# bytedance/particle-sfm

Hardware: AMD Instinct MI355X
Metric: trajectory-points/s (higher is better)
Workload: dtype f32 sampling + f64 positions; 1 GPU; configs[1]: synthetic 100x(1920x1080) flow pairs, sample_ratio=2, flow_check + chaining + occlusion + id assignment, 1 sequence per GPU; frames=101, height=1080, width=1920, trajectories=2073277, parallelism=sequence-per-gpu x1, world_size=1

## Files before the change

particle-sfm_amd/csrc/psfm_api.hip:

```cpp
#include <stdarg.h>
#include <stdio.h>
#include <string.h>
#include <mutex>
#include <shared_mutex>
#include <atomic>
#include <chrono>
#include <stdlib.h>

#include "psfm_internal.h"

static thread_local char g_err[512] = "";
static std::shared_mutex g_dev_gate[16];
std::shared_mutex& psfm_device_gate(int device) { return g_dev_gate[device & 15]; }
static std::atomic<int> g_dev_waiters[16];
int psfm_gate_waiters(int device) { return g_dev_waiters[device & 15].load(std::memory_order_relaxed); }
void psfm_gate_waiters_add(int device, int d) { g_dev_waiters[device & 15].fetch_add(d, std::memory_order_relaxed); }
static int psfm_wants_persist(psfm_ctx* c, bool optimize, int h, int w, int ratio, bool fused)
{
    if (c->chain_mode == 1 || ratio < 1 || !psfm_frame_ok(h, w)) return 0;
    if (optimize) return c->resident_budget > 0 ? 0 : 1;
    const int64_t G = (int64_t)((w + ratio - 1) / ratio) * ((h + ratio - 1) / ratio);
    const int64_t P = (int64_t)h * w;
    const int maxb = psfm_persist_max_blocks(c);
    if (maxb <= 0 || (G + 255) / 256 > maxb) return 0;
    if (c->chain_mode == 2) return 2;
    if (ratio < 2 || G < 100000) return 0;
    if (fused && (G < 400000 || P > 6 * G)) return 0;
    return 1;
}

void psfm_set_error(const char* fmt, ...)
{
    va_list ap;
    va_start(ap, fmt);
    vsnprintf(g_err, sizeof(g_err), fmt, ap);
    va_end(ap);
}

extern "C" const char* psfm_last_error(void) { return g_err; }
extern "C" int psfm_version(void) { return PSFM_VERSION; }

extern "C" int psfm_device_count(void)
{
    int n = 0;
    if (hipGetDeviceCount(&n) != hipSuccess) { (void)hipGetLastError(); return 0; }
    return n;
}

psfm_status PsfmBuf::ensure(size_t need)
{
    if (need <= bytes) return PSFM_OK;
    if (p) { (void)hipFree(p); p = nullptr; bytes = 0; }
    size_t want = (need + (size_t)(1 << 20) - 1) & ~((size_t)(1 << 20) - 1);
    hipError_t e = hipMalloc(&p, want);
    if (e != hipSuccess) {
        p = nullptr;
        psfm_set_error("hipMalloc(%zu bytes) failed: %s", want, hipGetErrorString(e));
        return PSFM_ERR_HIP;
    }
    bytes = want;
    return PSFM_OK;
}

void PsfmBuf::release()
{
    if (p) (void)hipFree(p);
    p = nullptr;
    bytes = 0;
}

hipEvent_t PsfmProfiler::get()
{
    if (!pool.empty()) { hipEvent_t e = pool.back(); pool.pop_back(); return e; }
    hipEvent_t e;
    (void)hipEventCreate(&e);
    return e;
}
void PsfmProfiler::begin(int kind, hipStream_t s)
{
    if (!enabled) return;
    Span sp; sp.kind = kind; sp.a = get(); sp.b = get();
    (void)hipEventRecord(sp.a, s);
    spans.push_back(sp);
}
void PsfmProfiler::kernel_span(int kind, hipEvent_t* a, hipEvent_t* b, bool always)
{
    if (!enabled || (!always && (calls++ % stride) != 0)) { *a = nullptr; *b = nullptr; return; }
    Span sp; sp.kind = kind; sp.a = get(); sp.b = get();
    spans.push_back(sp);
    *a = sp.a; *b = sp.b;
}
void PsfmProfiler::end(hipStream_t s)
{
    if (!enabled) return;
    (void)hipEventRecord(spans.back().b, s);
}
void PsfmProfiler::collect()
{
    for (auto& sp : spans) {
        float ms = 0.f;
        if (hipEventElapsedTime(&ms, sp.a, sp.b) == hipSuccess) { total_ms[sp.kind] += ms; launches[sp.kind]++; }
        pool.push_back(sp.a); pool.push_back(sp.b);
    }
    spans.clear();
}
void PsfmProfiler::reset()
{
    for (int k = 0; k < PSFM_PROF_KINDS; ++k) { total_ms[k] = 0; launches[k] = 0; }
}
void PsfmProfiler::destroy()
{
    collect();
    for (auto e : pool) (void)hipEventDestroy(e);
    pool.clear();
}

#define PSFM_CHECK_CTX(c)                                                     \
    do {                                                                      \
        if (!(c)) { psfm_set_error("ctx is NULL"); return PSFM_ERR_ARG; }     \
        PSFM_HIP(hipSetDevice((c)->device));                                  \
    } while (0)

extern "C" psfm_status psfm_ctx_create(int device, psfm_ctx** out)
{
    if (!out) { psfm_set_error("psfm_ctx_create: out is NULL"); return PSFM_ERR_ARG; }
    *out = nullptr;
    int n = 0;
    hipError_t e = hipGetDeviceCount(&n);
    if (e != hipSuccess || n <= 0) {
        (void)hipGetLastError();
        psfm_set_error("no HIP device available (%s); libpsfm_hip has no CPU fallback",
                       e != hipSuccess ? hipGetErrorString(e) : "device count 0");
        return PSFM_ERR_HIP;
    }
    if (device < 0 || device >= n) { psfm_set_error("device %d out of range [0,%d)", device, n); return PSFM_ERR_ARG; }
    PSFM_HIP(hipSetDevice(device));
    psfm_ctx* c = new psfm_ctx();
    c->device = device;
    c->host_pinned_bytes = 512 + sizeof(PsfmShard) * PSFM_NSHARD + 4096;
    e = hipHostMalloc(&c->host_pinned, c->host_pinned_bytes, hipHostMallocDefault);
    if (e != hipSuccess) { delete c; psfm_set_error("hipHostMalloc failed: %s", hipGetErrorString(e)); return PSFM_ERR_HIP; }
    *out = c;
    return PSFM_OK;
}

extern "C" psfm_status psfm_ctx_destroy(psfm_ctx* c)
{
    if (!c) return PSFM_OK;
    (void)hipSetDevice(c->device);
    PsfmBuf* bufs[] = {&c->log, &c->birth_frame, &c->birth_idx, &c->free_stack, &c->fin_keys, &c->fin_lanes,
                       &c->occupied, &c->counters, &c->shards, &c->survivors, &c->sort_keys, &c->sort_lanes, &c->sort_tmp,
                       &c->scan_tmp, &c->fin_marks, &c->res_birth, &c->res_len, &c->res_off, &c->res_xy, &c->sol_x, &c->sol_state,
                       &c->sol_partials, &c->sol_ctrl, &c->sol_misc, &c->sol_stats, &c->sol_fused, &c->sol_bar, &c->sol_list, &c->occ_own, &c->occ2_own,
                       &c->handoff, &c->seg_info, &c->seg_table, &c->persist_bar, &c->batch_tab, &c->batch_ws, &c->batch_fc, &c->win_ws, &c->flt_ids, &c->flt_birth, &c->flt_len, &c->flt_off, &c->flt_xy,
                       &c->mt_kp_off, &c->mt_q, &c->mt_pts, &c->mt_kp_ind, &c->mt_kp_xy, &c->mt_moff, &c->mt_keys, &c->mt_rows, &c->mt_gid, &c->mt_pairs,
                       &c->lb_state, &c->lb_first, &c->lb_flag, &c->lb_ws, &c->lb_ids, &c->lb_off, &c->lb_frames, &c->lb_xy, &c->lb_labels};
    for (auto b : bufs) b->release();
    for (void*& q : c->peer_opened) { if (q) (void)hipIpcCloseMemHandle(q); q = nullptr; }
    c->peer_area.release();
    psfm_shard_abandon(c);
    c->prof.destroy();
    if (c->side_stream) (void)hipStreamDestroy(c->side_stream);
    if (c->redo_stream) (void)hipStreamDestroy(c->redo_stream);
    if (c->copy_stream) (void)hipStreamDestroy(c->copy_stream);
    if (c->copy_stream2) (void)hipStreamDestroy(c->copy_stream2);
    for (void* p : c->ingest_slots) (void)hipHostFree(p);
    for (hipEvent_t e : c->ingest_events) (void)hipEventDestroy(e);
    if (c->host_pinned) (void)hipHostFree(c->host_pinned);
    if (c->host_seg) (void)hipHostFree(c->host_seg);
    if (c->host_batch) (void)hipHostFree(c->host_batch);
    if (c->host_batch2) (void)hipHostFree(c->host_batch2);
    delete c;
    return PSFM_OK;
}

extern "C" psfm_status psfm_ctx_set_capacity(psfm_ctx* c, double lane_factor, double traj_factor)
{
    if (!c || !(lane_factor >= 1.0) || !(traj_factor >= 1.0)) { psfm_set_error("psfm_ctx_set_capacity: factors must be >= 1"); return PSFM_ERR_ARG; }
    c->lane_factor = lane_factor;
    c->traj_factor = traj_factor;
    return PSFM_OK;
}

extern "C" psfm_status psfm_ctx_set_chain_mode(psfm_ctx* c, int mode)
{
    if (!c || mode < 0 || mode > 2) { psfm_set_error("psfm_ctx_set_chain_mode: mode must be 0 (auto), 1 (per-frame launches) or 2 (persistent loop)"); return PSFM_ERR_ARG; }
    c->chain_mode = mode;
    return PSFM_OK;
}

extern "C" psfm_status psfm_ctx_set_solver(psfm_ctx* c, int mode, int k)
{
    if (!c || mode < 0 || mode > 2 || k < 0 || k > psfm_solve_kmax()) {
        psfm_set_error("psfm_ctx_set_solver: mode must be 0 (adaptive), 1 (launch chain) or 2 (fused solve), k in [0, %d]", psfm_solve_kmax());
        return PSFM_ERR_ARG;
    }
    c->solver_mode = mode;
    c->solver_K = k;
    return PSFM_OK;
}

extern "C" psfm_status psfm_solver_counters(psfm_ctx* c, int64_t* fused, int64_t* fused_redone, int64_t* chain, int32_t* k_now)
{
    if (!c) { psfm_set_error("ctx is NULL"); return PSFM_ERR_ARG; }
    if (fused) *fused = c->n_fused_ok;
    if (fused_redone) *fused_redone = c->n_fused_redone;
    if (chain) *chain = c->n_chain;
    if (k_now) *k_now = c->solve_K;
    return PSFM_OK;
}

extern "C" psfm_status psfm_ctx_set_resident_budget(psfm_ctx* c, int blocks)
{
    if (!c || blocks < 0) { psfm_set_error("psfm_ctx_set_resident_budget: blocks must be >= 0"); return PSFM_ERR_ARG; }
    c->resident_budget = blocks;
    return PSFM_OK;
}

extern "C" psfm_status psfm_resident_capacity(psfm_ctx* c, int32_t* blocks)
{
    PSFM_CHECK_CTX(c);
    if (blocks) *blocks = psfm_resident_blocks(c);
    return PSFM_OK;
}

extern "C" psfm_status psfm_solver_launches(psfm_ctx* c, int64_t* resident, int64_t* giveups, int64_t* iterations)
{
    if (!c) { psfm_set_error("ctx is NULL"); return PSFM_ERR_ARG; }
    if (resident) *resident = c->n_resident;
    if (giveups) *giveups = c->pc_giveups;
    if (iterations) *iterations = c->n_iter_launches;
    return PSFM_OK;
}

extern "C" psfm_status psfm_ctx_set_profiling(psfm_ctx* c, int enable)
{
    if (!c) { psfm_set_error("ctx is NULL"); return PSFM_ERR_ARG; }
    c->prof.enabled = enable != 0;
    c->prof.stride = enable > 1 ? enable : 1;
    c->prof.calls = 0;
    c->prof.collect();
    c->prof.reset();
    return PSFM_OK;
}

extern "C" psfm_status psfm_profile_get(psfm_ctx* c, int kind, double* total_ms, int64_t* launches)
{
    if (!c || kind < 0 || kind >= PSFM_PROF_KINDS) { psfm_set_error("psfm_profile_get: bad argument"); return PSFM_ERR_ARG; }
    if (total_ms) *total_ms = c->prof.total_ms[kind];
    if (launches) *launches = c->prof.launches[kind];
    return PSFM_OK;
}

extern "C" psfm_status psfm_flow_check(psfm_ctx* c, const float* flows_f, const float* flows_b, int n_pairs, int h, int w,
                                       float thres, uint8_t* occ_out, float* err_out, void* stream)
{
    PSFM_CHECK_CTX(c);
    PsfmGate gate(c->device, 0);
    if (n_pairs < 0 || !psfm_frame_ok(h, w) || (n_pairs > 0 && (!flows_f || !flows_b || !occ_out))) {
        psfm_set_error("psfm_flow_check: bad argument (n_pairs=%d h=%d w=%d)", n_pairs, h, w);
        return PSFM_ERR_ARG;
    }
    hipStream_t s = (hipStream_t)stream;
    c->prof.begin(PSFM_PROF_FLOW_CHECK, s);
    psfm_status st = psfm_launch_flow_check(flows_f, flows_b, n_pairs, h, w, thres, occ_out, err_out, s);
    c->prof.end(s);
    return st;
}

extern "C" psfm_status psfm_grid_sample(psfm_ctx* c, const float* map_hwc, int ch, int h, int w, const double* xy,
                                        int64_t n, float* out, void* stream)
{
    PSFM_CHECK_CTX(c);
    PsfmGate gate(c->device, 0);
    if ((ch != 1 && ch != 2) || !psfm_frame_ok(h, w) || n < 0 || (n > 0 && (!map_hwc || !xy || !out))) {
        psfm_set_error("psfm_grid_sample: bad argument (c=%d h=%d w=%d n=%lld)", ch, h, w, (long long)n);
        return PSFM_ERR_ARG;
    }
    return psfm_launch_grid_sample(map_hwc, ch, h, w, xy, n, out, (hipStream_t)stream);
}

extern "C" psfm_status psfm_optimize_location(psfm_ctx* c, const double* uv12, const double* ref1, const double* ref2,
                                              const double* scale, const float* flow12, int64_t n, int w, int h,
                                              double* out, psfm_solve_stats* stats_host, void* stream)
{
    PSFM_CHECK_CTX(c);
    PsfmGate gate(c->device, (c->chain_mode == 1 || c->resident_budget > 0) ? 0 : 1);
    c->pc_persist_ok = gate.exclusive || c->resident_budget > 0;
    c->pc_giveups = 0;
    c->n_resident = c->n_iter_launches = 0;
    if (n < 0 || !psfm_frame_ok(h, w) || (n > 0 && (!uv12 || !ref1 || !ref2 || !scale || !flow12 || !out))) {
        psfm_set_error("psfm_optimize_location: bad argument (n=%lld h=%d w=%d)", (long long)n, h, w);
        return PSFM_ERR_ARG;
    }
    psfm_solve_stats st;
    memset(&st, 0, sizeof(st));
    hipStream_t s = (hipStream_t)stream;
    c->prof.begin(PSFM_PROF_SOLVER, s);
    psfm_status rc = psfm_solve_batch(c, uv12, ref1, ref2, scale, flow12, n, w, h, out, &st, s);
    c->prof.end(s);
    if (stats_host) *stats_host = st;
    return rc;
}

extern "C" psfm_status psfm_path_consistency_eval(psfm_ctx* c, const double* uv12, const double* ref1, const double* ref2,
                                                  const double* scale, const float* flow12, int64_t n, int w, int h,
                                                  double* residuals, double* jacobians, void* stream)
{
    PSFM_CHECK_CTX(c);
    PsfmGate gate(c->device, 0);
    if (n < 0 || n > 0x3fffffff || !psfm_frame_ok(h, w) || (n > 0 && (!uv12 || !ref1 || !ref2 || !scale || !flow12 || (!residuals && !jacobians)))) {
        psfm_set_error("psfm_path_consistency_eval: bad argument (n=%lld h=%d w=%d)", (long long)n, h, w);
        return PSFM_ERR_ARG;
    }
    return psfm_launch_pc_eval(uv12, ref1, ref2, scale, flow12, n, w, h, residuals, jacobians, (hipStream_t)stream);
}

extern "C" psfm_status psfm_sort_records(psfm_ctx* c, uint32_t* keys, int32_t* values, int64_t n, int end_bit, void* stream)
{
    PSFM_CHECK_CTX(c);
    PsfmGate gate(c->device, 0);
    if (n < 0 || n >= (1ll << 31) || end_bit < 1 || end_bit > 32 || (n > 0 && (!keys || !values))) {
        psfm_set_error("psfm_sort_records: bad argument (n=%lld end_bit=%d)", (long long)n, end_bit);
        return PSFM_ERR_ARG;
    }
    if (n == 0) return PSFM_OK;
    hipStream_t s = (hipStream_t)stream;
    psfm_status st;
    if ((st = c->sort_keys.ensure(sizeof(unsigned long long) * (size_t)n * 2)) != PSFM_OK) return st;
    if ((st = c->sort_lanes.ensure(sizeof(int) * (size_t)n * 2)) != PSFM_OK) return st;
    const int64_t half = psfm_sort_pairs32_passes((unsigned)end_bit) % 2 == 0 ? 0 : n;
    unsigned* k0 = c->sort_keys.as<unsigned>();
    int* v0 = c->sort_lanes.as<int>();
    PSFM_HIP(hipMemcpyAsync(k0 + half, keys, sizeof(unsigned) * (size_t)n, hipMemcpyDeviceToDevice, s));
    PSFM_HIP(hipMemcpyAsync(v0 + half, values, sizeof(int) * (size_t)n, hipMemcpyDeviceToDevice, s));
    if ((st = psfm_sort_pairs32(c, k0, v0, k0 + n, v0 + n, n, (unsigned)end_bit, s)) != PSFM_OK) return st;
    PSFM_HIP(hipMemcpyAsync(keys, k0, sizeof(unsigned) * (size_t)n, hipMemcpyDeviceToDevice, s));
    PSFM_HIP(hipMemcpyAsync(values, v0, sizeof(int) * (size_t)n, hipMemcpyDeviceToDevice, s));
    return PSFM_OK;
}

psfm_status psfm_track_dims(psfm_ctx* c, int n_flows, int h, int w, int ratio, int64_t g_own, PsfmTrackDims& d)
{
    d.H = h; d.W = w; d.ratio = ratio; d.n_flows = n_flows;
    d.GW = (w + ratio - 1) / ratio; d.GH = (h + ratio - 1) / ratio;
    d.G = (int64_t)d.GW * d.GH;
    const int64_t Gown = g_own < 0 ? d.G : (g_own > 0 ? g_own : 1);
    d.cap = (int64_t)(c->lane_factor * (double)Gown);
    d.cap = ((d.cap + 255) / 256) * 256;
    const int64_t n_blocks = d.cap / 256;
    {
        const int64_t gb = (Gown + 255) / 256;
        d.nsh = (int)(gb < PSFM_NSHARD ? (gb > 0 ? gb : 1) : PSFM_NSHARD);
    }
    d.free_cap = (int)(((n_blocks + d.nsh - 1) / d.nsh) * 256) + 1024;
    const double tf = c->traj_factor > (double)n_flows / 8.0 ? c->traj_factor : (double)n_flows / 8.0;
    d.shard_cap = (int)(((int64_t)(tf * (double)Gown) + d.cap) / d.nsh) + 1024;
    d.traj_cap = (int64_t)d.shard_cap * PSFM_NSHARD;
    if (d.cap > 0x7fffffff / 2 || d.traj_cap > 0x7fffffff / 2) { psfm_set_error("psfm_track: grid too large"); return PSFM_ERR_ARG; }
    d.shift_b = 1; while ((1ll << d.shift_b) < d.G) ++d.shift_b;
    int tbits = 1; while ((1ll << tbits) < (long long)n_flows + 2) ++tbits;
    d.shift_d = d.shift_b + tbits;
    if (d.shift_d + tbits > 63) { psfm_set_error("psfm_track: key does not fit 64 bits"); return PSFM_ERR_ARG; }
    d.cw = (float)((double)(w - 1) / 2.0); d.ch = (float)((double)(h - 1) / 2.0);
    return PSFM_OK;
}

psfm_status psfm_track_alloc(psfm_ctx* c, const PsfmTrackDims& d)
{
    psfm_status st;
    const int n_flows = d.n_flows;
    if ((st = c->log.ensure(sizeof(double2) * (size_t)(n_flows + 1) * d.cap)) != PSFM_OK) return st;
    if ((st = c->birth_frame.ensure(sizeof(int) * d.cap)) != PSFM_OK) return st;
    if ((st = c->birth_idx.ensure(sizeof(int) * d.cap)) != PSFM_OK) return st;
    if ((st = c->free_stack.ensure(sizeof(int) * (size_t)d.free_cap * PSFM_NSHARD * 2)) != PSFM_OK) return st;
    if ((st = c->shards.ensure(sizeof(PsfmShard) * PSFM_NSHARD * 2)) != PSFM_OK) return st;
    if ((st = c->fin_keys.ensure(sizeof(unsigned long long) * d.traj_cap)) != PSFM_OK) return st;
    if ((st = c->fin_lanes.ensure(sizeof(int) * d.traj_cap)) != PSFM_OK) return st;
    if ((st = c->occupied.ensure((size_t)d.G * 3 + 8)) != PSFM_OK) return st;
    if ((st = c->counters.ensure(sizeof(PsfmCounters))) != PSFM_OK) return st;
    if ((st = c->survivors.ensure(sizeof(int) * (size_t)(n_flows + 1))) != PSFM_OK) return st;
    return PSFM_OK;
}

struct PsfmOccPipeline {
    int chunk = 0;
    std::vector<hipEvent_t> ready;
    std::vector<hipEvent_t> ready_s2;
    int waited = -1, waited_s2 = -1;
    psfm_status need(int pair, bool s2, hipStream_t s)
    {
        if (chunk <= 0) return PSFM_OK;
        std::vector<hipEvent_t>& ev = s2 ? ready_s2 : ready;
        int& w = s2 ? waited_s2 : waited;
        const int cidx = pair / chunk;
        while (w < cidx && w + 1 < (int)ev.size()) {
            ++w;
            PSFM_HIP(hipStreamWaitEvent(s, ev[w], 0));
        }
        return PSFM_OK;
    }
};

static psfm_status psfm_track_impl(psfm_ctx* c, const float* flows, const uint8_t* occ, const float* flows_f2,
                                   const uint8_t* occ_s2, int n_flows, int h, int w, int ratio, psfm_track_info* info,
                                   void* stream, PsfmOccPipeline* pipe, PsfmGate& gate,
                                   const float* fuse_flows_b = nullptr, float fuse_thres = 0.f, int64_t occ_pitch = 0)
{
    const bool device_is_ours = gate.exclusive;
    if (occ_pitch == 0) occ_pitch = (int64_t)h * w;
    PSFM_CHECK_CTX(c);
    psfm_shard_abandon(c);
    const bool optimize = flows_f2 != nullptr;
    if (n_flows < 1 || !psfm_frame_ok(h, w) || ratio < 1 || !flows || !occ || (optimize && !occ_s2 && n_flows > 1)) {
        psfm_set_error("psfm_track: bad argument (n_flows=%d h=%d w=%d ratio=%d)", n_flows, h, w, ratio);
        return PSFM_ERR_ARG;
    }
    if (ratio > 64) { psfm_set_error("psfm_track: sample_ratio %d > 64 unsupported", ratio); return PSFM_ERR_ARG; }
    hipStream_t s = (hipStream_t)stream;
    PsfmTrackDims d;
    psfm_status st;
    if ((st = psfm_track_dims(c, n_flows, h, w, ratio, -1, d)) != PSFM_OK) return st;
    const int64_t P = (int64_t)h * w;
    if ((st = psfm_track_alloc(c, d)) != PSFM_OK) return st;

    c->solve_stats.clear();
    c->res_n_traj = c->res_n_points = 0;
    c->res_n_flows = n_flows;
    c->pc_persist_ok = device_is_ours || c->resident_budget > 0;
    c->pc_giveups = 0;

    if (!optimize && c->chain_mode != 1) {
        const int maxb = psfm_persist_max_blocks(c);
        const int64_t need_blocks = (d.G + 255) / 256;
        if (maxb > 0 && need_blocks <= maxb && device_is_ours) {
            PsfmTrackDims dp = d;
            int64_t nb = need_blocks <= 256 ? 2 * need_blocks + 4 : need_blocks + need_blocks / 4;
            dp.nblk = (int)(nb < maxb ? nb : maxb);
            if (fuse_flows_b) {
                const int64_t fc_blocks = (P + 1023) / 1024;
                const int64_t want = fc_blocks < maxb ? fc_blocks : maxb;
                if (want > dp.nblk) dp.nblk = (int)want;
            }
            dp.cap = (int64_t)dp.nblk * (256 + psfm_persist_guests());
            dp.nsh = dp.nblk < PSFM_NSHARD ? dp.nblk : PSFM_NSHARD;
            dp.free_cap = (int)(((dp.nblk + dp.nsh - 1) / dp.nsh) * 256) + 1024;
            dp.seg_cap = (int)(d.traj_cap / dp.nblk) + 64;
            dp.spill_cap = (int)(d.traj_cap / 8) + 4096;
            const int64_t fin_total = (int64_t)dp.nblk * dp.seg_cap + dp.spill_cap;
            if ((st = c->log.ensure(sizeof(double2) * (size_t)(n_flows + 1) * dp.cap)) != PSFM_OK) return st;
            if ((st = c->free_stack.ensure(sizeof(int) * (size_t)dp.free_cap * PSFM_NSHARD * 2)) != PSFM_OK) return st;
            if ((st = c->fin_keys.ensure(sizeof(unsigned long long) * fin_total)) != PSFM_OK) return st;
            if ((st = c->fin_lanes.ensure(sizeof(int) * fin_total)) != PSFM_OK) return st;
            if ((st = c->handoff.ensure((size_t)dp.nblk * 256 * 24)) != PSFM_OK) return st;
            if ((st = c->seg_info.ensure(sizeof(int) * 2 * (size_t)dp.nblk)) != PSFM_OK) return st;
            if ((st = c->persist_bar.ensure((size_t)(4 * PSFM_NSHARD + 1) * 128)) != PSFM_OK) return st;
            if (pipe && (st = pipe->need(n_flows - 1, false, s)) != PSFM_OK) return st;
            bool fallback = false;
            {
                const bool trace = getenv("PSFM_TRACE") != nullptr;
                const auto t1 = std::chrono::steady_clock::now();
                st = psfm_launch_chain_persist(c, dp, flows, occ, occ_pitch, fuse_flows_b, fuse_thres, s);
                if (st == PSFM_ERR_CAPACITY) {
                    fallback = true;
                    st = PSFM_OK;
                } else {
                    if (st != PSFM_OK) return st;
                    c->prof.begin(PSFM_PROF_FINALIZE, s);
                    st = psfm_finalize_persist(c, dp, &fallback, s);
                    c->prof.end(s);
                }
                if (trace) {
                    const auto t2 = std::chrono::steady_clock::now();
                    fprintf(stderr, "[psfm %p] persistent loop: launch+finalize %.2f ms, fallback %d, overflow %d\n", (void*)c,
                            std::chrono::duration<double, std::milli>(t2 - t1).count(), (int)fallback,
                            ((PsfmCounters*)c->host_pinned)->overflow);
                }
            }
            if (st != PSFM_OK) return st;
            if (!fallback) {
                PSFM_HIP(hipStreamSynchronize(s));
                c->prof.collect();
                if (info) {
                    memset(info, 0, sizeof(*info));
                    info->n_traj = c->res_n_traj;
                    info->n_points = c->res_n_points;
                    info->n_lanes_peak = ((PsfmCounters*)c->host_pinned)->n_lanes;
                    info->lane_capacity = dp.cap;
                    info->chain_mode = 2;
                }
                return PSFM_OK;
            }
            c->prof.collect();
        }
    }
    if (fuse_flows_b) {
        c->prof.begin(PSFM_PROF_FLOW_CHECK, s);
        for (int f = 0; f < n_flows; ++f)
            if ((st = psfm_launch_flow_check(flows + (size_t)f * P * 2, fuse_flows_b + (size_t)f * P * 2, 1, h, w, fuse_thres,
                                             const_cast<uint8_t*>(occ) + (size_t)f * occ_pitch, nullptr, s)) != PSFM_OK) return st;
        c->prof.end(s);
    }
    if ((st = psfm_launch_track_init(c, d, s)) != PSFM_OK) return st;
    int64_t total_iters = 0;
    static const int check_env = getenv("PSFM_CHECK_FRAMES") ? atoi(getenv("PSFM_CHECK_FRAMES")) : 0;
    const int PSFM_CHECK = check_env >= 2 ? check_env : 16;
    std::vector<psfm_solve_stats> hstats((size_t)n_flows + 1);
    int first_unchecked = 1;
    if (optimize) {
        if ((st = c->sol_stats.ensure(sizeof(psfm_solve_stats) * (size_t)(n_flows + 1))) != PSFM_OK) return st;
    }
    const char* unroll_env = getenv("PSFM_SOLVE_UNROLL");
    const int unroll_fixed = unroll_env ? (atoi(unroll_env) < 1 ? 1 : atoi(unroll_env)) : 0;
    c->n_fused_ok = c->n_fused_redone = c->n_chain = 0;
    c->n_resident = c->n_iter_launches = 0;
    if (optimize && (st = psfm_solve_prepare(c, d, s)) != PSFM_OK) return st;
    static const bool merge = !(getenv("PSFM_MERGE_FRAME") && atoi(getenv("PSFM_MERGE_FRAME")) == 0);
    const bool seq_env = !(getenv("PSFM_SEQ") && atoi(getenv("PSFM_SEQ")) == 0);
    bool seq_ok = optimize && merge && seq_env && unroll_fixed == 0;
    int launch_id = 0;
    int idle_windows = 0;
    bool pc_in_step = true;
    int* hpc = (int*)((char*)c->host_pinned + 320);
    PsfmCounters* dctr = c->counters.as<PsfmCounters>();

    auto checkpoint = [&](int f_hi, bool fused_now, bool seq, int* f_next) -> psfm_status {
        PsfmCounters* hc = (PsfmCounters*)c->host_pinned;
        PSFM_HIP(hipMemcpyAsync(hc, c->counters.p, sizeof(PsfmCounters), hipMemcpyDeviceToHost, s));
        PSFM_HIP(hipMemcpyAsync(hstats.data() + first_unchecked, c->sol_stats.as<psfm_solve_stats>() + first_unchecked,
                                sizeof(psfm_solve_stats) * (size_t)(f_hi - first_unchecked + 1), hipMemcpyDeviceToHost, s));
        PSFM_HIP(hipStreamSynchronize(s));
        if (gate.yield_exclusive()) c->pc_persist_ok = c->resident_budget > 0;
        if ((hc->overflow & 7) != 0 || hc->n_lanes > d.cap) {
            psfm_set_error("capacity exceeded: lanes used %d of %lld, overflow bits %d (frame %d of %d); raise psfm_ctx_set_capacity",
                           hc->n_lanes, (long long)d.cap, hc->overflow, hc->pc_frame, n_flows);
            return PSFM_ERR_CAPACITY;
        }
        const int stalled = hc->stall ? hc->stall - 1 : -1;
        int last_ok = f_hi;
        if (seq) {
            const int pcf = hc->pc_frame < n_flows ? hc->pc_frame : n_flows;
            last_ok = pcf - 1;
        }
        if (stalled >= 0) {
            const int fs = stalled;
            psfm_solve_stats ss;
            memset(&ss, 0, sizeof(ss));
            const int k_used = c->solver_K > 0 ? c->solver_K : c->solve_K;
            psfm_status st2 = psfm_solve_frame_resume(c, d, flows + (size_t)(fs - 1) * P * 2, flows + (size_t)fs * P * 2,
                                                      flows_f2 + (size_t)(fs - 1) * P * 2, occ_s2 + (size_t)(fs - 1) * P, fs, &ss,
                                                      (fused_now && !seq && c->solver_K == 0 && k_used < psfm_solve_kmax())
                                                          ? (k_used + 2 < psfm_solve_kmax() ? k_used + 2 : psfm_solve_kmax()) : 0,
                                                      !fused_now, s);
            if (st2 != PSFM_OK) return st2;
            hstats[fs] = ss;
            last_ok = fs;
            pc_in_step = false;
        }
        int max_it = 0, n_solved = 0, n_unclean = 0, k_need = 2;
        for (int k = first_unchecked; k <= last_ok; ++k) {
            if (hstats[k].termination >= 0) {
                c->solve_stats.push_back(hstats[k]);
                total_iters += hstats[k].iterations;
                const psfm_solve_stats& q = hstats[k];
                const bool clean = q.dogleg_nonGN == 0 && q.termination != PSFM_TERM_FAILURE &&
                                   (q.iterations == q.successful_steps + 1 ||
                                    (q.termination == PSFM_TERM_GRADIENT_TOL && q.iterations == q.successful_steps)) &&
                                   q.successful_steps + 1 <= psfm_solve_kmax();
                ++n_solved;
                if (!clean) ++n_unclean;
                else if (q.successful_steps + 1 > k_need) k_need = q.successful_steps + 1;
                if (!fused_now) ++c->n_chain;
                else if (k == stalled) ++c->n_fused_redone;
                else ++c->n_fused_ok;
            }
            if (hstats[k].iterations > max_it) max_it = hstats[k].iterations;
        }
        if (n_solved > 0) {
            c->solve_mode = (n_unclean * 8 > n_solved) ? 1 : 0;
            if (seq) {
                int hist[16] = {0};
                for (int k = first_unchecked; k <= last_ok; ++k)
                    if (hstats[k].termination >= 0) ++hist[hstats[k].successful_steps + 1 < 15 ? hstats[k].successful_steps + 1 : 15];
                int best = 2;
                for (int q = 2; q <= psfm_solve_kmax(); ++q) if (hist[q] > hist[best]) best = q;
                c->solve_K = best;
            } else {
                c->solve_K = k_need > c->solve_K ? k_need : c->solve_K - (c->solve_K - k_need + 1) / 2;
            }
        }
        int want = max_it + 1;
        want = want < 4 ? 4 : (want > 64 ? 64 : want);
        c->solve_unroll = want > c->solve_unroll ? want : c->solve_unroll - (c->solve_unroll - want + 1) / 2;
        first_unchecked = last_ok + 1;
        *f_next = last_ok + 1;
        return PSFM_OK;
    };

    int f = 0;
    while (f < n_flows) {
        const bool fused_now = c->solver_mode == 2 || (c->solver_mode == 0 && c->solve_mode == 0);
        if (seq_ok && fused_now && f >= 1) {
            const int k_now = c->solver_K > 0 ? c->solver_K : c->solve_K;
            if (!pc_in_step) {
                hpc[0] = f; hpc[1] = 0; hpc[2] = launch_id; hpc[3] = k_now;
                PSFM_HIP(hipMemcpyAsync(&dctr->pc_frame, hpc, 4 * sizeof(int), hipMemcpyHostToDevice, s));
                pc_in_step = true;
            } else {
                hpc[3] = k_now;
                PSFM_HIP(hipMemcpyAsync(&dctr->solve_K, hpc + 3, sizeof(int), hipMemcpyHostToDevice, s));
            }
            const int left = n_flows - f;
            const int n_launch = (left < PSFM_CHECK ? left : PSFM_CHECK) + 2;
            const int f_hi = f + n_launch - 1 < n_flows - 1 ? f + n_launch - 1 : n_flows - 1;
            if (pipe && (st = pipe->need(f_hi, false, s)) != PSFM_OK) return st;
            if (pipe && (st = pipe->need(f_hi - 1, true, s)) != PSFM_OK) return st;
            if ((st = psfm_launch_seq(c, d, flows, occ, occ_pitch, flows_f2, occ_s2, n_launch, launch_id, s)) != PSFM_OK) return st;
            launch_id += n_launch;
            const int f_before = f;
            if ((st = checkpoint(f_hi, true, true, &f)) != PSFM_OK) return st;
            if (f == f_before) {
                if (getenv("PSFM_TRACE")) {
                    const PsfmCounters* hc = (const PsfmCounters*)c->host_pinned;
                    unsigned tk[8] = {0};
                    if (c->sol_fused.p) (void)hipMemcpy(tk, c->sol_fused.p, sizeof(tk), hipMemcpyDeviceToHost);
                    fprintf(stderr, "[psfm %p] device-paced window without a completed frame: host frame %d, next launch %d; device pc {frame %d, phase %d, "
                            "owner %d, K %d}, lanes %d (snapshots %d %d), stall %d, overflow %d, tickets %u %u %u %u\n", (void*)c, f, launch_id,
                            hc->pc_frame, hc->pc_phase, hc->pc_owner, hc->solve_K, hc->n_lanes, hc->n_lanes_snap[0], hc->n_lanes_snap[1], hc->stall,
                            hc->overflow, tk[0], tk[1], tk[2], tk[3]);
                }
                if (++idle_windows > 8) { psfm_set_error("psfm_track: the device-paced sequence made no progress in 8 windows (frame %d)", f); return PSFM_ERR_SOLVER; }
            } else {
                idle_windows = 0;
            }
            continue;
        }
        pc_in_step = false;
        if (pipe && (st = pipe->need(f, false, s)) != PSFM_OK) return st;
        const bool solve_now = optimize && f + 1 >= 2;
        if (solve_now && fused_now && merge) {
            if (pipe && (st = pipe->need(f - 1, true, s)) != PSFM_OK) return st;
            st = psfm_launch_frame(c, d, flows + (size_t)(f - 1) * P * 2, flows + (size_t)f * P * 2, flows_f2 + (size_t)(f - 1) * P * 2,
                                   occ + (size_t)f * occ_pitch, occ_s2 + (size_t)(f - 1) * P, f, c->solver_K > 0 ? c->solver_K : c->solve_K, s);
            if (st != PSFM_OK) return st;
        } else {
            st = psfm_launch_chain_step(c, d, flows + (size_t)f * P * 2, occ + (size_t)f * occ_pitch, f, optimize, s);
            if (st != PSFM_OK) return st;
            if (solve_now) {
                if (pipe && (st = pipe->need(f - 1, true, s)) != PSFM_OK) return st;
                if (fused_now) {
                    st = psfm_solve_frame_fused(c, d, flows + (size_t)(f - 1) * P * 2, flows + (size_t)f * P * 2,
                                                flows_f2 + (size_t)(f - 1) * P * 2, occ_s2 + (size_t)(f - 1) * P, f,
                                                c->solver_K > 0 ? c->solver_K : c->solve_K, s);
                } else {
                    c->prof.begin(PSFM_PROF_SOLVER, s);
                    st = psfm_solve_frame_enqueue(c, d, flows + (size_t)(f - 1) * P * 2, flows + (size_t)f * P * 2,
                                                  flows_f2 + (size_t)(f - 1) * P * 2, occ_s2 + (size_t)(f - 1) * P, f,
                                                  unroll_fixed > 0 ? unroll_fixed : c->solve_unroll, s);
                    c->prof.end(s);
                }
                if (st != PSFM_OK) return st;
            }
        }
        if (optimize && f >= 1 && ((f % PSFM_CHECK) == PSFM_CHECK - 1 || f == n_flows - 1)) {
            if ((st = checkpoint(f, fused_now, false, &f)) != PSFM_OK) return st;
            continue;
        }
        ++f;
    }
    if (optimize && n_flows >= 2 && (st = psfm_solve_flush(c, d, n_flows - 1, s)) != PSFM_OK) return st;
    c->prof.begin(PSFM_PROF_FINALIZE, s);
    st = psfm_finalize(c, d, s);
    c->prof.end(s);
    if (st != PSFM_OK) return st;
    PSFM_HIP(hipStreamSynchronize(s));
    c->prof.collect();
    if (info) {
        memset(info, 0, sizeof(*info));
        info->n_traj = c->res_n_traj;
        info->n_points = c->res_n_points;
        info->n_lanes_peak = ((PsfmCounters*)c->host_pinned)->n_lanes;
        info->lane_capacity = d.cap;
        info->solver_iterations = total_iters;
        info->n_solves = (int32_t)c->solve_stats.size();
        info->chain_mode = 1;
    }
    return PSFM_OK;
}

extern "C" psfm_status psfm_track(psfm_ctx* c, const float* flows, const uint8_t* occ, const float* flows_f2,
                                  const uint8_t* occ_s2, int n_flows, int h, int w, int ratio, psfm_track_info* info,
                                  void* stream)
{
    PSFM_CHECK_CTX(c);
    c->res_gen++;
    PsfmGate gate(c->device, psfm_wants_persist(c, flows_f2 != nullptr, h, w, ratio, false));
    return psfm_track_impl(c, flows, occ, flows_f2, occ_s2, n_flows, h, w, ratio, info, stream, nullptr, gate);
}

extern "C" psfm_status psfm_connect(psfm_ctx* c, const float* flows_f, const float* flows_b, const float* flows_f2,
                                    const float* flows_b2, int n_flows, int h, int w, float thres, int ratio,
                                    uint8_t* occ, uint8_t* occ_s2, psfm_track_info* info, void* stream)
{
    PSFM_CHECK_CTX(c);
    c->res_gen++;
    const bool optimize = flows_f2 != nullptr;
    PsfmGate gate(c->device, psfm_wants_persist(c, optimize, h, w, ratio, true));
    if (n_flows < 1 || !psfm_frame_ok(h, w) || !flows_f || !flows_b || (optimize && n_flows > 1 && !flows_b2)) {
        psfm_set_error("psfm_connect: bad argument (n_flows=%d h=%d w=%d)", n_flows, h, w);
        return PSFM_ERR_ARG;
    }
    hipStream_t s = (hipStream_t)stream;
    const size_t P = (size_t)h * w;
    psfm_status st;
    if (gate.exclusive && !optimize && (!occ || (P % 128 == 0 && ((uintptr_t)occ & 127) == 0))) {
        int64_t pitch = (int64_t)P;
        if (!occ) {
            pitch = (int64_t)((P + 127) / 128 * 128);
            if ((st = c->occ_own.ensure((size_t)pitch * (size_t)n_flows)) != PSFM_OK) return st;
            occ = c->occ_own.as<uint8_t>();
        }
        return psfm_track_impl(c, flows_f, occ, nullptr, nullptr, n_flows, h, w, ratio, info, stream, nullptr, gate, flows_b,
                               thres, pitch);
    }
    if (!occ) {
        if ((st = c->occ_own.ensure(P * (size_t)n_flows)) != PSFM_OK) return st;
        occ = c->occ_own.as<uint8_t>();
    }
    const int n2 = optimize ? (n_flows > 1 ? n_flows - 1 : 0) : 0;
    if (optimize && !occ_s2) {
        if ((st = c->occ2_own.ensure(P * (size_t)(n2 > 0 ? n2 : 1))) != PSFM_OK) return st;
        occ_s2 = c->occ2_own.as<uint8_t>();
    }
    if (!c->side_stream) PSFM_HIP(hipStreamCreateWithFlags(&c->side_stream, hipStreamNonBlocking));
    hipStream_t side = c->side_stream;
    hipEvent_t e_in = c->prof.get();
    PSFM_HIP(hipEventRecord(e_in, s));
    PSFM_HIP(hipStreamWaitEvent(side, e_in, 0));
    PsfmOccPipeline pipe;
    pipe.chunk = getenv("PSFM_FC_CHUNK") && atoi(getenv("PSFM_FC_CHUNK")) > 0 ? atoi(getenv("PSFM_FC_CHUNK")) : (optimize ? 5 : 10);
    c->prof.begin(PSFM_PROF_FLOW_CHECK, side);
    const bool bg = optimize && getenv("PSFM_FC_BG") && atoi(getenv("PSFM_FC_BG")) == 1;
    int cus = 256;
    if (bg) {
        (void)hipDeviceGetAttribute(&cus, hipDeviceAttributeMultiprocessorCount, c->device);
        const int mult = getenv("PSFM_FC_BG_BLOCKS") ? atoi(getenv("PSFM_FC_BG_BLOCKS")) : 0;
        cus *= mult > 0 ? mult : 0;
    }
    for (int p0 = 0; p0 < n_flows; p0 += pipe.chunk) {
        const int np = n_flows - p0 < pipe.chunk ? n_flows - p0 : pipe.chunk;
        if (bg && p0 > 0) st = psfm_launch_flow_check_bg(flows_f + (size_t)p0 * P * 2, flows_b + (size_t)p0 * P * 2, np, h, w, thres,
                                                        occ + (size_t)p0 * P, cus, side);
        else st = psfm_launch_flow_check(flows_f + (size_t)p0 * P * 2, flows_b + (size_t)p0 * P * 2, np, h, w, thres,
                                         occ + (size_t)p0 * P, nullptr, side);
        if (st != PSFM_OK) return st;
        hipEvent_t e = c->prof.get();
        PSFM_HIP(hipEventRecord(e, side));
        pipe.ready.push_back(e);
        if (p0 < n2) {
            const int np2 = n2 - p0 < pipe.chunk ? n2 - p0 : pipe.chunk;
            if (bg && p0 > 0) st = psfm_launch_flow_check_bg(flows_f2 + (size_t)p0 * P * 2, flows_b2 + (size_t)p0 * P * 2, np2, h, w, thres,
                                                            occ_s2 + (size_t)p0 * P, cus, side);
            else st = psfm_launch_flow_check(flows_f2 + (size_t)p0 * P * 2, flows_b2 + (size_t)p0 * P * 2, np2, h, w,
                                             thres, occ_s2 + (size_t)p0 * P, nullptr, side);
            if (st != PSFM_OK) return st;
            hipEvent_t e2 = c->prof.get();
            PSFM_HIP(hipEventRecord(e2, side));
            pipe.ready_s2.push_back(e2);
        }
    }
    c->prof.end(side);
    st = psfm_track_impl(c, flows_f, occ, flows_f2, occ_s2, n_flows, h, w, ratio, info, stream, &pipe, gate);
    c->prof.pool.push_back(e_in);
    for (auto e : pipe.ready) c->prof.pool.push_back(e);
    for (auto e : pipe.ready_s2) c->prof.pool.push_back(e);
    return st;
}

extern "C" psfm_status psfm_result_device(psfm_ctx* c, const int32_t** birth, const int32_t** len, const int64_t** off,
                                          const double** xy)
{
    if (!c) { psfm_set_error("ctx is NULL"); return PSFM_ERR_ARG; }
    if (birth) *birth = c->res_birth.as<int32_t>();
    if (len) *len = c->res_len.as<int32_t>();
    if (off) *off = c->res_off.as<int64_t>();
    if (xy) *xy = c->res_xy.as<double>();
    return PSFM_OK;
}

extern "C" psfm_status psfm_result_copy(psfm_ctx* c, int32_t* birth_host, int32_t* len_host, int64_t* off_host,
                                        double* xy_host, void* stream)
{
    PSFM_CHECK_CTX(c);
    PsfmGate gate(c->device, 0);
    hipStream_t s = (hipStream_t)stream;
    const int64_t n = c->res_n_traj, np = c->res_n_points;
    if (n > 0) {
        if (birth_host) PSFM_HIP(hipMemcpyAsync(birth_host, c->res_birth.p, sizeof(int32_t) * n, hipMemcpyDeviceToHost, s));
        if (len_host) PSFM_HIP(hipMemcpyAsync(len_host, c->res_len.p, sizeof(int32_t) * n, hipMemcpyDeviceToHost, s));
        if (off_host) PSFM_HIP(hipMemcpyAsync(off_host, c->res_off.p, sizeof(int64_t) * (n + 1), hipMemcpyDeviceToHost, s));
        if (xy_host && np > 0) PSFM_HIP(hipMemcpyAsync(xy_host, c->res_xy.p, sizeof(double) * 2 * np, hipMemcpyDeviceToHost, s));
    } else if (off_host) {
        off_host[0] = 0;
    }
    PSFM_HIP(hipStreamSynchronize(s));
    return PSFM_OK;
}

extern "C" psfm_status psfm_result_solve_stats(psfm_ctx* c, psfm_solve_stats* stats_host, int32_t max_n, int32_t* n_out)
{
    if (!c) { psfm_set_error("ctx is NULL"); return PSFM_ERR_ARG; }
    const int32_t n = (int32_t)c->solve_stats.size();
    if (n_out) *n_out = n;
    if (stats_host) for (int32_t i = 0; i < n && i < max_n; ++i) stats_host[i] = c->solve_stats[i];
    return PSFM_OK;
}
```

particle-sfm_amd/csrc/psfm_finalize.hip:

```cpp
#include <cstring>
#include <stdio.h>
#include <rocprim/device/device_radix_sort.hpp>
#include <rocprim/device/device_scan.hpp>

#include "psfm_device.h"
#include "psfm_internal.h"

#define PSFM_BLOCK 256

__device__ __forceinline__ void psfm_collect_alive_body(
    const int* __restrict__ birth_frame, const int* __restrict__ birth_idx, PsfmCounters* __restrict__ ctr,
    PsfmShard* __restrict__ shards, unsigned long long* __restrict__ fin_keys, int* __restrict__ fin_lanes, int cap,
    int shard_cap, int last_time, int shift_b, int shift_d)
{
    __shared__ int s_cnt[PSFM_BLOCK / PSFM_WAVE];
    __shared__ int s_base;
    const int n_lanes = min(ctr->n_lanes, cap);
    if ((int)(blockIdx.x * PSFM_BLOCK) >= n_lanes) return;
    const int i = blockIdx.x * PSFM_BLOCK + threadIdx.x;
    int bf = -1;
    if (i < n_lanes) bf = birth_frame[i];
    const bool pending = bf <= -2;
    const bool alive = (bf >= 0) | pending;
    const int my_last = pending ? last_time - 1 : last_time;
    if (pending) bf = -2 - bf;
    const unsigned long long am = __ballot(alive);
    const int lane = psfm_lane_id(), wave = threadIdx.x / PSFM_WAVE;
    if (lane == 0) s_cnt[wave] = __popcll(am);
    __syncthreads();
    const int shard = blockIdx.x % PSFM_NSHARD;
    if (threadIdx.x == 0) {
        int tot = 0;
        for (int w = 0; w < PSFM_BLOCK / PSFM_WAVE; ++w) tot += s_cnt[w];
        s_base = tot > 0 ? atomicAdd(&shards[shard].fin_cnt, tot) : 0;
    }
    __syncthreads();
    if (alive) {
        int r = s_base + psfm_rank_in(am);
        for (int w = 0; w < wave; ++w) r += s_cnt[w];
        if (r < shard_cap) {
            const int64_t o = (int64_t)shard * shard_cap + r;
            fin_keys[o] = ((unsigned long long)my_last << shift_d) | ((unsigned long long)bf << shift_b) |
                          (unsigned long long)birth_idx[i];
            fin_lanes[o] = i;
        } else {
            atomicOr(&ctr->overflow, 2);
        }
    }
}

__global__ __launch_bounds__(PSFM_BLOCK) void psfm_collect_alive_kernel(
    const int* __restrict__ birth_frame, const int* __restrict__ birth_idx, PsfmCounters* __restrict__ ctr,
    PsfmShard* __restrict__ shards, unsigned long long* __restrict__ fin_keys, int* __restrict__ fin_lanes, int cap,
    int shard_cap, int last_time, int shift_b, int shift_d)
{
    psfm_collect_alive_body(birth_frame, birth_idx, ctr, shards, fin_keys, fin_lanes, cap, shard_cap, last_time, shift_b, shift_d);
}

struct PsfmKeyFmt { int shift_b, shift_d; int use32; };
__device__ __forceinline__ unsigned psfm_key32(unsigned long long k, const PsfmKeyFmt& f)
{
    const unsigned last = (unsigned)(k >> f.shift_d);
    const unsigned birth = (unsigned)((k >> f.shift_b) & ((1ull << (f.shift_d - f.shift_b)) - 1ull));
    const unsigned idx = (unsigned)(k & ((1ull << f.shift_b) - 1ull));
    return ((last * (last + 1u) / 2u + birth) << f.shift_b) | idx;
}
__device__ __forceinline__ void psfm_put_key(unsigned long long* keys, int64_t pos, unsigned long long k, const PsfmKeyFmt& f)
{
    if (f.use32) ((unsigned*)keys)[pos] = psfm_key32(k, f);
    else keys[pos] = k;
}

struct PsfmShardOffsets { int count[PSFM_NSHARD]; int64_t start[PSFM_NSHARD]; };
__global__ __launch_bounds__(PSFM_BLOCK) void psfm_compact_shards_kernel(
    const unsigned long long* __restrict__ fin_keys, const int* __restrict__ fin_lanes, int shard_cap,
    PsfmShardOffsets so, unsigned long long* __restrict__ keys, int* __restrict__ lanes, PsfmKeyFmt fmt)
{
    const int shard = blockIdx.y;
    const int n = so.count[shard];
    for (int i = blockIdx.x * PSFM_BLOCK + threadIdx.x; i < n; i += gridDim.x * PSFM_BLOCK) {
        psfm_put_key(keys, so.start[shard] + i, fin_keys[(int64_t)shard * shard_cap + i], fmt);
        lanes[so.start[shard] + i] = fin_lanes[(int64_t)shard * shard_cap + i];
    }
}

__global__ __launch_bounds__(PSFM_BLOCK) void psfm_decode_kernel(const unsigned long long* __restrict__ keys, int64_t n,
                                                                 int shift_b, int shift_d, int* __restrict__ birth,
                                                                 int* __restrict__ len, int64_t* __restrict__ len64)
{
    const int64_t i = (int64_t)blockIdx.x * PSFM_BLOCK + threadIdx.x;
    if (i > n) return;
    if (i == n) { len64[i] = 0; return; }
    const unsigned long long k = keys[i];
    const int last = (int)(k >> shift_d);
    const int b = (int)((k >> shift_b) & ((1ull << (shift_d - shift_b)) - 1ull));
    birth[i] = b;
    len[i] = last - b + 1;
    len64[i] = (int64_t)(last - b + 1);
}

__global__ __launch_bounds__(PSFM_BLOCK) void psfm_decode32_kernel(const unsigned* __restrict__ keys, int64_t n, int shift_b,
                                                                   int* __restrict__ birth, int* __restrict__ len,
                                                                   int64_t* __restrict__ len64)
{
    const int64_t i = (int64_t)blockIdx.x * PSFM_BLOCK + threadIdx.x;
    if (i > n) return;
    if (i == n) { len64[i] = 0; return; }
    const unsigned tri = keys[i] >> shift_b;
    int l = (int)((sqrtf(8.0f * (float)tri + 1.0f) - 1.0f) * 0.5f);
    while (l > 0 && (unsigned)l * (unsigned)(l + 1) / 2u > tri) --l;
    while ((unsigned)(l + 1) * (unsigned)(l + 2) / 2u <= tri) ++l;
    const int b = (int)(tri - (unsigned)l * (unsigned)(l + 1) / 2u);
    birth[i] = b;
    len[i] = l - b + 1;
    len64[i] = (int64_t)(l - b + 1);
}

#define PSFM_PLAN_MAX_GROUPS 16384
#define PSFM_PLAN_BLOCK 1024
struct PsfmPlan {
    const int* gstart; const int64_t* goff;
    const void* keys; int use32, shift_b, shift_d;
    int* birth_w; int* len_w; int64_t* off_w;
};
__device__ __forceinline__ void psfm_tri_invert(unsigned tri, int* last, int* birth)
{
    int l = (int)((sqrtf(8.0f * (float)tri + 1.0f) - 1.0f) * 0.5f);
    while (l > 0 && (unsigned)l * (unsigned)(l + 1) / 2u > tri) --l;
    while ((unsigned)(l + 1) * (unsigned)(l + 2) / 2u <= tri) ++l;
    *last = l;
    *birth = (int)(tri - (unsigned)l * (unsigned)(l + 1) / 2u);
}
__device__ __forceinline__ void psfm_key_fields(const void* keys, int64_t id, int use32, int shift_b, int shift_d, int* last, int* birth, int* idx)
{
    if (use32) {
        const unsigned k = ((const unsigned*)keys)[id];
        psfm_tri_invert(k >> shift_b, last, birth);
        *idx = (int)(k & ((1u << shift_b) - 1u));
    } else {
        const unsigned long long k = ((const unsigned long long*)keys)[id];
        *last = (int)(k >> shift_d);
        *birth = (int)((k >> shift_b) & ((1ull << (shift_d - shift_b)) - 1ull));
        *idx = (int)(k & ((1ull << shift_b) - 1ull));
    }
}
__device__ __forceinline__ int psfm_key_group(const void* keys, int64_t id, int use32, int shift_b, int shift_d)
{
    if (use32) return (int)(((const unsigned*)keys)[id] >> shift_b);
    const unsigned long long k = ((const unsigned long long*)keys)[id];
    const unsigned last = (unsigned)(k >> shift_d);
    const unsigned birth = (unsigned)((k >> shift_b) & ((1ull << (shift_d - shift_b)) - 1ull));
    return (int)(last * (last + 1u) / 2u + birth);
}

__global__ __launch_bounds__(PSFM_BLOCK) void psfm_group_bounds_kernel(const void* __restrict__ keys, int64_t n, int use32, int shift_b,
                                                                       int shift_d, int* __restrict__ gstart)
{
    const int64_t i = (int64_t)blockIdx.x * PSFM_BLOCK + threadIdx.x;
    if (i >= n) return;
    const int g = psfm_key_group(keys, i, use32, shift_b, shift_d);
    const int gp = i > 0 ? psfm_key_group(keys, i - 1, use32, shift_b, shift_d) : -1;
    if (g != gp) gstart[g] = (int)i;
}

__global__ __launch_bounds__(PSFM_PLAN_BLOCK) void psfm_group_plan_kernel(int* __restrict__ marks, int* __restrict__ gstart,
                                                                          int64_t* __restrict__ goff, int ng, int64_t n,
                                                                          int64_t* __restrict__ off_n)
{
    __shared__ int s_g[PSFM_PLAN_MAX_GROUPS];
    __shared__ int s_wmin[PSFM_PLAN_BLOCK / PSFM_WAVE];
    __shared__ long long s_wsum[PSFM_PLAN_BLOCK / PSFM_WAVE];
    constexpr int NW = PSFM_PLAN_BLOCK / PSFM_WAVE;
    constexpr int INF = 0x7fffffff;
    const int tid = threadIdx.x, lane = tid & (PSFM_WAVE - 1), wave = tid / PSFM_WAVE;
    for (int k = tid; k < ng; k += PSFM_PLAN_BLOCK) {
        const int v = marks[k];
        s_g[k] = v;
        gstart[k] = v;
        if (v >= 0) marks[k] = -1;
    }
    __syncthreads();
    const int per = (ng + PSFM_PLAN_BLOCK - 1) / PSFM_PLAN_BLOCK;
    const int g0 = min(tid * per, ng), g1 = min(g0 + per, ng);
    int first = INF;
    for (int g = g1 - 1; g >= g0; --g) if (s_g[g] >= 0) first = s_g[g];
    int sm = first;
#pragma unroll
    for (int o = 1; o < PSFM_WAVE; o <<= 1) {
        const int v = __shfl_down(sm, o);
        if (lane + o < PSFM_WAVE && v < sm) sm = v;
    }
    if (lane == 0) s_wmin[wave] = sm;
    int nxt = __shfl_down(sm, 1);
    if (lane == PSFM_WAVE - 1) nxt = INF;
    __syncthreads();
    for (int w = wave + 1; w < NW; ++w) nxt = min(nxt, s_wmin[w]);
    if (nxt == INF) nxt = (int)n;
    int last = 0, birth = 0;
    if (g0 < g1) psfm_tri_invert((unsigned)g0, &last, &birth);
    for (int g = g1 - 1; g >= g0; --g) {
        const int st = s_g[g];
        if (st >= 0) { s_g[g] = nxt - st; nxt = st; } else s_g[g] = 0;
    }
    long long pts = 0;
    {
        int l = last, b = birth;
        for (int g = g0; g < g1; ++g) {
            pts += (long long)s_g[g] * (long long)(l - b + 1);
            if (++b > l) { ++l; b = 0; }
        }
    }
    long long inc = pts;
#pragma unroll
    for (int o = 1; o < PSFM_WAVE; o <<= 1) {
        const long long v = __shfl_up(inc, o);
        if (lane >= o) inc += v;
    }
    if (lane == PSFM_WAVE - 1) s_wsum[wave] = inc;
    __syncthreads();
    long long base = 0, total = 0;
    for (int w = 0; w < NW; ++w) { const long long v = s_wsum[w]; if (w < wave) base += v; total += v; }
    long long run = base + inc - pts;
    {
        int l = last, b = birth;
        for (int g = g0; g < g1; ++g) {
            goff[g] = run;
            run += (long long)s_g[g] * (long long)(l - b + 1);
            if (++b > l) { ++l; b = 0; }
        }
    }
    if (tid == 0) *off_n = total;
}

__device__ __forceinline__ void psfm_track_header(const PsfmPlan& pl, const int* __restrict__ birth, const int* __restrict__ len,
                                                  int64_t id, int* b, int* l, int* idx)
{
    if (pl.gstart) {
        int last;
        psfm_key_fields(pl.keys, id, pl.use32, pl.shift_b, pl.shift_d, &last, b, idx);
        *l = last - *b + 1;
    } else {
        *b = birth[id]; *l = len[id]; *idx = -1;
    }
}
__device__ __forceinline__ int64_t psfm_track_offset(const PsfmPlan& pl, const int64_t* __restrict__ off, int64_t id, int b, int l)
{
    if (!pl.gstart) return off[id];
    const int last = b + l - 1;
    const int g = last * (last + 1) / 2 + b;
    const int64_t o = pl.goff[g] + (id - (int64_t)pl.gstart[g]) * (int64_t)l;
    pl.birth_w[id] = b; pl.len_w[id] = l; pl.off_w[id] = o;
    return o;
}

#ifndef TILE_J
#define TILE_J 64
#endif
#ifndef TILE_K
#define TILE_K 32
#endif
__device__ __forceinline__ void psfm_gather_body(const double2* __restrict__ log, int64_t cap,
                                                                 const int* __restrict__ lanes,
                                                                 const int* __restrict__ birth,
                                                                 const int* __restrict__ len,
                                                                 const int64_t* __restrict__ off, int64_t n,
                                                                 double2* __restrict__ out, const PsfmPlan& pl)
{
    __shared__ double2 tile[TILE_J][TILE_K + 1];
    __shared__ int s_lane[TILE_J], s_birth[TILE_J], s_len[TILE_J];
    __shared__ int64_t s_off[TILE_J];
    __shared__ int s_maxlen;
    const int tid = threadIdx.x;
    const int64_t id0 = (int64_t)blockIdx.x * TILE_J;
    int hb = 0, hl = 0;
    if (tid == 0) s_maxlen = 0;
    __syncthreads();
    if (tid < TILE_J) {
        const int64_t id = id0 + tid;
        const bool ok = id < n;
        int b = 0, l = 0, idx;
        const int my_lane = ok ? lanes[id] : 0;
        if (ok) psfm_track_header(pl, birth, len, id, &b, &l, &idx);
        hb = b; hl = l;
        s_lane[tid] = my_lane;
        s_birth[tid] = b;
        s_len[tid] = l;
        if (ok) atomicMax(&s_maxlen, l);
    }
    __syncthreads();
    const int maxlen = s_maxlen;
    const int j = tid & (TILE_J - 1);
    const int q = tid / TILE_J;
    constexpr int NLD = TILE_K * TILE_J / PSFM_BLOCK;
    const int lj = s_len[j];
    const int64_t col = s_lane[j];
    const int bj = s_birth[j];
    double2 r[NLD];
#pragma unroll
    for (int u = 0; u < NLD; ++u) {
        const int t = q + u * (PSFM_BLOCK / TILE_J);
        r[u] = t < lj ? log[(int64_t)(bj + t) * cap + col] : make_double2(0.0, 0.0);
    }
    if (tid < TILE_J) s_off[tid] = id0 + tid < n ? psfm_track_offset(pl, off, id0 + tid, hb, hl) : 0;
    for (int k0 = 0; k0 < maxlen; k0 += TILE_K) {
#pragma unroll
        for (int u = 0; u < NLD; ++u) tile[j][q + u * (PSFM_BLOCK / TILE_J)] = r[u];
        __syncthreads();
        if (k0 + TILE_K < maxlen) {
#pragma unroll
            for (int u = 0; u < NLD; ++u) {
                const int t = k0 + TILE_K + q + u * (PSFM_BLOCK / TILE_J);
                r[u] = t < lj ? log[(int64_t)(bj + t) * cap + col] : make_double2(0.0, 0.0);
            }
        }
        const int kk = tid & (TILE_K - 1);
        for (int jj = tid / TILE_K; jj < TILE_J; jj += PSFM_BLOCK / TILE_K) {
            const int t = k0 + kk;
            if (t < s_len[jj]) out[s_off[jj] + t] = tile[jj][kk];
        }
        __syncthreads();
    }
}

__global__ __launch_bounds__(PSFM_BLOCK) void psfm_gather_kernel(const double2* __restrict__ log, int64_t cap,
                                                                 const int* __restrict__ lanes,
                                                                 const int* __restrict__ birth,
                                                                 const int* __restrict__ len,
                                                                 const int64_t* __restrict__ off, int64_t n,
                                                                 double2* __restrict__ out, PsfmPlan pl)
{
    psfm_gather_body(log, cap, lanes, birth, len, off, n, out, pl);
}

__global__ __launch_bounds__(PSFM_BLOCK) void psfm_gather_delta_kernel(const float2* __restrict__ dlog, int64_t cap,
                                                                       const int* __restrict__ lanes,
                                                                       const int* __restrict__ birth,
                                                                       const int* __restrict__ len,
                                                                       const int64_t* __restrict__ off, int64_t n,
                                                                       const void* __restrict__ keys, int use32, int shift_b,
                                                                       int GW, int ratio, double2* __restrict__ out, PsfmPlan pl)
{
    __shared__ float2 dtile[TILE_J][TILE_K + 1];
    __shared__ double2 tile[TILE_J][TILE_K + 1];
    __shared__ double2 s_pos[TILE_J];
    __shared__ int s_lane[TILE_J], s_birth[TILE_J], s_len[TILE_J];
    __shared__ int64_t s_off[TILE_J];
    __shared__ int s_maxlen;
    const int tid = threadIdx.x;
    const int64_t id0 = (int64_t)blockIdx.x * TILE_J;
    int hb = 0, hl = 0;
    if (tid == 0) s_maxlen = 0;
    __syncthreads();
    if (tid < TILE_J) {
        const int64_t id = id0 + tid;
        const bool ok = id < n;
        int b = 0, l = 0, idx = -1;
        const int my_lane = ok ? lanes[id] : 0;
        if (ok) psfm_track_header(pl, birth, len, id, &b, &l, &idx);
        hb = b; hl = l;
        s_lane[tid] = my_lane;
        s_birth[tid] = b;
        s_len[tid] = l;
        if (ok) {
            atomicMax(&s_maxlen, l);
            if (idx < 0) {
                const unsigned long long mask = (1ull << shift_b) - 1ull;
                idx = (int)((use32 ? (unsigned long long)((const unsigned*)keys)[id] : ((const unsigned long long*)keys)[id]) & mask);
            }
            const int gy = idx / GW, gx = idx - gy * GW;
            s_pos[tid] = make_double2((double)(gx * ratio), (double)(gy * ratio));
        }
    }
    __syncthreads();
    const int maxlen = s_maxlen;
    const int j = tid & (TILE_J - 1);
    const int q = tid / TILE_J;
    constexpr int NLD = TILE_K * TILE_J / PSFM_BLOCK;
    const int lj = s_len[j];
    const int64_t col = s_lane[j];
    const int bj = s_birth[j];
    float2 r[NLD];
#pragma unroll
    for (int u = 0; u < NLD; ++u) {
        const int t = q + u * (PSFM_BLOCK / TILE_J);
        r[u] = (t >= 1 && t < lj) ? dlog[(int64_t)(bj + t - 1) * cap + col] : make_float2(0.f, 0.f);
    }
    if (tid < TILE_J) s_off[tid] = id0 + tid < n ? psfm_track_offset(pl, off, id0 + tid, hb, hl) : 0;
    for (int k0 = 0; k0 < maxlen; k0 += TILE_K) {
#pragma unroll
        for (int u = 0; u < NLD; ++u) dtile[j][q + u * (PSFM_BLOCK / TILE_J)] = r[u];
        __syncthreads();
        if (k0 + TILE_K < maxlen) {
#pragma unroll
            for (int u = 0; u < NLD; ++u) {
                const int t = k0 + TILE_K + q + u * (PSFM_BLOCK / TILE_J);
                r[u] = (t < lj) ? dlog[(int64_t)(bj + t - 1) * cap + col] : make_float2(0.f, 0.f);
            }
        }
        if (tid < TILE_J) {
            double2 pos = s_pos[tid];
            const int l = s_len[tid];
            float2 f[TILE_K];
#pragma unroll
            for (int k = 0; k < TILE_K; ++k) f[k] = dtile[tid][k];
#pragma unroll
            for (int k = 0; k < TILE_K; ++k) {
                const int t = k0 + k;
                if (t >= 1 && t < l) { pos.x = pos.x + (double)f[k].x; pos.y = pos.y + (double)f[k].y; }
                tile[tid][k] = pos;
            }
            s_pos[tid] = pos;
        }
        __syncthreads();
        const int kk = tid & (TILE_K - 1);
        for (int jj = tid / TILE_K; jj < TILE_J; jj += PSFM_BLOCK / TILE_K) {
            const int t = k0 + kk;
            if (t < s_len[jj]) out[s_off[jj] + t] = tile[jj][kk];
        }
        __syncthreads();
    }
}

static PsfmKeyFmt psfm_key_fmt(const PsfmTrackDims& d, unsigned* end_bit)
{
    PsfmKeyFmt f;
    f.shift_b = d.shift_b; f.shift_d = d.shift_d;
    const long long lmax = (long long)d.n_flows + 1;
    const long long tri_max = lmax * (lmax + 1) / 2 + lmax;
    int tri_bits = 1;
    while ((1ll << tri_bits) <= tri_max) ++tri_bits;
    f.use32 = (tri_bits + d.shift_b <= 32) ? 1 : 0;
    int tbits = 1;
    while ((1ll << tbits) < (long long)d.n_flows + 2) ++tbits;
    *end_bit = f.use32 ? (unsigned)(tri_bits + d.shift_b) : (unsigned)(d.shift_d + tbits);
    return f;
}

static bool psfm_own_sort(const PsfmKeyFmt& fmt, int64_t n)
{
    static const int on = getenv("PSFM_FIN_SORT") ? atoi(getenv("PSFM_FIN_SORT")) : 1;
    return on && fmt.use32 && n < (1ll << 31);
}
static bool psfm_records_in_first_half(const PsfmTrackDims& d, int64_t n)
{
    unsigned end_bit = 0;
    const PsfmKeyFmt fmt = psfm_key_fmt(d, &end_bit);
    return psfm_own_sort(fmt, n) && (psfm_sort_pairs32_passes(end_bit) % 2 == 0);
}

static psfm_status psfm_finalize_sorted(psfm_ctx* c, const PsfmTrackDims& d, int64_t n, int64_t npts, bool delta_log, hipStream_t s)
{
    psfm_status st;
    unsigned end_bit = 0;
    const PsfmKeyFmt fmt = psfm_key_fmt(d, &end_bit);
    int* l_in = c->sort_lanes.as<int>() + n;
    int* l_out = c->sort_lanes.as<int>();
    size_t tmp_bytes = 0, scan_bytes = 0;
    PSFM_HIP(rocprim::exclusive_scan(nullptr, scan_bytes, (int64_t*)nullptr, (int64_t*)nullptr, (int64_t)0,
                                     (size_t)(n + 1), rocprim::plus<int64_t>(), s));
    if (psfm_own_sort(fmt, n)) {
        if ((st = c->sort_tmp.ensure(scan_bytes)) != PSFM_OK) return st;
        if ((st = psfm_sort_pairs32(c, c->sort_keys.as<unsigned>(), l_out, c->sort_keys.as<unsigned>() + n, l_in, n, end_bit, s)) != PSFM_OK) return st;
    } else if (fmt.use32) {
        unsigned* k_in = c->sort_keys.as<unsigned>() + n;
        unsigned* k_out = c->sort_keys.as<unsigned>();
        PSFM_HIP(rocprim::radix_sort_pairs(nullptr, tmp_bytes, k_in, k_out, l_in, l_out, (size_t)n, 0u, end_bit, s));
        if ((st = c->sort_tmp.ensure(tmp_bytes > scan_bytes ? tmp_bytes : scan_bytes)) != PSFM_OK) return st;
        PSFM_HIP(rocprim::radix_sort_pairs(c->sort_tmp.p, tmp_bytes, k_in, k_out, l_in, l_out, (size_t)n, 0u, end_bit, s));
    } else {
        unsigned long long* k_in = c->sort_keys.as<unsigned long long>() + n;
        unsigned long long* k_out = c->sort_keys.as<unsigned long long>();
        PSFM_HIP(rocprim::radix_sort_pairs(nullptr, tmp_bytes, k_in, k_out, l_in, l_out, (size_t)n, 0u, end_bit, s));
        if ((st = c->sort_tmp.ensure(tmp_bytes > scan_bytes ? tmp_bytes : scan_bytes)) != PSFM_OK) return st;
        PSFM_HIP(rocprim::radix_sort_pairs(c->sort_tmp.p, tmp_bytes, k_in, k_out, l_in, l_out, (size_t)n, 0u, end_bit, s));
    }
    if ((st = c->res_birth.ensure(sizeof(int) * n)) != PSFM_OK) return st;
    if ((st = c->res_len.ensure(sizeof(int) * n)) != PSFM_OK) return st;
    if ((st = c->res_off.ensure(sizeof(int64_t) * (n + 1))) != PSFM_OK) return st;
    static const int plan_on = getenv("PSFM_FIN_PLAN") ? atoi(getenv("PSFM_FIN_PLAN")) : 1;
    const long long lmax = (long long)d.n_flows + 1;
    const long long ng = lmax * (lmax + 1) / 2 + lmax + 1;
    PsfmPlan pl;
    pl.gstart = nullptr; pl.goff = nullptr; pl.keys = (const void*)c->sort_keys.p; pl.use32 = fmt.use32; pl.shift_b = d.shift_b; pl.shift_d = d.shift_d;
    pl.birth_w = c->res_birth.as<int>(); pl.len_w = c->res_len.as<int>(); pl.off_w = c->res_off.as<int64_t>();
    if (plan_on && ng <= PSFM_PLAN_MAX_GROUPS && n < (1ll << 31)) {
        if ((st = c->scan_tmp.ensure((sizeof(int64_t) + sizeof(int)) * (size_t)ng)) != PSFM_OK) return st;
        int64_t* goff = c->scan_tmp.as<int64_t>();
        int* gstart = (int*)(goff + ng);
        const void* had = c->fin_marks.p;
        if ((st = c->fin_marks.ensure(sizeof(int) * (size_t)PSFM_PLAN_MAX_GROUPS)) != PSFM_OK) return st;
        if (!c->fin_marks_clean || had != c->fin_marks.p)
            PSFM_HIP(hipMemsetAsync(c->fin_marks.p, 0xff, sizeof(int) * (size_t)PSFM_PLAN_MAX_GROUPS, s));
        c->fin_marks_clean = false;
        hipLaunchKernelGGL(psfm_group_bounds_kernel, dim3((unsigned)((n + PSFM_BLOCK - 1) / PSFM_BLOCK)), dim3(PSFM_BLOCK), 0, s,
                           (const void*)c->sort_keys.p, n, fmt.use32, d.shift_b, d.shift_d, c->fin_marks.as<int>());
        hipLaunchKernelGGL(psfm_group_plan_kernel, dim3(1), dim3(PSFM_PLAN_BLOCK), 0, s, c->fin_marks.as<int>(), gstart, goff, (int)ng, n,
                           c->res_off.as<int64_t>() + n);
        PSFM_HIP(hipGetLastError());
        c->fin_marks_clean = true;
        pl.gstart = gstart; pl.goff = goff;
    } else {
        if ((st = c->scan_tmp.ensure(sizeof(int64_t) * (n + 1))) != PSFM_OK) return st;
        if (fmt.use32)
            hipLaunchKernelGGL(psfm_decode32_kernel, dim3((unsigned)((n + 1 + PSFM_BLOCK - 1) / PSFM_BLOCK)), dim3(PSFM_BLOCK), 0, s,
                               c->sort_keys.as<unsigned>(), n, d.shift_b, c->res_birth.as<int>(), c->res_len.as<int>(),
                               c->scan_tmp.as<int64_t>());
        else
            hipLaunchKernelGGL(psfm_decode_kernel, dim3((unsigned)((n + 1 + PSFM_BLOCK - 1) / PSFM_BLOCK)), dim3(PSFM_BLOCK), 0, s,
                               c->sort_keys.as<unsigned long long>(), n, d.shift_b, d.shift_d, c->res_birth.as<int>(),
                               c->res_len.as<int>(), c->scan_tmp.as<int64_t>());
        PSFM_HIP(hipGetLastError());
        PSFM_HIP(rocprim::exclusive_scan(c->sort_tmp.p, scan_bytes, c->scan_tmp.as<int64_t>(), c->res_off.as<int64_t>(),
                                         (int64_t)0, (size_t)(n + 1), rocprim::plus<int64_t>(), s));
    }
    c->res_n_points = npts;
    if ((st = c->res_xy.ensure(sizeof(double2) * (size_t)(npts > 0 ? npts : 1))) != PSFM_OK) return st;
    if (delta_log)
        hipLaunchKernelGGL(psfm_gather_delta_kernel, dim3((unsigned)((n + TILE_J - 1) / TILE_J)), dim3(PSFM_BLOCK), 0, s,
                           c->log.as<float2>(), d.cap, c->sort_lanes.as<int>(), c->res_birth.as<int>(),
                           c->res_len.as<int>(), c->res_off.as<int64_t>(), n, (const void*)c->sort_keys.p, fmt.use32,
                           d.shift_b, d.GW, d.ratio, c->res_xy.as<double2>(), pl);
    else
        hipLaunchKernelGGL(psfm_gather_kernel, dim3((unsigned)((n + TILE_J - 1) / TILE_J)), dim3(PSFM_BLOCK), 0, s,
                           c->log.as<double2>(), d.cap, c->sort_lanes.as<int>(), c->res_birth.as<int>(),
                           c->res_len.as<int>(), c->res_off.as<int64_t>(), n, c->res_xy.as<double2>(), pl);
    PSFM_HIP(hipGetLastError());
    return PSFM_OK;
}

psfm_status psfm_finalize(psfm_ctx* c, const PsfmTrackDims& d, hipStream_t s)
{
    PsfmCounters* ctr = c->counters.as<PsfmCounters>();
    PsfmShard* shards = c->shards.as<PsfmShard>();
    hipLaunchKernelGGL(psfm_collect_alive_kernel, dim3((unsigned)((d.cap + PSFM_BLOCK - 1) / PSFM_BLOCK)), dim3(PSFM_BLOCK),
                       0, s, c->birth_frame.as<int>(), c->birth_idx.as<int>(), ctr, shards,
                       c->fin_keys.as<unsigned long long>(), c->fin_lanes.as<int>(), (int)d.cap, d.shard_cap,
                       d.n_flows, d.shift_b, d.shift_d);
    PSFM_HIP(hipGetLastError());
    PsfmCounters* hc = (PsfmCounters*)c->host_pinned;
    PsfmShard* hs = (PsfmShard*)((char*)c->host_pinned + 512);
    PSFM_HIP(hipMemcpyAsync(hc, ctr, sizeof(PsfmCounters), hipMemcpyDeviceToHost, s));
    PSFM_HIP(hipMemcpyAsync(hs, shards, sizeof(PsfmShard) * PSFM_NSHARD, hipMemcpyDeviceToHost, s));
    PSFM_HIP(hipStreamSynchronize(s));
    PsfmShardOffsets so;
    int64_t n = 0, npts = 0;
    bool over = hc->overflow != 0;
    for (int k = 0; k < PSFM_NSHARD; ++k) npts += hs[k].points;
    for (int k = 0; k < PSFM_NSHARD; ++k) {
        if (hs[k].fin_cnt > d.shard_cap) over = true;
        so.count[k] = hs[k].fin_cnt > d.shard_cap ? d.shard_cap : hs[k].fin_cnt;
        so.start[k] = n;
        n += so.count[k];
    }
    if (over || hc->n_lanes > d.cap) {
        psfm_set_error("capacity exceeded: lanes used %d of %lld, trajectory records %lld of %lld (%d shards); "
                       "raise psfm_ctx_set_capacity", hc->n_lanes, (long long)d.cap, (long long)n,
                       (long long)d.traj_cap, PSFM_NSHARD);
        return PSFM_ERR_CAPACITY;
    }
    c->res_n_traj = n;
    c->res_n_points = 0;
    if (n == 0) return PSFM_OK;
    psfm_status st;
    if ((st = c->sort_keys.ensure(sizeof(unsigned long long) * n * 2)) != PSFM_OK) return st;
    if ((st = c->sort_lanes.ensure(sizeof(int) * n * 2)) != PSFM_OK) return st;
    unsigned end_bit_unused = 0;
    const PsfmKeyFmt fmt = psfm_key_fmt(d, &end_bit_unused);
    const int64_t half = psfm_records_in_first_half(d, n) ? 0 : n;
    unsigned long long* kdst = fmt.use32 ? (unsigned long long*)(c->sort_keys.as<unsigned>() + half) : c->sort_keys.as<unsigned long long>() + half;
    hipLaunchKernelGGL(psfm_compact_shards_kernel, dim3(64, PSFM_NSHARD), dim3(PSFM_BLOCK), 0, s,
                       c->fin_keys.as<unsigned long long>(), c->fin_lanes.as<int>(), d.shard_cap, so,
                       kdst, c->sort_lanes.as<int>() + half, fmt);
    PSFM_HIP(hipGetLastError());
    return psfm_finalize_sorted(c, d, n, npts, false, s);
}

__global__ __launch_bounds__(PSFM_BLOCK) void psfm_compact_segments_kernel(
    const unsigned long long* __restrict__ fin_keys, const int* __restrict__ fin_lanes, const int2* __restrict__ seg_info, int nblk,
    int seg_cap, const PsfmCounters* __restrict__ ctr, int spill_cap, unsigned long long* __restrict__ keys, int* __restrict__ lanes,
    PsfmKeyFmt fmt)
{
    __shared__ long long s_part[PSFM_BLOCK / PSFM_WAVE];
    const int b = blockIdx.x, tid = threadIdx.x;
    long long mine = 0;
    for (int k = tid; k < b; k += PSFM_BLOCK) mine += seg_info[k].x;
#pragma unroll
    for (int o = 32; o > 0; o >>= 1) mine += __shfl_down(mine, o);
    if ((tid & (PSFM_WAVE - 1)) == 0) s_part[tid / PSFM_WAVE] = mine;
    __syncthreads();
    long long dst = 0;
    for (int w = 0; w < PSFM_BLOCK / PSFM_WAVE; ++w) dst += s_part[w];
    const int count = b < nblk ? seg_info[b].x : min(ctr->spill_cnt, spill_cap);
    const long long src = (long long)b * seg_cap;
    for (int i0 = 0; i0 < count; i0 += 4 * PSFM_BLOCK) {
        unsigned long long k[4];
        int l[4];
#pragma unroll
        for (int u = 0; u < 4; ++u) {
            const int i = i0 + u * PSFM_BLOCK + tid;
            k[u] = i < count ? fin_keys[src + i] : 0ull;
            l[u] = i < count ? fin_lanes[src + i] : 0;
        }
#pragma unroll
        for (int u = 0; u < 4; ++u) {
            const int i = i0 + u * PSFM_BLOCK + tid;
            if (i < count) {
                psfm_put_key(keys, dst + i, k[u], fmt);
                lanes[dst + i] = l[u];
            }
        }
    }
}

psfm_status psfm_finalize_persist(psfm_ctx* c, const PsfmTrackDims& d, bool* fallback, hipStream_t s)
{
    *fallback = false;
    const int nseg = d.nblk + 1;
    const size_t need = sizeof(int2) * (size_t)d.nblk;
    if (c->host_seg_bytes < need) {
        if (c->host_seg) (void)hipHostFree(c->host_seg);
        c->host_seg = nullptr; c->host_seg_bytes = 0;
        PSFM_HIP(hipHostMalloc(&c->host_seg, need, hipHostMallocDefault));
        c->host_seg_bytes = need;
    }
    int2* hinfo = (int2*)c->host_seg;
    PsfmCounters* hc = (PsfmCounters*)c->host_pinned;
    PSFM_HIP(hipMemcpyAsync(hc, c->counters.p, sizeof(PsfmCounters), hipMemcpyDeviceToHost, s));
    PSFM_HIP(hipMemcpyAsync(hinfo, c->seg_info.p, sizeof(int2) * (size_t)d.nblk, hipMemcpyDeviceToHost, s));
    PSFM_HIP(hipStreamSynchronize(s));
    if (hc->pad[0]) fprintf(stderr, "psfm persist check: site %d index %d\n", hc->pad[0], hc->pad[1]);
    if (hc->overflow & (4 | 8)) {
        *fallback = true;
        return PSFM_OK;
    }
    int64_t n = 0, npts = 0;
    for (int b = 0; b < d.nblk; ++b) {
        n += hinfo[b].x;
        npts += hinfo[b].y;
    }
    const int spilled = hc->spill_cnt < d.spill_cap ? hc->spill_cnt : d.spill_cap;
    n += spilled;
    if (hc->overflow != 0) {
        psfm_set_error("capacity exceeded (persistent loop): overflow bits %d, trajectory records %lld (%d spilled of %d); "
                       "raise psfm_ctx_set_capacity", hc->overflow, (long long)n, hc->spill_cnt, d.spill_cap);
        return PSFM_ERR_CAPACITY;
    }
    c->res_n_traj = n;
    c->res_n_points = 0;
    if (n == 0) return PSFM_OK;
    psfm_status st;
    if ((st = c->sort_keys.ensure(sizeof(unsigned long long) * n * 2)) != PSFM_OK) return st;
    if ((st = c->sort_lanes.ensure(sizeof(int) * n * 2)) != PSFM_OK) return st;
    unsigned end_bit_unused = 0;
    const PsfmKeyFmt fmt = psfm_key_fmt(d, &end_bit_unused);
    const int64_t half = psfm_records_in_first_half(d, n) ? 0 : n;
    unsigned long long* kdst = fmt.use32 ? (unsigned long long*)(c->sort_keys.as<unsigned>() + half) : c->sort_keys.as<unsigned long long>() + half;
    hipLaunchKernelGGL(psfm_compact_segments_kernel, dim3((unsigned)nseg), dim3(PSFM_BLOCK), 0, s,
                       c->fin_keys.as<unsigned long long>(), c->fin_lanes.as<int>(), (const int2*)c->seg_info.as<int2>(), d.nblk, d.seg_cap,
                       (const PsfmCounters*)c->counters.as<PsfmCounters>(), d.spill_cap, kdst, c->sort_lanes.as<int>() + half, fmt);
    PSFM_HIP(hipGetLastError());
    return psfm_finalize_sorted(c, d, n, npts, true, s);
}

struct PsfmFinSeq {
    const int* birth_frame; const int* birth_idx; PsfmCounters* ctr; PsfmShard* shards;
    unsigned long long* fin_keys; int* fin_lanes;
    const double2* log; int64_t cap;
    int shard_cap, last_time;
    int64_t rec_start, n;
    int* res_birth; int* res_len; int64_t* res_off; double2* res_xy;
};

__global__ __launch_bounds__(PSFM_BLOCK) void psfm_collect_alive_batch_kernel(const PsfmFinSeq* __restrict__ T, int shift_b, int shift_d)
{
    const PsfmFinSeq& q = T[blockIdx.y];
    psfm_collect_alive_body(q.birth_frame, q.birth_idx, q.ctr, q.shards, q.fin_keys, q.fin_lanes, (int)q.cap, q.shard_cap, q.last_time,
                            shift_b, shift_d);
}

__global__ __launch_bounds__(PSFM_WAVE) void psfm_batch_counts_kernel(const PsfmFinSeq* __restrict__ T, long long* __restrict__ counts)
{
    const PsfmFinSeq& q = T[blockIdx.x];
    const int k = threadIdx.x;
    static_assert(PSFM_NSHARD == PSFM_WAVE, "one lane per shard");
    const int fc = q.shards[k].fin_cnt;
    long long n = fc > q.shard_cap ? q.shard_cap : fc;
    long long pts = q.shards[k].points;
    int over = fc > q.shard_cap ? 1 : 0;
#pragma unroll
    for (int o = 32; o > 0; o >>= 1) { n += __shfl_down(n, o); pts += __shfl_down(pts, o); over |= __shfl_down(over, o); }
    if (k == 0) {
        counts[blockIdx.x * 4 + 0] = n;
        counts[blockIdx.x * 4 + 1] = pts;
        counts[blockIdx.x * 4 + 2] = (long long)(q.ctr->overflow | (over ? 2 : 0));
        counts[blockIdx.x * 4 + 3] = (long long)q.ctr->n_lanes;
    }
}

__global__ __launch_bounds__(PSFM_BLOCK) void psfm_compact_shards_batch_kernel(const PsfmFinSeq* __restrict__ T, unsigned long long* __restrict__ keys,
                                                                               int* __restrict__ lanes, PsfmKeyFmt fmt, int seq_shift)
{
    __shared__ int s_cnt[PSFM_NSHARD];
    const int shard = blockIdx.y, seq = blockIdx.z;
    const PsfmFinSeq& q = T[seq];
    if (threadIdx.x < PSFM_NSHARD) { const int fc = q.shards[threadIdx.x].fin_cnt; s_cnt[threadIdx.x] = fc > q.shard_cap ? q.shard_cap : fc; }
    __syncthreads();
    int64_t start = q.rec_start;
    for (int k = 0; k < shard; ++k) start += s_cnt[k];
    const int n = s_cnt[shard];
    for (int i = blockIdx.x * PSFM_BLOCK + threadIdx.x; i < n; i += gridDim.x * PSFM_BLOCK) {
        const unsigned long long k = q.fin_keys[(int64_t)shard * q.shard_cap + i];
        if (fmt.use32) ((unsigned*)keys)[start + i] = psfm_key32(k, fmt) | (seq_shift < 32 ? (unsigned)seq << seq_shift : 0u);
        else keys[start + i] = k | ((unsigned long long)seq << seq_shift);
        lanes[start + i] = q.fin_lanes[(int64_t)shard * q.shard_cap + i];
    }
}

__global__ __launch_bounds__(PSFM_BLOCK) void psfm_decode_batch_kernel(const PsfmFinSeq* __restrict__ T, const void* __restrict__ keys, int64_t n,
                                                                       PsfmKeyFmt fmt, int seq_shift, int64_t* __restrict__ len64)
{
    const int64_t i = (int64_t)blockIdx.x * PSFM_BLOCK + threadIdx.x;
    if (i > n) return;
    if (i == n) { len64[i] = 0; return; }
    int seq, b, last;
    if (fmt.use32) {
        const unsigned k = ((const unsigned*)keys)[i];
        seq = seq_shift < 32 ? (int)(k >> seq_shift) : 0;
        const unsigned tri = (seq_shift < 32 ? k & ((1u << seq_shift) - 1u) : k) >> fmt.shift_b;
        int l = (int)((sqrtf(8.0f * (float)tri + 1.0f) - 1.0f) * 0.5f);
        while (l > 0 && (unsigned)l * (unsigned)(l + 1) / 2u > tri) --l;
        while ((unsigned)(l + 1) * (unsigned)(l + 2) / 2u <= tri) ++l;
        last = l;
        b = (int)(tri - (unsigned)l * (unsigned)(l + 1) / 2u);
    } else {
        const unsigned long long kk = ((const unsigned long long*)keys)[i];
        seq = (int)(kk >> seq_shift);
        const unsigned long long k = kk & ((1ull << seq_shift) - 1ull);
        last = (int)(k >> fmt.shift_d);
        b = (int)((k >> fmt.shift_b) & ((1ull << (fmt.shift_d - fmt.shift_b)) - 1ull));
    }
    const PsfmFinSeq& q = T[seq];
    const int64_t local = i - q.rec_start;
    q.res_birth[local] = b;
    q.res_len[local] = last - b + 1;
    len64[i] = (int64_t)(last - b + 1);
}

__global__ __launch_bounds__(PSFM_BLOCK) void psfm_offsets_batch_kernel(const PsfmFinSeq* __restrict__ T, const int64_t* __restrict__ scan)
{
    const PsfmFinSeq& q = T[blockIdx.y];
    const int64_t i = (int64_t)blockIdx.x * PSFM_BLOCK + threadIdx.x;
    if (i > q.n) return;
    q.res_off[i] = scan[q.rec_start + i] - scan[q.rec_start];
}

__global__ __launch_bounds__(PSFM_BLOCK) void psfm_gather_batch_kernel(const PsfmFinSeq* __restrict__ T, const int* __restrict__ lanes)
{
    const PsfmFinSeq& q = T[blockIdx.y];
    if ((int64_t)blockIdx.x * TILE_J >= q.n) return;
    PsfmPlan none; none.gstart = nullptr;
    psfm_gather_body(q.log, q.cap, lanes + q.rec_start, q.res_birth, q.res_len, q.res_off, q.n, q.res_xy, none);
}

psfm_status psfm_finalize_batch(psfm_ctx* own, psfm_ctx* const* ctxs, const PsfmTrackDims* dims, int n_seq, hipStream_t s)
{
    if (n_seq < 1 || n_seq > PSFM_BATCH_MAX) { psfm_set_error("psfm_finalize_batch: bad batch size %d", n_seq); return PSFM_ERR_ARG; }
    psfm_status st;
    const size_t tbytes = sizeof(PsfmFinSeq) * (size_t)n_seq, cbytes = sizeof(long long) * 4 * (size_t)n_seq;
    const size_t need_host = tbytes + cbytes;
    if (own->host_seg_bytes < need_host) {
        if (own->host_seg) (void)hipHostFree(own->host_seg);
        own->host_seg = nullptr; own->host_seg_bytes = 0;
        PSFM_HIP(hipHostMalloc(&own->host_seg, need_host + 4096, hipHostMallocDefault));
        own->host_seg_bytes = need_host + 4096;
    }
    if ((st = own->seg_table.ensure(tbytes + cbytes)) != PSFM_OK) return st;
    PsfmFinSeq* hT = (PsfmFinSeq*)own->host_seg;
    long long* hcnt = (long long*)((char*)own->host_seg + tbytes);
    PsfmFinSeq* dT = own->seg_table.as<PsfmFinSeq>();
    long long* dcnt = (long long*)((char*)own->seg_table.p + tbytes);
    int64_t cap_max = 0;
    PsfmTrackDims dk = dims[0];
    for (int i = 0; i < n_seq; ++i) {
        const PsfmTrackDims& d = dims[i];
        psfm_ctx* c = ctxs[i];
        if (d.shift_b != dk.shift_b || d.shift_d != dk.shift_d) { psfm_set_error("psfm_finalize_batch: sequences with different key formats"); return PSFM_ERR_ARG; }
        if (d.n_flows > dk.n_flows) dk.n_flows = d.n_flows;
        memset(&hT[i], 0, sizeof(PsfmFinSeq));
        hT[i].birth_frame = c->birth_frame.as<int>(); hT[i].birth_idx = c->birth_idx.as<int>();
        hT[i].ctr = c->counters.as<PsfmCounters>(); hT[i].shards = c->shards.as<PsfmShard>();
        hT[i].fin_keys = c->fin_keys.as<unsigned long long>(); hT[i].fin_lanes = c->fin_lanes.as<int>();
        hT[i].log = c->log.as<double2>(); hT[i].cap = d.cap;
        hT[i].shard_cap = d.shard_cap; hT[i].last_time = d.n_flows;
        if (d.cap > cap_max) cap_max = d.cap;
    }
    PSFM_HIP(hipMemcpyAsync(dT, hT, tbytes, hipMemcpyHostToDevice, s));
    hipLaunchKernelGGL(psfm_collect_alive_batch_kernel, dim3((unsigned)((cap_max + PSFM_BLOCK - 1) / PSFM_BLOCK), (unsigned)n_seq), dim3(PSFM_BLOCK),
                       0, s, dT, dk.shift_b, dk.shift_d);
    hipLaunchKernelGGL(psfm_batch_counts_kernel, dim3((unsigned)n_seq), dim3(PSFM_WAVE), 0, s, dT, dcnt);
    PSFM_HIP(hipGetLastError());
    PSFM_HIP(hipMemcpyAsync(hcnt, dcnt, cbytes, hipMemcpyDeviceToHost, s));
    PSFM_HIP(hipStreamSynchronize(s));
    int64_t N = 0, n_max = 0;
    for (int i = 0; i < n_seq; ++i) {
        psfm_ctx* c = ctxs[i];
        const int64_t n = hcnt[4 * i + 0], npts = hcnt[4 * i + 1];
        PsfmCounters* hc = (PsfmCounters*)c->host_pinned;
        hc->n_lanes = (int)hcnt[4 * i + 3]; hc->overflow = (int)hcnt[4 * i + 2];
        if (hcnt[4 * i + 2] != 0 || hcnt[4 * i + 3] > dims[i].cap) {
            psfm_set_error("capacity exceeded (sequence %d of the batch): lanes used %lld of %lld, trajectory records %lld of %lld, overflow bits %lld; "
                           "raise psfm_ctx_set_capacity", i, hcnt[4 * i + 3], (long long)dims[i].cap, (long long)n, (long long)dims[i].traj_cap,
                           hcnt[4 * i + 2]);
            return PSFM_ERR_CAPACITY;
        }
        c->res_n_traj = n;
        c->res_n_points = npts;
        hT[i].rec_start = N; hT[i].n = n;
        N += n;
        if (n > n_max) n_max = n;
        if ((st = c->res_birth.ensure(sizeof(int) * (size_t)(n > 0 ? n : 1))) != PSFM_OK) return st;
        if ((st = c->res_len.ensure(sizeof(int) * (size_t)(n > 0 ? n : 1))) != PSFM_OK) return st;
        if ((st = c->res_off.ensure(sizeof(int64_t) * (size_t)(n + 1))) != PSFM_OK) return st;
        if ((st = c->res_xy.ensure(sizeof(double2) * (size_t)(npts > 0 ? npts : 1))) != PSFM_OK) return st;
        hT[i].res_birth = c->res_birth.as<int>(); hT[i].res_len = c->res_len.as<int>();
        hT[i].res_off = c->res_off.as<int64_t>(); hT[i].res_xy = c->res_xy.as<double2>();
    }
    PSFM_HIP(hipMemcpyAsync(dT, hT, tbytes, hipMemcpyHostToDevice, s));
    if (N == 0) {
        for (int i = 0; i < n_seq; ++i) PSFM_HIP(hipMemsetAsync(ctxs[i]->res_off.p, 0, sizeof(int64_t), s));
        return PSFM_OK;
    }
    unsigned end_bit = 0;
    PsfmKeyFmt fmt = psfm_key_fmt(dk, &end_bit);
    int seq_bits = 0;
    while ((1 << seq_bits) < n_seq) ++seq_bits;
    if (fmt.use32 && (int)end_bit + seq_bits > 32) {
        fmt.use32 = 0;
        int tbits = 1;
        while ((1ll << tbits) < (long long)dk.n_flows + 2) ++tbits;
        end_bit = (unsigned)(dk.shift_d + tbits);
    }
    if (!fmt.use32 && (int)end_bit + seq_bits > 64) { psfm_set_error("psfm_finalize_batch: key does not fit 64 bits"); return PSFM_ERR_ARG; }
    const int seq_shift = (int)end_bit;
    const unsigned sort_end = end_bit + (unsigned)seq_bits;
    if ((st = own->sort_keys.ensure(sizeof(unsigned long long) * (size_t)N * 2)) != PSFM_OK) return st;
    if ((st = own->sort_lanes.ensure(sizeof(int) * (size_t)N * 2)) != PSFM_OK) return st;
    if ((st = own->scan_tmp.ensure(sizeof(int64_t) * (size_t)(N + 1) * 2)) != PSFM_OK) return st;
    const bool own_sort = psfm_own_sort(fmt, N);
    const int64_t half = (own_sort && psfm_sort_pairs32_passes(sort_end) % 2 == 0) ? 0 : N;
    unsigned long long* kdst = fmt.use32 ? (unsigned long long*)(own->sort_keys.as<unsigned>() + half) : own->sort_keys.as<unsigned long long>() + half;
    hipLaunchKernelGGL(psfm_compact_shards_batch_kernel, dim3(8, PSFM_NSHARD, (unsigned)n_seq), dim3(PSFM_BLOCK), 0, s, dT, kdst,
                       own->sort_lanes.as<int>() + half, fmt, seq_shift);
    PSFM_HIP(hipGetLastError());
    int* l_in = own->sort_lanes.as<int>() + N;
    int* l_out = own->sort_lanes.as<int>();
    size_t tmp_bytes = 0, scan_bytes = 0;
    PSFM_HIP(rocprim::exclusive_scan(nullptr, scan_bytes, (int64_t*)nullptr, (int64_t*)nullptr, (int64_t)0, (size_t)(N + 1),
                                     rocprim::plus<int64_t>(), s));
    if (own_sort) {
        if ((st = own->sort_tmp.ensure(scan_bytes)) != PSFM_OK) return st;
        if ((st = psfm_sort_pairs32(own, own->sort_keys.as<unsigned>(), l_out, own->sort_keys.as<unsigned>() + N, l_in, N, sort_end, s)) != PSFM_OK) return st;
    } else if (fmt.use32) {
        unsigned* k_in = own->sort_keys.as<unsigned>() + N;
        unsigned* k_out = own->sort_keys.as<unsigned>();
        PSFM_HIP(rocprim::radix_sort_pairs(nullptr, tmp_bytes, k_in, k_out, l_in, l_out, (size_t)N, 0u, sort_end, s));
        if ((st = own->sort_tmp.ensure(tmp_bytes > scan_bytes ? tmp_bytes : scan_bytes)) != PSFM_OK) return st;
        PSFM_HIP(rocprim::radix_sort_pairs(own->sort_tmp.p, tmp_bytes, k_in, k_out, l_in, l_out, (size_t)N, 0u, sort_end, s));
    } else {
        unsigned long long* k_in = own->sort_keys.as<unsigned long long>() + N;
        unsigned long long* k_out = own->sort_keys.as<unsigned long long>();
        PSFM_HIP(rocprim::radix_sort_pairs(nullptr, tmp_bytes, k_in, k_out, l_in, l_out, (size_t)N, 0u, sort_end, s));
        if ((st = own->sort_tmp.ensure(tmp_bytes > scan_bytes ? tmp_bytes : scan_bytes)) != PSFM_OK) return st;
        PSFM_HIP(rocprim::radix_sort_pairs(own->sort_tmp.p, tmp_bytes, k_in, k_out, l_in, l_out, (size_t)N, 0u, sort_end, s));
    }
    int64_t* len64 = own->scan_tmp.as<int64_t>();
    int64_t* scan = len64 + (N + 1);
    hipLaunchKernelGGL(psfm_decode_batch_kernel, dim3((unsigned)((N + 1 + PSFM_BLOCK - 1) / PSFM_BLOCK)), dim3(PSFM_BLOCK), 0, s, dT,
                       (const void*)own->sort_keys.p, N, fmt, seq_shift, len64);
    PSFM_HIP(hipGetLastError());
    PSFM_HIP(rocprim::exclusive_scan(own->sort_tmp.p, scan_bytes, len64, scan, (int64_t)0, (size_t)(N + 1), rocprim::plus<int64_t>(), s));
    hipLaunchKernelGGL(psfm_offsets_batch_kernel, dim3((unsigned)((n_max + 1 + PSFM_BLOCK - 1) / PSFM_BLOCK), (unsigned)n_seq), dim3(PSFM_BLOCK), 0, s,
                       dT, (const int64_t*)scan);
    hipLaunchKernelGGL(psfm_gather_batch_kernel, dim3((unsigned)((n_max + TILE_J - 1) / TILE_J), (unsigned)n_seq), dim3(PSFM_BLOCK), 0, s, dT,
                       (const int*)own->sort_lanes.as<int>());
    PSFM_HIP(hipGetLastError());
    return PSFM_OK;
}
```

particle-sfm_amd/csrc/psfm_internal.h:

```cpp
#pragma once
#include <hip/hip_runtime.h>
#include <stdint.h>
#include <shared_mutex>
#include <string>
#include <vector>

#include "../../include/psfm.h"

#define PSFM_MAX_PEERS 8

void psfm_set_error(const char* fmt, ...);

#define PSFM_HIP(expr)                                                                          \
    do {                                                                                        \
        hipError_t e_ = (expr);                                                                 \
        if (e_ != hipSuccess) {                                                                 \
            psfm_set_error("%s failed: %s (%s:%d)", #expr, hipGetErrorString(e_), __FILE__, __LINE__); \
            return PSFM_ERR_HIP;                                                                \
        }                                                                                       \
    } while (0)

static inline bool psfm_frame_ok(int h, int w) { return h >= 2 && w >= 2 && (int64_t)h * (int64_t)w * 8 < ((int64_t)1 << 32); }

std::shared_mutex& psfm_device_gate(int device);
int psfm_gate_waiters(int device);
void psfm_gate_waiters_add(int device, int d);
struct PsfmGate {
    std::shared_mutex& m;
    int device;
    bool exclusive = false;
    PsfmGate(int dev, int want_exclusive ) : m(psfm_device_gate(dev)), device(dev)
    {
        if (want_exclusive == 2) { m.lock(); exclusive = true; }
        else if (want_exclusive == 1 && m.try_lock()) exclusive = true;
        else if (!m.try_lock_shared()) {
            psfm_gate_waiters_add(device, 1);
            m.lock_shared();
            psfm_gate_waiters_add(device, -1);
        }
    }
    bool yield_exclusive()
    {
        if (!exclusive || psfm_gate_waiters(device) <= 0) return false;
        m.unlock();
        exclusive = false;
        m.lock_shared();
        return true;
    }
    ~PsfmGate() { if (exclusive) m.unlock(); else m.unlock_shared(); }
    PsfmGate(const PsfmGate&) = delete;
    PsfmGate& operator=(const PsfmGate&) = delete;
};

struct PsfmBuf {
    void* p = nullptr;
    size_t bytes = 0;
    psfm_status ensure(size_t need);
    void release();
    template <class T> T* as() const { return (T*)p; }
};

struct PsfmCounters {
    int n_lanes;
    int overflow;
    int stall;
    int abort;
    int spill_cnt;
    int sel;
    int n_lanes_snap[2];
    int pc_frame, pc_phase, pc_owner, solve_K;
    int pad[4];
};

#define PSFM_NSHARD 64
struct PsfmShard {
    int fin_cnt;
    unsigned points;
    int pad0[30];
    int free_top;
    int pad1[31];
};

enum { PSFM_PROF_FLOW_CHECK = 0, PSFM_PROF_CHAIN = 1, PSFM_PROF_RESPAWN = 2, PSFM_PROF_SOLVER = 3,
       PSFM_PROF_FINALIZE = 4, PSFM_PROF_KINDS = 5 };

struct PsfmProfiler {
    bool enabled = false;
    int stride = 1;
    int64_t calls = 0;
    struct Span { int kind; hipEvent_t a, b; };
    std::vector<Span> spans;
    std::vector<hipEvent_t> pool;
    double total_ms[PSFM_PROF_KINDS] = {0};
    int64_t launches[PSFM_PROF_KINDS] = {0};
    hipEvent_t get();
    void begin(int kind, hipStream_t s);
    void kernel_span(int kind, hipEvent_t* a, hipEvent_t* b, bool always = false);
    void end(hipStream_t s);
    void collect();
    void reset();
    void destroy();
};

struct PsfmSolveCtrl;

struct PsfmTrackDims;

struct psfm_ctx {
    int device = 0;
    double lane_factor = 2.0, traj_factor = 8.0;
    PsfmBuf log;
    PsfmBuf birth_frame;
    PsfmBuf birth_idx;
    PsfmBuf free_stack;
    PsfmBuf fin_keys;
    PsfmBuf fin_lanes;
    PsfmBuf occupied;
    PsfmBuf counters;
    PsfmBuf shards;
    PsfmBuf survivors;
    PsfmBuf handoff;
    PsfmBuf seg_info;
    PsfmBuf seg_table;
    PsfmBuf persist_bar;
    int persist_max_blocks = -1;
    int chain_mode = 0;
    void* host_seg = nullptr;
    size_t host_seg_bytes = 0;
    PsfmBuf sort_keys, sort_lanes, sort_tmp, scan_tmp;
    PsfmBuf fin_marks;
    bool fin_marks_clean = false;
    PsfmBuf res_birth, res_len, res_off, res_xy;
    int64_t res_n_traj = 0, res_n_points = 0;
    int res_n_flows = 0;
    PsfmBuf sol_x, sol_state, sol_partials, sol_ctrl, sol_misc, sol_stats, sol_fused, sol_bar;
    PsfmBuf sol_list;
    int pc_persist_blocks[4] = {-1, -1, -1, -1};
    bool pc_persist_ok = false;
    int resident_budget = 0;
    unsigned pc_epoch = 0;
    PsfmBuf peer_area;
    unsigned peer_epoch = 0;
    int peer_world = 0, peer_rank = 0;
    int peer_L[PSFM_MAX_PEERS] = {0};
    void* peer_lead[PSFM_MAX_PEERS] = {nullptr};
    void* peer_opened[PSFM_MAX_PEERS] = {nullptr};
    int pc_giveups = 0;
    int solve_K = 4;
    int solve_mode = 0;
    int solver_mode = 0, solver_K = 0;
    int64_t n_fused_ok = 0, n_fused_redone = 0, n_chain = 0;
    int64_t n_resident = 0, n_iter_launches = 0;
    PsfmTrackDims* shard_dims = nullptr;
    bool shard_optimize = false;
    int solve_unroll = 6;
    PsfmBuf occ_own, occ2_own;
    PsfmBuf batch_tab, batch_ws, batch_fc;
    void* host_batch = nullptr;
    size_t host_batch_bytes = 0;
    void* host_batch2 = nullptr;
    size_t host_batch2_bytes = 0;
    int64_t batch_notrim_shape = 0;
    PsfmBuf win_ws;
    PsfmBuf flt_ids, flt_birth, flt_len, flt_off, flt_xy;
    int64_t flt_n_traj = 0, flt_n_points = 0;
    PsfmBuf mt_kp_off, mt_q, mt_pts, mt_kp_ind, mt_kp_xy, mt_moff, mt_keys, mt_rows, mt_gid, mt_pairs;
    int64_t mt_n_kp = 0, mt_n_m = 0, mt_n_pairs = 0;
    int mt_n_img = 0;
    uint64_t res_gen = 0;
    uint64_t lb_gen = 0;
    bool lb_active = false, lb_finished = false;
    int64_t lb_rows = 0;
    PsfmBuf lb_state, lb_first, lb_flag;
    PsfmBuf lb_ws;
    PsfmBuf lb_ids, lb_off, lb_frames, lb_xy, lb_labels;
    int64_t lb_n_traj = 0, lb_n_points = 0;
    hipStream_t side_stream = nullptr;
    hipStream_t copy_stream = nullptr;
    hipStream_t copy_stream2 = nullptr;
    std::vector<void*> ingest_slots;
    std::vector<hipEvent_t> ingest_events;
    size_t ingest_slot_bytes = 0;
    hipStream_t redo_stream = nullptr;
    std::vector<psfm_solve_stats> solve_stats;
    PsfmProfiler prof;
    void* host_pinned = nullptr;
    size_t host_pinned_bytes = 0;
};

psfm_status psfm_launch_flow_check(const float* ff, const float* fb, int n_pairs, int h, int w, float thres,
                                   uint8_t* occ, float* err, hipStream_t s);
psfm_status psfm_launch_flow_check_bg(const float* ff, const float* fb, int n_pairs, int h, int w, float thres, uint8_t* occ,
                                      int n_blocks, hipStream_t s);
psfm_status psfm_launch_grid_sample(const float* map, int c, int h, int w, const double* xy, int64_t n,
                                    float* out, hipStream_t s);

struct PsfmTrackDims {
    int H, W, ratio, GW, GH, n_flows;
    int64_t G, cap, traj_cap;
    int shard_cap;
    int free_cap;
    int nsh = PSFM_NSHARD;
    int shift_b, shift_d;
    float cw, ch;
    int nblk = 0, seg_cap = 0, spill_cap = 0;
    int64_t g0 = 0, Gband = 0, shard_pitch = 0;
    uint8_t* shard_maps = nullptr;
};

psfm_status psfm_track_dims(psfm_ctx* c, int n_flows, int h, int w, int ratio, int64_t g_own, PsfmTrackDims& d);
psfm_status psfm_track_alloc(psfm_ctx* c, const PsfmTrackDims& d);
psfm_status psfm_launch_track_init(psfm_ctx* c, const PsfmTrackDims& d, hipStream_t s);
psfm_status psfm_launch_chain_step(psfm_ctx* c, const PsfmTrackDims& d, const float* flow, const uint8_t* occ,
                                   int frame, bool optimize, hipStream_t s);

#define PSFM_BATCH_MAX 64
struct PsfmBatchSeq;
struct PsfmFcSeq { const float* ff; const float* fb; uint8_t* occ; int n_pairs; int pad; };
bool psfm_flow_check_batch_ok(int h, int w, const void* ff, const void* fb, const void* occ);
psfm_status psfm_launch_flow_check_batch(const PsfmFcSeq* tab_dev, int n_seq, int pair0, int n_pairs, int h, int w, float thres, hipStream_t s);
void psfm_batch_fill_seq(psfm_ctx* c, const PsfmTrackDims& d, const float* flows, const uint8_t* occ, int64_t occ_pitch, PsfmBatchSeq* row);
psfm_status psfm_launch_track_init_batch(const PsfmBatchSeq* tab_dev, int n_seq, int64_t cap_max, hipStream_t s);
psfm_status psfm_launch_chain_step_batch(psfm_ctx* owner, const PsfmBatchSeq* tab_dev, int n_seq, int ratio, int64_t cap_max, int frame,
                                         bool optimize, hipStream_t s);
size_t psfm_batch_seq_opt_bytes(void);
psfm_status psfm_batch_fill_seq_opt(psfm_ctx* c, const PsfmTrackDims& d, const float* flows, const uint8_t* occ, int64_t occ_pitch,
                                    const float* flows_f2, const uint8_t* occ_s2, void* row_host, hipStream_t s);
psfm_status psfm_launch_seq_batch(psfm_ctx* owner, const void* tab_dev, int n_seq, int ratio, int64_t cap_max, int n_launches, int launch_id0,
                                  hipStream_t s);
psfm_status psfm_launch_flush_batch(const void* tab_dev, int n_seq, int64_t cap_max, hipStream_t s);
psfm_status psfm_launch_batch_set_pc(const void* tab_dev, const int (*v)[4], int n_seq, hipStream_t s);
size_t psfm_batch_pack_row_bytes(int win);
psfm_status psfm_launch_batch_pack(const void* tab_dev, const int* lo, int n_seq, int win, char* out_dev, hipStream_t s);
psfm_status psfm_finalize_batch(psfm_ctx* own, psfm_ctx* const* ctxs, const PsfmTrackDims* dims, int n_seq, hipStream_t s);

struct PsfmMatchSrc {
    int64_t k = 0, n_pts = 0;
    const int64_t* off = nullptr; const int* birth = nullptr; const int* frames = nullptr;
    const double2* xy = nullptr; const uint8_t* labels = nullptr;
    const char* who = "psfm_traj_to_matches";
};
psfm_status psfm_match_tables(psfm_ctx* c, const PsfmMatchSrc& src, int n_img, int sample_k, int64_t* n_kp_host, int64_t* n_matches_host,
                              int64_t* n_pairs_host, hipStream_t s);

int psfm_persist_max_blocks(psfm_ctx* c);
int psfm_persist_guests(void);
psfm_status psfm_launch_chain_persist(psfm_ctx* c, const PsfmTrackDims& d, const float* flows, const uint8_t* occ,
                                      int64_t occ_pitch, const float* flows_b, float thres, hipStream_t s);

psfm_status psfm_finalize(psfm_ctx* c, const PsfmTrackDims& d, hipStream_t s);
int psfm_sort_pairs32_passes(unsigned end_bit);
psfm_status psfm_sort_pairs32(psfm_ctx* c, unsigned* k_half0, int* v_half0, unsigned* k_half1, int* v_half1, int64_t n, unsigned end_bit, hipStream_t s);
psfm_status psfm_finalize_persist(psfm_ctx* c, const PsfmTrackDims& d, bool* fallback, hipStream_t s);

psfm_status psfm_solve_frame_enqueue(psfm_ctx* c, const PsfmTrackDims& d, const float* flow01, const float* flow12,
                                     const float* flow02, const uint8_t* occ02, int frame, int unroll, hipStream_t s);
psfm_status psfm_solve_frame_resume(psfm_ctx* c, const PsfmTrackDims& d, const float* flow01, const float* flow12,
                                    const float* flow02, const uint8_t* occ02, int frame, psfm_solve_stats* st,
                                    int try_fused_k, bool chain_stalled, hipStream_t s);
psfm_status psfm_solve_frame_fused(psfm_ctx* c, const PsfmTrackDims& d, const float* flow01, const float* flow12,
                                   const float* flow02, const uint8_t* occ02, int frame, int K, hipStream_t s);
psfm_status psfm_launch_frame(psfm_ctx* c, const PsfmTrackDims& d, const float* flow01, const float* flow12, const float* flow02,
                              const uint8_t* occ, const uint8_t* occ02, int frame, int K, hipStream_t s, double* export_sums = nullptr);
psfm_status psfm_launch_seq(psfm_ctx* c, const PsfmTrackDims& d, const float* flows, const uint8_t* occ, int64_t occ_pitch,
                            const float* flows_f2, const uint8_t* occ_s2, int n_launches, int launch_id0, hipStream_t s);
psfm_status psfm_solve_flush(psfm_ctx* c, const PsfmTrackDims& d, int frame, hipStream_t s);
psfm_status psfm_solve_prepare(psfm_ctx* c, const PsfmTrackDims& d, hipStream_t s);
int psfm_solve_kmax(void);
int psfm_resident_blocks(psfm_ctx* c);
void psfm_shard_abandon(psfm_ctx* c);
psfm_status psfm_solve_export(psfm_ctx* c, const PsfmTrackDims& d, const float* flow01, const float* flow12, const float* flow02,
                              const uint8_t* occ02, int frame, int kind, int K, double* sums_out, hipStream_t s);
psfm_status psfm_solve_control(psfm_ctx* c, const PsfmTrackDims& d, int frame, int kind, int K, const double* totals, hipStream_t s,
                               int* stall_host = nullptr);
psfm_status psfm_solve_state(psfm_ctx* c, int* done, int* stall, psfm_solve_stats* st, hipStream_t s);
psfm_status psfm_solve_restore(psfm_ctx* c, const PsfmTrackDims& d, int frame, hipStream_t s);
psfm_status psfm_solve_writeback(psfm_ctx* c, const PsfmTrackDims& d, int frame, hipStream_t s);
size_t psfm_peer_area_bytes(void);
size_t psfm_peer_lead_offset(void);
int psfm_peer_leaders(int n_blocks);
int psfm_solve_blocks(psfm_ctx* c, const PsfmTrackDims& d);
psfm_status psfm_solve_frame_enqueue_peer(psfm_ctx* c, const PsfmTrackDims& d, const float* flow01, const float* flow12,
                                          const float* flow02, const uint8_t* occ02, int frame, unsigned epoch, hipStream_t s);
psfm_status psfm_launch_pc_eval(const double* uv12, const double* ref1, const double* ref2, const double* scale, const float* flow12,
                                int64_t n, int w, int h, double* res, double* jac, hipStream_t s);
psfm_status psfm_solve_batch(psfm_ctx* c, const double* uv12, const double* ref1, const double* ref2,
                             const double* scale, const float* flow12, int64_t n, int w, int h, double* out,
                             psfm_solve_stats* st, hipStream_t s);
```

particle-sfm_amd/csrc/psfm_persist.hip:

```cpp
#include <hip/hip_ext.h>
#include <stdlib.h>

#include "psfm_internal.h"
#include "psfm_chain.h"

#define PP_BLOCK 256
#define PP_NW (PP_BLOCK / PSFM_WAVE)
#define PP_PROBE 8
#ifndef PP_PRE_WAVES
#define PP_PRE_WAVES 4
#endif
#ifndef PP_KEEP
#define PP_KEEP 0
#endif
#ifndef PP_FC_AHEAD
#define PP_FC_AHEAD 4
#endif
#ifndef PP_FC_FAST
#define PP_FC_FAST 0
#endif
#define PP_GUESTS 32
#ifndef PP_WHATIF
#define PP_WHATIF 0
#endif
#ifndef PP_WAVES_N
#define PP_WAVES_N 8
#endif
#define PP_WAVES __attribute__((amdgpu_waves_per_eu(PP_WAVES_N, PP_WAVES_N)))

#ifdef PSFM_PERSIST_CHECK
#define PP_CHK(idx, lim, code) (((idx) >= 0 && (idx) < (lim)) ? true : (atomicCAS(&psfm_cold()->ctr->pad[0], 0, (code)), atomicMax(&psfm_cold()->ctr->pad[1], (int)(idx)), false))
#else
#define PP_CHK(idx, lim, code) true
#endif
#ifndef PP_COH_MARKS
#define PP_COH_MARKS true
#endif
#define PP_POOLED (-1)
#define PP_PEND (-2)
#define PP_DIED (-3)

struct PsfmPersistArgs {
    const float2* flows; uint8_t* occ;
    const float2* flows_b; float t2; int fc; int fc_xcd_per;
    int xcd_per;
    int64_t occ_pitch; PsfmFastDiv wdiv;
    int H, W; float cw, ch, rcw, rch;
    int ratio, GW, GH, G;
    float2* dlog; int cap;
    uint8_t* maps;
    unsigned long long* handoff;
    unsigned* bar;
    int n_flows;
    int nblk;
    PsfmFastDiv gwdiv, rdiv;
};
#define PP_SURV ((2 * PSFM_NSHARD + 1) * 32)

struct PsfmPersistCold {
    int cap_main;
    int cap;
    PsfmCounters* ctr;
    PsfmShard* shards;
    int* free_stack; int free_cap; int nsh;
    unsigned long long* fin_keys; int* fin_lanes;
    int seg_cap; int spill_base; int spill_cap;
    int2* seg_info;
    int shift_b, shift_d;
    int spin_limit;
};
struct PsfmPersistKernarg { PsfmPersistArgs hot; PsfmPersistCold cold; };

typedef const __attribute__((address_space(4))) PsfmPersistArgs* PsfmHotPtr;
typedef const __attribute__((address_space(4))) PsfmPersistCold* PsfmColdPtr;
__device__ __forceinline__ PsfmHotPtr psfm_hot()
{
    const __attribute__((address_space(4))) char* k = (const __attribute__((address_space(4))) char*)__builtin_amdgcn_kernarg_segment_ptr();
    asm volatile("" : "+s"(k));
    return (PsfmHotPtr)(k + offsetof(PsfmPersistKernarg, hot));
}
#define PA psfm_hot()
__device__ __forceinline__ int psfm_bid()
{
    int b = (int)blockIdx.x;
    asm volatile("" : "+s"(b));
    return b;
}
#define PP_BID psfm_bid()
#define PP_SHARD (psfm_bid() & (PSFM_NSHARD - 1))
template <class P> __device__ __forceinline__ PsfmFastDiv psfm_fd(P p)
{
    PsfmFastDiv f;
    f.m = p->m; f.sh1 = p->sh1; f.sh2 = p->sh2; f.d = 0u;
    return f;
}
__device__ __forceinline__ PsfmColdPtr psfm_cold()
{
    const __attribute__((address_space(4))) char* k = (const __attribute__((address_space(4))) char*)__builtin_amdgcn_kernarg_segment_ptr();
    asm volatile("" : "+s"(k));
    return (PsfmColdPtr)(k + offsetof(PsfmPersistKernarg, cold));
}

struct PsfmFrameView {
    const float2* flow; const uint8_t* occ;
    int H, W; float cw, ch, rcw, rch;
};
struct PsfmMarksView {
    int ratio, GW, GH;
    uint8_t* blocked_cur; uint8_t stamp_cur;
    PsfmFastDiv rdiv;
    float2* slab;
};

__device__ __forceinline__ PsfmFrameView psfm_frame_view(int t)
{
    const PsfmHotPtr a = psfm_hot();
    PsfmFrameView v;
    v.H = a->H; v.W = a->W; v.cw = a->cw; v.ch = a->ch; v.rcw = a->rcw; v.rch = a->rch;
    v.flow = a->flows + (size_t)t * ((size_t)v.H * v.W); v.occ = a->occ + (size_t)t * a->occ_pitch;
    return v;
}
template <int R>
__device__ __forceinline__ PsfmMarksView psfm_marks_view(int t)
{
    const PsfmHotPtr a = psfm_hot();
    PsfmMarksView m;
    m.ratio = R > 0 ? R : a->ratio; m.GW = a->GW; m.GH = a->GH;
    if (R > 0) { m.rdiv.m = 0u; m.rdiv.sh1 = 0; m.rdiv.sh2 = 0; m.rdiv.d = 0u; }
    else m.rdiv = psfm_fd(&a->rdiv);
    m.blocked_cur = a->maps + (size_t)(t % 3) * a->G; m.stamp_cur = 1;
    m.slab = a->dlog + (size_t)t * a->cap;
    return m;
}

__device__ __forceinline__ void psfm_put_record(int slot, unsigned long long key, int lane)
{
    const PsfmColdPtr c = psfm_cold();
    const int seg_cap = c->seg_cap;
    int64_t o;
    if (slot < seg_cap) {
        o = (int64_t)PP_BID * seg_cap + slot;
    } else {
        PsfmCounters* ctr = c->ctr;
        const int q = atomicAdd(&ctr->spill_cnt, 1);
        if (q >= c->spill_cap) { atomicOr(&ctr->overflow, 2); return; }
        o = (int64_t)c->spill_base + q;
    }
    if (!PP_CHK(lane, c->cap, 6)) return;
    c->fin_keys[o] = key;
    c->fin_lanes[o] = lane;
}
__device__ __forceinline__ unsigned long long psfm_cold_key(int last_time, int bf, int idx)
{
    const PsfmColdPtr c = psfm_cold();
    return psfm_key(last_time, bf, idx, c->shift_b, c->shift_d);
}

__device__ __forceinline__ int psfm_record_slot(int* s_rec_cnt, bool dead)
{
    const unsigned long long dm = __ballot(dead);
    if (dm == 0ull) return 0;
    int base = 0;
    if (psfm_lane_id() == (int)__builtin_ctzll(dm)) base = atomicAdd(s_rec_cnt, __popcll(dm));
    base = __shfl(base, (int)__builtin_ctzll(dm));
    return base + psfm_rank_in(dm);
}

#ifdef PSFM_TIMELINE
__device__ unsigned long long g_pp_tl[2 * 4096 * 8];
__device__ int g_pp_st[4096 * 8];
__device__ int g_pp_tl_frame = -1;
#define PP_TL(k) do { if ((unsigned)(t - g_pp_tl_frame) < 2u && tid == 0) g_pp_tl[((t - g_pp_tl_frame) * 4096 + blockIdx.x) * 8 + (k)] = __builtin_amdgcn_s_memrealtime(); } while (0)
extern "C" int psfm_debug_persist_timeline(int frame, unsigned long long* out_host, int n_blocks)
{
    if (out_host && n_blocks < 0) return hipMemcpyFromSymbol(out_host, HIP_SYMBOL(g_pp_st), (size_t)(-n_blocks) * 32) != hipSuccess;
    if (out_host) return hipMemcpyFromSymbol(out_host, HIP_SYMBOL(g_pp_tl), (size_t)2 * 4096 * 64) != hipSuccess;
    return hipMemcpyToSymbol(HIP_SYMBOL(g_pp_tl_frame), &frame, sizeof(int)) != hipSuccess;
}
#else
#define PP_TL(k) do {} while (0)
#endif

__device__ __forceinline__ void psfm_bar_arrive(int shard, int k, int lane)
{
    int last = 0;
    asm volatile("" : "+s"(k));
    if (lane == 0) {
        const int nblk = PA->nblk;
        const unsigned members = (unsigned)((nblk - shard + PSFM_NSHARD - 1) / PSFM_NSHARD);
        const unsigned old = __hip_atomic_fetch_add(PA->bar + shard * 32, 1u, __ATOMIC_RELAXED, __HIP_MEMORY_SCOPE_AGENT);
        if (old + 1 == members * (unsigned)(k + 1)) {
            const unsigned nsh = (unsigned)(nblk < PSFM_NSHARD ? nblk : PSFM_NSHARD);
            const unsigned o2 = __hip_atomic_fetch_add(PA->bar + 64 * 32, 1u, __ATOMIC_RELAXED, __HIP_MEMORY_SCOPE_AGENT);
            if (o2 + 1 == nsh * (unsigned)(k + 1)) last = 1;
        }
    }
    last = __builtin_amdgcn_readfirstlane(last);
    if (last) psfm_coh_st(PA->bar + (65 + lane) * 32, (unsigned)(k + 1));
}
__device__ __forceinline__ bool psfm_bar_wait(int shard, int k)
{
    const unsigned* flag = PA->bar + (65 + shard) * 32;
    int n = 0;
    while (psfm_coh_ld(flag) < (unsigned)(k + 1)) {
        __builtin_amdgcn_s_sleep(1);
        if (++n > psfm_cold()->spin_limit) { PsfmCounters* ctr = psfm_cold()->ctr; atomicOr(&ctr->overflow, 8); psfm_coh_st(&ctr->abort, 1); return false; }
        if ((n & 127) == 0 && psfm_coh_ld(&psfm_cold()->ctr->abort)) return false;
    }
    return true;
}

__device__ __forceinline__ void psfm_fc_slice(int f, int tid)
{
    const PsfmHotPtr a = psfm_hot();
    const int P = a->H * a->W;
    PsfmFcParams q;
    q.H = a->H; q.W = a->W; q.cw = a->cw; q.ch = a->ch; q.rcw = a->rcw; q.rch = a->rch; q.thres = 0.f ; q.t2 = a->t2;
    const float2* __restrict__ F = a->flows + (size_t)f * P;
    const float2* __restrict__ B = a->flows_b + (size_t)f * P;
    uint8_t* O = a->occ + (size_t)f * a->occ_pitch;
    const PsfmFastDiv wdiv = psfm_fd(&a->wdiv);
    const int W = a->W;
    const int nch = (P + 1023) / 1024;
    const int per = a->fc_xcd_per, nblk = a->nblk;
    for (int q0 = PP_BID; q0 < (per > 0 ? 8 * per : nch); q0 += nblk) {
        const int ci = per > 0 ? (q0 & 7) * per + (q0 >> 3) : q0;
        if (ci >= nch) continue;
        const int p0 = ci * 1024 + tid;
        float2 fv[4];
#pragma unroll
        for (int k = 0; k < 4; ++k) {
            const int p = p0 + k * 256;
            fv[k] = p < P ? psfm_ld(F, (unsigned)p * 8u) : make_float2(0.f, 0.f);
        }
        int y = (int)psfm_fastdiv((unsigned)p0, wdiv), x = p0 - y * W;
#pragma unroll
        for (int k = 0; k < 4; ++k) {
            const int p = p0 + k * 256;
            if (p >= P) break;
            uint8_t o;
#if PP_FC_FAST
            {
                const float X = __fadd_rn((float)x, fv[k].x), Y = __fadd_rn((float)y, fv[k].y);
                const PsfmTaps t = psfm_taps_t<true>(X, Y, q.cw, q.ch, q.rcw, q.rch, q.H, q.W);
                const bool interior = (t.x0 >= 0) & (t.x0 + 1 < q.W) & (t.y0 >= 0) & (t.y0 + 1 < q.H);
                if (__builtin_amdgcn_ballot_w64(!interior) == 0ull) o = psfm_flow_check_px_interior(B, X, Y, fv[k], t, q);
                else { float e; int xb = x, yb = y; asm volatile("" : "+v"(xb), "+v"(yb)); o = psfm_flow_check_px<false>(B, xb, yb, fv[k], q, &e); }
            }
#else
            float e;
            o = psfm_flow_check_px<false>(B, x, y, fv[k], q, &e);
#endif
            psfm_coh_st(O + p, o);
            x += 256;
            while (x >= W) { x -= W; ++y; }
        }
    }
}

__device__ __forceinline__ int psfm_vblock()
{
    const int b = PP_BID, per = PA->xcd_per;
    return (per > 0 && b < 8 * per) ? (b & 7) * per + (b >> 3) : b;
}

struct PsfmEntry { int kind, ex, host; };

template <int R>
__global__ __launch_bounds__(PP_BLOCK) PP_WAVES void psfm_chain_persist_kernel(PsfmPersistKernarg)
{
    __shared__ int s_births[PP_NW], s_adopt[PP_NW], s_pend[PP_NW];
    __shared__ int s_new_g[PP_BLOCK];
    __shared__ int s_ad_tid[PP_BLOCK];
    __shared__ int s_pend_tid[PP_BLOCK];
    __shared__ double2 s_xp[PP_BLOCK];
    __shared__ int s_xg[PP_BLOCK];
    __shared__ int s_xf[PP_BLOCK];
    __shared__ int s_gi[PP_BLOCK];
    __shared__ int s_npts[PP_BLOCK];
    __shared__ int s_seg_start[PP_PROBE + 1], s_seg_end[PP_PROBE + 1];
    __shared__ int s_nseg, s_base_free, s_ok, s_alive_any[2], s_rec_cnt, s_done;
    __shared__ double2 s_gp[PP_GUESTS];
    __shared__ int s_gbf[PP_GUESTS];
    __shared__ int s_ggi[PP_GUESTS];
    __shared__ int s_glive[PP_GUESTS], s_gfree[PP_GUESTS], s_nglive, s_ngfree;

    int tid = threadIdx.x;
    int L = psfm_vblock() * PP_BLOCK + tid;
    const int ratio = R > 0 ? R : PA->ratio;

    int bf = PP_POOLED;
    double2 p = make_double2(0.0, 0.0);
    s_gi[tid] = L;
    s_npts[tid] = 0;
    if (L < PA->G) {
        const PsfmHotPtr a = psfm_hot();
        const int gy = (int)psfm_fastdiv((unsigned)L, psfm_fd(&a->gwdiv)), gx = L - gy * a->GW;
        p = make_double2((double)(gx * ratio), (double)(gy * ratio));
        bf = 0;
        s_npts[tid] = 1;
    }
    s_xf[tid] = 0;
    if (tid < PP_GUESTS) s_gbf[tid] = -1;
    if (tid == 0) { s_rec_cnt = 0; s_alive_any[0] = 0; s_alive_any[1] = 0; s_done = 0; }
    int fc_next = 0;
    if (PA->fc) {
        for (; fc_next < 2 && fc_next < PA->n_flows; ++fc_next) psfm_fc_slice(fc_next, tid);
        __builtin_amdgcn_s_waitcnt(0);
    }
    __syncthreads();
    if (tid / PSFM_WAVE == PP_NW - 1) psfm_bar_arrive(PP_SHARD, 0, tid & (PSFM_WAVE - 1));
    if (PA->fc) {
        if (tid == 0) s_ok = psfm_bar_wait(PP_SHARD, 0) ? 1 : 0;
        __syncthreads();
        if (!s_ok) return;
    }

    for (int t = 0; t < PA->n_flows; ++t) {
        asm volatile("" : "+v"(tid));
        L = psfm_vblock() * PP_BLOCK + tid;
        const int lane = tid & (PSFM_WAVE - 1), wave = tid / PSFM_WAVE;
        PsfmFrameView v = psfm_frame_view(t);
        const int cur = t & 1, prev = cur ^ 1;

        PP_TL(0);
        const bool live = bf >= 0;
        bool any_alive = false;
        int npts = 0;
        auto own_step = [&](const PsfmFrameView& vs, int s, const PsfmStepLoads& ld, bool mine, bool& alive_any) {
            PsfmStep s1;
            s1.alive = true;
            if (mine) s1 = psfm_step_finish(vs, p, ld);
            const int slot1 = psfm_record_slot(&s_rec_cnt, !s1.alive);
            if (mine) {
                if (s1.alive) {
                    const PsfmMarksView m = psfm_marks_view<R>(s);
                    if (PP_CHK(L, PA->cap, 1)) m.slab[L] = s1.flow;
                    psfm_block_grid<R, PP_COH_MARKS>(m, (int)s1.next.x, (int)s1.next.y);
                    p = s1.next;
                    alive_any = true;
                    ++npts;
                } else {
                    psfm_put_record(slot1, psfm_cold_key(s, bf, s_gi[tid]), L);
                    bf = PP_DIED;
                    p = make_double2(0.0, 0.0);
                }
            }
        };
        PsfmStepLoads l1 = psfm_step_issue(v, p);

        auto do_E = [&]() { own_step(v, t, l1, live, any_alive); };
        const bool e_first = wave < PP_PRE_WAVES;
        if (e_first) do_E();

        if (PA->fc) {
            const PsfmHotPtr a = psfm_hot();
            const unsigned* flag = a->bar + (65 + PP_SHARD) * 32;
            const int nf = a->n_flows, fc_lim = t + PP_FC_AHEAD < nf ? t + PP_FC_AHEAD : nf;
            while (fc_next < fc_lim) {
                if (__builtin_amdgcn_readfirstlane((int)psfm_coh_ld(flag)) >= t + 1 || (PP_WHATIF & 32)) break;
                psfm_fc_slice(fc_next, tid);
                ++fc_next;
            }
        }
        if (tid == 0) s_ok = (PP_WHATIF & 4) ? 1 : (psfm_bar_wait(PP_SHARD, t) ? 1 : 0);
        __syncthreads();
        if (!s_ok) return;

#ifndef PP_NO_SETPRIO
        __builtin_amdgcn_s_setprio(3);
#endif
        PP_TL(1);
        const bool poll = t > 0 && bf == PP_POOLED && !(PP_WHATIF & 8);
        const PsfmHotPtr ac = psfm_hot();
        const int G = ac->G;
        const bool gridpt = t > 0 && L < G && !(PP_WHATIF & 8);
        uint8_t* map_prev = ac->maps + (size_t)((t + 2) % 3) * G;
        unsigned sv = 0, byte = 0;
        unsigned long long h0 = 0, h1 = 0, h2 = ~0ull;
        if (t > 0 && PP_BID == 0 && tid < PSFM_NSHARD) sv = psfm_coh_ld(ac->bar + PP_SURV + (prev * PSFM_NSHARD + tid) * 32);
        if (gridpt) byte = psfm_coh_ld(map_prev + L);
        if (poll) {
            const unsigned long long* h = ac->handoff + (size_t)L * 3;
            h0 = psfm_coh_ld(h); h1 = psfm_coh_ld(h + 1); h2 = psfm_coh_ld(h + 2);
        }

        v = psfm_frame_view(t);
        if (!e_first) do_E();

        const unsigned long long svm = __ballot(sv == (unsigned)t);
        bool birth = false;
        if (gridpt) {
            if (byte != 0) psfm_coh_st(map_prev + L, (uint8_t)0);
            birth = byte == 0;
            if (L == 0 && svm == 0ull) {
                const int r0 = R > 0 ? R : PA->ratio;
                birth = ((0 + 1) * (0 + 1) + 0 * 0) > r0 * r0;
            }
            if (PP_WHATIF & 1) birth = false;
        }
        bool adopted = false;
        if (poll) {
            const int tag = (int)(h2 >> 32);
            if ((tag >> 1) == t - 1 && !(PP_WHATIF & 1)) {
                if (tag & 1) {
                    adopted = true;
                    s_xp[tid] = make_double2(__longlong_as_double((long long)h0), __longlong_as_double((long long)h1));
                    s_xg[tid] = (int)(unsigned)h2;
                } else {
                    bf = PP_PEND;
                }
            }
        }
        const bool pend = bf == PP_PEND;
        if (bf == PP_DIED) bf = PP_PEND;
        const unsigned long long bm = __ballot(birth), am = __ballot(adopted), pm = __ballot(pend);
        if (lane == 0) { s_births[wave] = __popcll(bm); s_adopt[wave] = __popcll(am); s_pend[wave] = __popcll(pm); }
        if (birth) s_new_g[wave * PSFM_WAVE + psfm_rank_in(bm)] = L;
        if (adopted) s_ad_tid[wave * PSFM_WAVE + psfm_rank_in(am)] = tid;
        if (pend) s_pend_tid[wave * PSFM_WAVE + psfm_rank_in(pm)] = tid;
        if (wave == 0) {
            const int gb = tid < PP_GUESTS ? s_gbf[tid] : -1;
            const bool gl = gb >= 0, gf = (tid < PP_GUESTS) & (gb < 0);
            const unsigned long long glm = __ballot(gl), gfm = __ballot(gf);
            if (lane == 0) { s_nglive = __popcll(glm); s_ngfree = __popcll(gfm); }
            if (gl) s_glive[psfm_rank_in(glm)] = tid;
            if (gf) s_gfree[psfm_rank_in(gfm)] = tid;
        }
        __syncthreads();

        PP_TL(2);
        int nb = 0, nad = 0, npd = 0, my_pend_before = 0;
#pragma unroll
        for (int w = 0; w < PP_NW; ++w) {
            if (w == wave) my_pend_before = npd;
            nb += s_births[w]; nad += s_adopt[w]; npd += s_pend[w];
        }
        const int matched = nb < npd ? nb : npd;
        const int ngl = s_nglive;
        const int gmatched = (nb - matched) < s_ngfree ? (nb - matched) : s_ngfree;
        const int n2 = nb + nad + ngl;
        const int t_frame = t, nb_f = __builtin_amdgcn_readfirstlane(nb), nad_f = __builtin_amdgcn_readfirstlane(nad), npd_f = __builtin_amdgcn_readfirstlane(npd),
                  matched_f = __builtin_amdgcn_readfirstlane(matched), gmatched_f = __builtin_amdgcn_readfirstlane(gmatched);

        for (int base = 0; base == 0 || base < n2; base += PP_BLOCK) {
            int t = t_frame, nb = nb_f, nad = nad_f, npd = npd_f, matched = matched_f, gmatched = gmatched_f;
            asm volatile("" : "+s"(t), "+s"(nb), "+s"(nad), "+s"(npd), "+s"(matched), "+s"(gmatched));
            const int cur = t & 1, prev = cur ^ 1;
            const int k = base + tid;
            PsfmEntry e;
            e.kind = 0; e.ex = -1; e.host = -1;
            if (k < nb) {
                int before = 0, pb = 0;
#pragma unroll
                for (int w = 0; w < PP_NW; ++w) {
                    const int c = s_births[w], pc = s_pend[w];
                    if (k >= before && k < before + c) e.ex = s_new_g[w * PSFM_WAVE + (k - before)];
                    if (k >= pb && k < pb + pc) e.host = s_pend_tid[w * PSFM_WAVE + (k - pb)];
                    before += c; pb += pc;
                }
                e.kind = 1;
            } else if (k < nb + nad) {
                const int kk = k - nb;
                int before = 0;
#pragma unroll
                for (int w = 0; w < PP_NW; ++w) {
                    const int c = s_adopt[w];
                    if (kk >= before && kk < before + c) e.ex = s_ad_tid[w * PSFM_WAVE + (kk - before)];
                    before += c;
                }
                e.kind = 2;
            } else if (k < n2) {
                e.ex = s_glive[k - nb - nad];
                e.kind = 3;
            }
            PsfmStepLoads l2 = {};
            if (e.kind != 0) {
                double2 q;
                if (e.kind == 1) {
                    const PsfmHotPtr a = psfm_hot();
                    const int gy = (int)psfm_fastdiv((unsigned)e.ex, psfm_fd(&a->gwdiv)), gx = e.ex - gy * a->GW;
                    q = make_double2((double)(gx * ratio), (double)(gy * ratio));
                } else if (e.kind == 2) {
                    q = s_xp[e.ex];
                } else {
                    q = s_gp[e.ex];
                }
                l2 = psfm_step_issue(v, q);
            }
#ifdef PSFM_TIMELINE
            if (base == 0 && tid == 0 && t == g_pp_tl_frame) {
                int* st = g_pp_st + PP_BID * 8;
                st[0] = nb; st[1] = nad; st[2] = npd; st[3] = ngl; st[4] = s_ngfree; st[5] = nb - matched - gmatched; st[6] = npd - matched - PP_KEEP;
            }
#endif
            if (base == 0 && tid == 0) {
                const PsfmColdPtr c = psfm_cold();
                const int nsh = c->nsh, free_cap = c->free_cap;
                PsfmShard* sh_pop = c->shards + cur * PSFM_NSHARD;
                PsfmShard* sh_push = c->shards + prev * PSFM_NSHARD;
                int need = nb - matched - gmatched;
                const int n_push = npd - matched - PP_KEEP;
                int bfree = 0;
                const int fsh = PP_BID % nsh;
                if (n_push > 0) bfree = atomicAdd(&sh_push[fsh].free_top, n_push);
                int nseg = 0, done = 0;
                for (int rd = 0; rd < PP_PROBE / 4 && need > 0; ++rd) {
                    const int q4 = need >> 2, r4 = need & 3;
                    int sh[4], ask[4], old[4];
#pragma unroll
                    for (int j = 0; j < 4; ++j) {
                        sh[j] = (fsh + (rd * 4 + j) * 7) % nsh;
                        ask[j] = q4 + (j < r4 ? 1 : 0);
                        old[j] = ask[j] > 0 ? atomicSub(&sh_pop[sh[j]].free_top, ask[j]) : 0;
                    }
#pragma unroll
                    for (int j = 0; j < 4; ++j) {
                        const int take = old[j] < 0 ? 0 : (old[j] > ask[j] ? ask[j] : old[j]);
                        if (take < ask[j]) atomicAdd(&sh_pop[sh[j]].free_top, ask[j] - take);
                        if (take > 0) {
                            s_seg_start[nseg] = sh[j] * free_cap + old[j] - 1;
                            done += take;
                            s_seg_end[nseg] = done;
                            ++nseg;
                            need -= take;
                        }
                    }
                }
                s_base_free = bfree;
                if (need > 0) {
                    const int base_new = atomicAdd(&c->ctr->n_lanes, need);
                    s_seg_start[nseg] = -(base_new + 1);
                    done += need;
                    s_seg_end[nseg] = done;
                    ++nseg;
                }
                s_nseg = nseg;
            }
            PP_TL(3);
            __syncthreads();
            PP_TL(4);

            if (base == 0) {
                if (pend) {
                    const int r = my_pend_before + psfm_rank_in(pm);
                    if (r >= matched + PP_KEEP) {
                        const PsfmColdPtr c = psfm_cold();
                        const int free_cap = c->free_cap;
                        int* free_push = c->free_stack + (size_t)prev * free_cap * PSFM_NSHARD;
                        const int fpos = s_base_free + (r - matched - PP_KEEP);
                        if (fpos < free_cap && PP_CHK(fpos, free_cap, 7)) psfm_coh_st(free_push + (size_t)(PP_BID % c->nsh) * free_cap + fpos, L);
                        else atomicOr(&c->ctr->overflow, 1);
                        bf = PP_POOLED;
                    }
                }
            }
            psfm_step_pin<true>(l2);
            asm volatile("" : "+v"(e.ex));
            if (e.kind != 0) {
                double2 q;
                int bfk, gik, col, gs = -1;
                if (e.kind == 1) {
                    const PsfmHotPtr a = psfm_hot();
                    const int gy = (int)psfm_fastdiv((unsigned)e.ex, psfm_fd(&a->gwdiv)), gx = e.ex - gy * a->GW;
                    q = make_double2((double)(gx * ratio), (double)(gy * ratio));
                    bfk = t; gik = e.ex;
                    if (k < matched) {
                        col = psfm_vblock() * PP_BLOCK + e.host;
                    } else if (k < matched + gmatched) {
                        gs = s_gfree[k - matched];
                        col = psfm_cold()->cap_main + PP_BID * PP_GUESTS + gs;
                    } else {
                        const PsfmColdPtr c = psfm_cold();
                        const int* free_pop = c->free_stack + (size_t)cur * c->free_cap * PSFM_NSHARD;
                        const int qq = k - matched - gmatched;
                        int j = 0, pv = 0;
                        while (j < s_nseg - 1 && qq >= s_seg_end[j]) { pv = s_seg_end[j]; ++j; }
                        const int st = s_seg_start[j];
                        if (st >= 0) (void)PP_CHK(st - (qq - pv), 2 * c->free_cap * PSFM_NSHARD, 9);
                        col = st >= 0 ? psfm_coh_ld(free_pop + (st - (qq - pv))) : (-(st + 1) + (qq - pv));
                        if (col >= c->cap_main) col = -1;
                    }
                } else if (e.kind == 2) {
                    q = s_xp[e.ex];
                    bfk = t - 1; gik = s_xg[e.ex];
                    col = psfm_vblock() * PP_BLOCK + e.ex;
                } else {
                    q = s_gp[e.ex];
                    bfk = s_gbf[e.ex]; gik = s_ggi[e.ex];
                    col = psfm_cold()->cap_main + PP_BID * PP_GUESTS + e.ex;
                }
                if (col >= 0) {
                    (void)PP_CHK(col, PA->cap, 2);
                    const PsfmStep s2 = psfm_step_finish(v, q, l2);
                    if (e.kind == 1) ++npts;
                    if (s2.alive) {
                        const PsfmMarksView m = psfm_marks_view<R>(t);
                        if (PP_CHK(col, PA->cap, 3)) m.slab[col] = s2.flow;
                        psfm_block_grid<R, PP_COH_MARKS>(m, (int)s2.next.x, (int)s2.next.y);
                        any_alive = true;
                        ++npts;
                    } else {
                        const int slot = atomicAdd(&s_rec_cnt, 1);
                        psfm_put_record(slot, psfm_cold_key(t, bfk, gik), col);
                    }
                    if (e.kind == 1) {
                        const bool popped = k >= matched + gmatched;
                        const int nf = PA->n_flows;
                        if (popped && s2.alive && t == nf - 1) {
                            const int slot = atomicAdd(&s_rec_cnt, 1);
                            psfm_put_record(slot, psfm_cold_key(nf, t, e.ex), col);
                        }
                        if (k < matched) {
                            s_xp[e.host] = s2.next; s_xg[e.host] = e.ex; s_xf[e.host] = s2.alive ? 1 : 2;
                        } else if (gs >= 0) {
                            if (s2.alive) { s_gp[gs] = s2.next; s_ggi[gs] = e.ex; s_gbf[gs] = t; }
                        } else if (PP_CHK(col, psfm_cold()->cap_main, 8)) {
                            unsigned long long* h = PA->handoff + (size_t)col * 3;
                            psfm_coh_st(h, (unsigned long long)__double_as_longlong(s2.next.x));
                            psfm_coh_st(h + 1, (unsigned long long)__double_as_longlong(s2.next.y));
                            psfm_coh_st(h + 2, (unsigned long long)(unsigned)e.ex |
                                                   ((unsigned long long)(unsigned)(2 * t + (s2.alive ? 1 : 0)) << 32));
                        }
                    } else if (e.kind == 2) {
                        if (s2.alive) s_xp[e.ex] = s2.next;
                        s_xf[e.ex] = s2.alive ? 3 : 2;
                    } else {
                        if (s2.alive) s_gp[e.ex] = s2.next;
                        else s_gbf[e.ex] = -1;
                    }
                } else {
                    atomicOr(&psfm_cold()->ctr->overflow, 4);
                }
            }
        }
        PP_TL(5);
        asm volatile("" : "+s"(t), "+v"(tid));
        if (npts) s_npts[tid] += npts;
        const unsigned long long alm = __ballot(any_alive);
        if (lane == 0 && alm != 0ull) s_alive_any[t & 1] = 1;
        __syncthreads();
        {
            const int f = s_xf[tid];
            if (f != 0) {
                s_xf[tid] = 0;
                if (f != 2) {
                    bf = f == 3 ? t - 1 : t;
                    s_gi[tid] = s_xg[tid];
                    p = s_xp[tid];
                } else {
                    bf = PP_PEND;
                }
            }
        }
        if (tid == 0 && s_alive_any[t & 1]) { psfm_coh_st(PA->bar + PP_SURV + ((t & 1) * PSFM_NSHARD + PP_SHARD) * 32, (unsigned)(t + 1)); s_alive_any[t & 1] = 0; }
        if (PA->fc) {
            const int nf = PA->n_flows, need = t + 3 < nf ? t + 3 : nf;
            if (!(PP_WHATIF & 16)) for (; fc_next < need; ++fc_next) psfm_fc_slice(fc_next, tid);
        }
        if (!(PP_WHATIF & 2)) asm volatile("s_waitcnt vmcnt(0) lgkmcnt(0)" ::: "memory");
        PP_TL(6);
        {
            int last_wave = 0;
            if (lane == 0) last_wave = atomicAdd(&s_done, 1) == PP_NW - 1 ? 1 : 0;
            last_wave = __builtin_amdgcn_readfirstlane(last_wave);
            if (last_wave) {
                if (lane == 0) s_done = 0;
                PP_TL(7);
                psfm_bar_arrive(PP_SHARD, t + 1, lane);
            }
        }
#ifndef PP_NO_SETPRIO
        __builtin_amdgcn_s_setprio(0);
#endif
    }

    const int lane = tid & (PSFM_WAVE - 1), wave = tid / PSFM_WAVE;
    {
        const int nf = PA->n_flows;
        const bool alive = bf >= 0;
        const int slot = psfm_record_slot(&s_rec_cnt, alive);
        if (alive) psfm_put_record(slot, psfm_cold_key(nf, bf, s_gi[tid]), L);
        if (tid < PP_GUESTS && s_gbf[tid] >= 0) {
            const int gslot = atomicAdd(&s_rec_cnt, 1);
            psfm_put_record(gslot, psfm_cold_key(nf, s_gbf[tid], s_ggi[tid]),
                            psfm_cold()->cap_main + PP_BID * PP_GUESTS + tid);
        }
    }
    {
        __shared__ int s_pts[PP_NW];
        int w = s_npts[tid];
#pragma unroll
        for (int o = 32; o > 0; o >>= 1) w += __shfl_down(w, o);
        if (lane == 0) s_pts[wave] = w;
        __syncthreads();
        if (tid == 0) {
            int tot = 0;
            for (int j = 0; j < PP_NW; ++j) tot += s_pts[j];
            const int c = s_rec_cnt;
            const PsfmColdPtr cold = psfm_cold();
            const int seg_cap = cold->seg_cap;
            cold->seg_info[PP_BID] = make_int2(c < seg_cap ? c : seg_cap, tot);
        }
    }
}

__global__ __launch_bounds__(256) void psfm_persist_init_kernel(PsfmCounters* ctr, PsfmShard* shards, int G,
                                                                unsigned long long* maps64, size_t n_maps64,
                                                                unsigned long long* bar64, size_t n_bar64,
                                                                unsigned long long* handoff, size_t n_handoff)
{
    const size_t i = (size_t)blockIdx.x * 256 + threadIdx.x, stride = (size_t)gridDim.x * 256;
    if (i == 0) { ctr->n_lanes = G; ctr->overflow = 0; ctr->stall = 0; ctr->abort = 0; ctr->spill_cnt = 0; ctr->pad[0] = 0; ctr->pad[1] = 0; }
    if (i < 2 * PSFM_NSHARD) { shards[i].fin_cnt = 0; shards[i].free_top = 0; shards[i].points = 0u; }
    for (size_t k = i; k < n_maps64; k += stride) maps64[k] = 0ull;
    for (size_t k = i; k < n_bar64; k += stride) bar64[k] = 0ull;
    for (size_t k = i; k < n_handoff; k += stride) handoff[k] = ~0ull;
}

int psfm_persist_guests(void) { return PP_GUESTS; }

int psfm_persist_max_blocks(psfm_ctx* c)
{
    if (c->persist_max_blocks >= 0) return c->persist_max_blocks;
    int cus = 0;
    c->persist_max_blocks = 0;
    if (hipDeviceGetAttribute(&cus, hipDeviceAttributeMultiprocessorCount, c->device) != hipSuccess) {
        (void)hipGetLastError();
        return 0;
    }
    int per_cu = 1 << 30;
    const void* inst[4] = {(const void*)psfm_chain_persist_kernel<0>, (const void*)psfm_chain_persist_kernel<1>,
                           (const void*)psfm_chain_persist_kernel<2>, (const void*)psfm_chain_persist_kernel<4>};
    for (int k = 0; k < 4; ++k) {
        int v = 0;
        if (hipOccupancyMaxActiveBlocksPerMultiprocessor(&v, inst[k], PP_BLOCK, 0) != hipSuccess) {
            (void)hipGetLastError();
            return 0;
        }
        per_cu = v < per_cu ? v : per_cu;
    }
    if (per_cu > 8) per_cu = 8;
    c->persist_max_blocks = per_cu * cus;
    return c->persist_max_blocks;
}

psfm_status psfm_launch_chain_persist(psfm_ctx* c, const PsfmTrackDims& d, const float* flows, const uint8_t* occ,
                                      int64_t occ_pitch, const float* flows_b, float thres, hipStream_t s)
{
    const size_t bar_bytes = (size_t)(4 * PSFM_NSHARD + 1) * 128;
    {
        const size_t n_maps64 = ((size_t)d.G * 3 + 7) / 8, n_bar64 = bar_bytes / 8, n_handoff = (size_t)d.nblk * PP_BLOCK * 3;
        hipLaunchKernelGGL(psfm_persist_init_kernel, dim3(1024), dim3(256), 0, s, c->counters.as<PsfmCounters>(),
                           c->shards.as<PsfmShard>(), (int)d.G, c->occupied.as<unsigned long long>(), n_maps64,
                           c->persist_bar.as<unsigned long long>(), n_bar64, c->handoff.as<unsigned long long>(), n_handoff);
    }
    PsfmPersistKernarg ka;
    PsfmPersistArgs& a = ka.hot;
    PsfmPersistCold& k = ka.cold;
    a.flows = (const float2*)flows; a.occ = const_cast<uint8_t*>(occ);
    a.occ_pitch = occ_pitch;
    a.flows_b = (const float2*)flows_b; a.t2 = psfm_sq_threshold(thres); a.fc = flows_b != nullptr;
    {
        static const int xcd_on = getenv("PSFM_FC_XCD") ? atoi(getenv("PSFM_FC_XCD")) : 1;
        const int64_t nch = ((int64_t)d.H * d.W + 1023) / 1024;
        a.fc_xcd_per = xcd_on && nch >= 64 ? (int)((nch + 7) / 8) : 0;
    }
    {
        static const int pp_xcd = getenv("PSFM_PP_XCD") ? atoi(getenv("PSFM_PP_XCD")) : 1;
        const int64_t gb = (d.G + PP_BLOCK - 1) / PP_BLOCK;
        const int per = (int)((gb + 7) / 8);
        a.xcd_per = (pp_xcd && gb >= 64 && 8 * per <= d.nblk) ? per : 0;
    }
    a.wdiv = psfm_fastdiv_make((unsigned)d.W);
    a.H = d.H; a.W = d.W; a.cw = d.cw; a.ch = d.ch; a.rcw = psfm_rcp_host(d.cw); a.rch = psfm_rcp_host(d.ch);
    a.ratio = d.ratio; a.GW = d.GW; a.GH = d.GH; a.G = (int)d.G;
    a.dlog = c->log.as<float2>(); a.cap = k.cap = (int)d.cap; k.cap_main = d.nblk * PP_BLOCK;
    a.maps = c->occupied.as<uint8_t>();
    k.ctr = c->counters.as<PsfmCounters>();
    k.shards = c->shards.as<PsfmShard>();
    k.free_stack = c->free_stack.as<int>(); k.free_cap = d.free_cap; k.nsh = d.nsh;
    a.handoff = c->handoff.as<unsigned long long>();
    k.fin_keys = c->fin_keys.as<unsigned long long>(); k.fin_lanes = c->fin_lanes.as<int>();
    k.seg_cap = d.seg_cap; k.spill_base = d.nblk * d.seg_cap; k.spill_cap = d.spill_cap;
    k.seg_info = c->seg_info.as<int2>();
    a.bar = c->persist_bar.as<unsigned>();
    a.n_flows = d.n_flows; a.nblk = d.nblk; k.shift_b = d.shift_b; k.shift_d = d.shift_d;
    a.gwdiv = psfm_fastdiv_make((unsigned)d.GW); a.rdiv = psfm_fastdiv_make((unsigned)d.ratio);
    k.spin_limit = 1 << 18;
    if (const char* e = getenv("PSFM_PERSIST_SPIN_LIMIT")) k.spin_limit = atoi(e);
    hipEvent_t e0 = nullptr, e1 = nullptr;
    c->prof.kernel_span(PSFM_PROF_CHAIN, &e0, &e1, true);
    const dim3 grid((unsigned)d.nblk), block(PP_BLOCK);
    const bool coop = getenv("PSFM_PERSIST_COOP") && atoi(getenv("PSFM_PERSIST_COOP")) != 0;
    const void* fn = d.ratio == 1 ? (const void*)psfm_chain_persist_kernel<1> : d.ratio == 2 ? (const void*)psfm_chain_persist_kernel<2>
                   : d.ratio == 4 ? (const void*)psfm_chain_persist_kernel<4> : (const void*)psfm_chain_persist_kernel<0>;
    if (coop) {
        void* kargs[] = {(void*)&ka};
        if (e0) PSFM_HIP(hipEventRecord(e0, s));
        const hipError_t le = hipLaunchCooperativeKernel(fn, grid, block, kargs, 0, s);
        if (le != hipSuccess) {
            (void)hipGetLastError();
            psfm_set_error("cooperative launch of the persistent frame loop refused: %s", hipGetErrorString(le));
            return PSFM_ERR_CAPACITY;
        }
        if (e1) PSFM_HIP(hipEventRecord(e1, s));
        return PSFM_OK;
    }
    switch (d.ratio) {
        case 1: hipExtLaunchKernelGGL(psfm_chain_persist_kernel<1>, grid, block, 0, s, e0, e1, 0, ka); break;
        case 2: hipExtLaunchKernelGGL(psfm_chain_persist_kernel<2>, grid, block, 0, s, e0, e1, 0, ka); break;
        case 4: hipExtLaunchKernelGGL(psfm_chain_persist_kernel<4>, grid, block, 0, s, e0, e1, 0, ka); break;
        default: hipExtLaunchKernelGGL(psfm_chain_persist_kernel<0>, grid, block, 0, s, e0, e1, 0, ka); break;
    }
    PSFM_HIP(hipGetLastError());
    return PSFM_OK;
}
```

Before: 21.65 billion trajectory-points/s.

## Overlap persistent finalize group counting on side stream and skip redundant state reset

```diff
diff --git a/particle-sfm_amd/csrc/psfm_api.hip b/particle-sfm_amd/csrc/psfm_api.hip
--- a/particle-sfm_amd/csrc/psfm_api.hip
+++ b/particle-sfm_amd/csrc/psfm_api.hip
@@ -150,7 +150,7 @@
     (void)hipSetDevice(c->device);
     PsfmBuf* bufs[] = {&c->log, &c->birth_frame, &c->birth_idx, &c->free_stack, &c->fin_keys, &c->fin_lanes,
                        &c->occupied, &c->counters, &c->shards, &c->survivors, &c->sort_keys, &c->sort_lanes, &c->sort_tmp,
-                       &c->scan_tmp, &c->fin_marks, &c->res_birth, &c->res_len, &c->res_off, &c->res_xy, &c->sol_x, &c->sol_state,
+                       &c->scan_tmp, &c->fin_marks, &c->fin_counts, &c->fin_totals, &c->res_birth, &c->res_len, &c->res_off, &c->res_xy, &c->sol_x, &c->sol_state,
                        &c->sol_partials, &c->sol_ctrl, &c->sol_misc, &c->sol_stats, &c->sol_fused, &c->sol_bar, &c->sol_list, &c->occ_own, &c->occ2_own,
                        &c->handoff, &c->seg_info, &c->seg_table, &c->persist_bar, &c->batch_tab, &c->batch_ws, &c->batch_fc, &c->win_ws, &c->flt_ids, &c->flt_birth, &c->flt_len, &c->flt_off, &c->flt_xy,
                        &c->mt_kp_off, &c->mt_q, &c->mt_pts, &c->mt_kp_ind, &c->mt_kp_xy, &c->mt_moff, &c->mt_keys, &c->mt_rows, &c->mt_gid, &c->mt_pairs,
@@ -161,6 +161,10 @@
     psfm_shard_abandon(c);
     c->prof.destroy();
     if (c->side_stream) (void)hipStreamDestroy(c->side_stream);
+    if (c->fin_stream) (void)hipStreamDestroy(c->fin_stream);
+    if (c->fin_ev_compact) (void)hipEventDestroy(c->fin_ev_compact);
+    if (c->fin_ev_side) (void)hipEventDestroy(c->fin_ev_side);
+    if (c->host_fin) (void)hipHostFree(c->host_fin);
     if (c->redo_stream) (void)hipStreamDestroy(c->redo_stream);
     if (c->copy_stream) (void)hipStreamDestroy(c->copy_stream);
     if (c->copy_stream2) (void)hipStreamDestroy(c->copy_stream2);
@@ -177,6 +181,7 @@
 extern "C" psfm_status psfm_ctx_set_capacity(psfm_ctx* c, double lane_factor, double traj_factor)
 {
     if (!c || !(lane_factor >= 1.0) || !(traj_factor >= 1.0)) { psfm_set_error("psfm_ctx_set_capacity: factors must be >= 1"); return PSFM_ERR_ARG; }
+    if (c->lane_factor != lane_factor || c->traj_factor != traj_factor) c->persist_clean.ok = false;
     c->lane_factor = lane_factor;
     c->traj_factor = traj_factor;
     return PSFM_OK;
@@ -370,6 +375,7 @@
 {
     psfm_status st;
     const int n_flows = d.n_flows;
+    c->persist_clean.ok = false;
     if ((st = c->log.ensure(sizeof(double2) * (size_t)(n_flows + 1) * d.cap)) != PSFM_OK) return st;
     if ((st = c->birth_frame.ensure(sizeof(int) * d.cap)) != PSFM_OK) return st;
     if ((st = c->birth_idx.ensure(sizeof(int) * d.cap)) != PSFM_OK) return st;
@@ -422,6 +428,7 @@
     psfm_status st;
     if ((st = psfm_track_dims(c, n_flows, h, w, ratio, -1, d)) != PSFM_OK) return st;
     const int64_t P = (int64_t)h * w;
+    const psfm_ctx::PersistClean was_clean = c->persist_clean;
     if ((st = psfm_track_alloc(c, d)) != PSFM_OK) return st;
 
     c->solve_stats.clear();
@@ -455,12 +462,14 @@
             if ((st = c->handoff.ensure((size_t)dp.nblk * 256 * 24)) != PSFM_OK) return st;
             if ((st = c->seg_info.ensure(sizeof(int) * 2 * (size_t)dp.nblk)) != PSFM_OK) return st;
             if ((st = c->persist_bar.ensure((size_t)(4 * PSFM_NSHARD + 1) * 128)) != PSFM_OK) return st;
+            if ((st = psfm_finalize_persist_prepare(c, dp)) != PSFM_OK) return st;
             if (pipe && (st = pipe->need(n_flows - 1, false, s)) != PSFM_OK) return st;
             bool fallback = false;
             {
                 const bool trace = getenv("PSFM_TRACE") != nullptr;
                 const auto t1 = std::chrono::steady_clock::now();
-                st = psfm_launch_chain_persist(c, dp, flows, occ, occ_pitch, fuse_flows_b, fuse_thres, s);
+                st = psfm_launch_chain_persist(c, dp, flows, occ, occ_pitch, fuse_flows_b, fuse_thres,
+                                               psfm_persist_state_clean(c, was_clean, dp), s);
                 if (st == PSFM_ERR_CAPACITY) {
                     fallback = true;
                     st = PSFM_OK;
@@ -479,7 +488,11 @@
             }
             if (st != PSFM_OK) return st;
             if (!fallback) {
-                PSFM_HIP(hipStreamSynchronize(s));
+                {
+                    const hipError_t e = hipStreamSynchronize(s);
+                    if (e != hipSuccess) c->persist_clean.ok = false;
+                    PSFM_HIP(e);
+                }
                 c->prof.collect();
                 if (info) {
                     memset(info, 0, sizeof(*info));
diff --git a/particle-sfm_amd/csrc/psfm_finalize.hip b/particle-sfm_amd/csrc/psfm_finalize.hip
--- a/particle-sfm_amd/csrc/psfm_finalize.hip
+++ b/particle-sfm_amd/csrc/psfm_finalize.hip
@@ -1,3 +1,4 @@
+#include <chrono>
 #include <cstring>
 #include <stdio.h>
 #include <rocprim/device/device_radix_sort.hpp>
@@ -226,6 +227,96 @@
         for (int g = g0; g < g1; ++g) {
             goff[g] = run;
             run += (long long)s_g[g] * (long long)(l - b + 1);
+            if (++b > l) { ++l; b = 0; }
+        }
+    }
+    if (tid == 0) *off_n = total;
+}
+
+#define PSFM_COUNT_BLOCKS 32
+#define PSFM_COUNT_BLOCK 1024
+__global__ __launch_bounds__(PSFM_COUNT_BLOCK) void psfm_group_count_kernel(
+    const unsigned long long* __restrict__ fin_keys, const int2* __restrict__ seg_info, int nblk, int seg_cap, int spilled, int shift_b,
+    int shift_d, int ng, int* __restrict__ rows)
+{
+    extern __shared__ int s_h[];
+    constexpr int NW = PSFM_COUNT_BLOCK / PSFM_WAVE, NLD = 8;
+    const int tid = threadIdx.x, lane = tid & (PSFM_WAVE - 1), wave = tid / PSFM_WAVE;
+    for (int k = tid; k < ng; k += PSFM_COUNT_BLOCK) s_h[k] = 0;
+    __syncthreads();
+    const unsigned long long bmask = (1ull << (shift_d - shift_b)) - 1ull;
+    for (int seg = blockIdx.x * NW + wave; seg <= nblk; seg += gridDim.x * NW) {
+        const int cnt = seg < nblk ? min(max(seg_info[seg].x, 0), seg_cap) : spilled;
+        const unsigned long long* __restrict__ src = fin_keys + (long long)seg * seg_cap;
+        for (int i0 = 0; i0 < cnt; i0 += NLD * PSFM_WAVE) {
+            unsigned long long k[NLD];
+#pragma unroll
+            for (int u = 0; u < NLD; ++u) {
+                const int i = i0 + u * PSFM_WAVE + lane;
+                k[u] = i < cnt ? src[i] : 0ull;
+            }
+#pragma unroll
+            for (int u = 0; u < NLD; ++u) {
+                const int i = i0 + u * PSFM_WAVE + lane;
+                const unsigned last = (unsigned)(k[u] >> shift_d);
+                const unsigned birth = (unsigned)((k[u] >> shift_b) & bmask);
+                const unsigned g = last * (last + 1u) / 2u + birth;
+                if (i < cnt && g < (unsigned)ng) atomicAdd(&s_h[g], 1);
+            }
+        }
+    }
+    __syncthreads();
+    int* __restrict__ row = rows + (size_t)blockIdx.x * ng;
+    for (int k = tid; k < ng; k += PSFM_COUNT_BLOCK) row[k] = s_h[k];
+}
+
+__global__ __launch_bounds__(PSFM_PLAN_BLOCK) void psfm_group_plan_counts_kernel(const int* __restrict__ rows, int nrows, int* __restrict__ gstart,
+                                                                                 int64_t* __restrict__ goff, int ng,
+                                                                                 int64_t* __restrict__ off_n)
+{
+    __shared__ int s_g[PSFM_PLAN_MAX_GROUPS];
+    __shared__ long long s_wsum[PSFM_PLAN_BLOCK / PSFM_WAVE];
+    __shared__ long long s_wcnt[PSFM_PLAN_BLOCK / PSFM_WAVE];
+    constexpr int NW = PSFM_PLAN_BLOCK / PSFM_WAVE;
+    const int tid = threadIdx.x, lane = tid & (PSFM_WAVE - 1), wave = tid / PSFM_WAVE;
+    for (int k = tid; k < ng; k += PSFM_PLAN_BLOCK) {
+        int v = 0;
+        for (int r = 0; r < nrows; ++r) v += rows[(size_t)r * ng + k];
+        s_g[k] = v;
+    }
+    __syncthreads();
+    const int per = (ng + PSFM_PLAN_BLOCK - 1) / PSFM_PLAN_BLOCK;
+    const int g0 = min(tid * per, ng), g1 = min(g0 + per, ng);
+    int last = 0, birth = 0;
+    if (g0 < g1) psfm_tri_invert((unsigned)g0, &last, &birth);
+    long long cnt = 0, pts = 0;
+    {
+        int l = last, b = birth;
+        for (int g = g0; g < g1; ++g) {
+            cnt += (long long)s_g[g];
+            pts += (long long)s_g[g] * (long long)(l - b + 1);
+            if (++b > l) { ++l; b = 0; }
+        }
+    }
+    long long inc = pts, cinc = cnt;
+#pragma unroll
+    for (int o = 1; o < PSFM_WAVE; o <<= 1) {
+        const long long v = __shfl_up(inc, o), w = __shfl_up(cinc, o);
+        if (lane >= o) { inc += v; cinc += w; }
+    }
+    if (lane == PSFM_WAVE - 1) { s_wsum[wave] = inc; s_wcnt[wave] = cinc; }
+    __syncthreads();
+    long long base = 0, total = 0, cbase = 0;
+    for (int w = 0; w < NW; ++w) { const long long v = s_wsum[w]; if (w < wave) { base += v; cbase += s_wcnt[w]; } total += v; }
+    long long run = base + inc - pts, crun = cbase + cinc - cnt;
+    {
+        int l = last, b = birth;
+        for (int g = g0; g < g1; ++g) {
+            const int c = s_g[g];
+            gstart[g] = c > 0 ? (int)crun : -1;
+            goff[g] = run;
+            crun += (long long)c;
+            run += (long long)c * (long long)(l - b + 1);
             if (++b > l) { ++l; b = 0; }
         }
     }
@@ -448,42 +539,66 @@
     return psfm_own_sort(fmt, n) && (psfm_sort_pairs32_passes(end_bit) % 2 == 0);
 }
 
-static psfm_status psfm_finalize_sorted(psfm_ctx* c, const PsfmTrackDims& d, int64_t n, int64_t npts, bool delta_log, hipStream_t s)
+struct PsfmSideWork { int nblk, seg_cap, spilled; };
+
+static psfm_status psfm_finalize_sorted(psfm_ctx* c, const PsfmTrackDims& d, int64_t n, int64_t npts, bool delta_log, void* k_half1,
+                                        int* l_half1, const PsfmSideWork* side, hipStream_t s)
 {
     psfm_status st;
     unsigned end_bit = 0;
     const PsfmKeyFmt fmt = psfm_key_fmt(d, &end_bit);
-    int* l_in = c->sort_lanes.as<int>() + n;
+    int* l_in = l_half1;
     int* l_out = c->sort_lanes.as<int>();
+    static const int plan_on = getenv("PSFM_FIN_PLAN") ? atoi(getenv("PSFM_FIN_PLAN")) : 1;
+    const long long lmax = (long long)d.n_flows + 1;
+    const long long ng = lmax * (lmax + 1) / 2 + lmax + 1;
+    const bool use_plan = plan_on && ng <= PSFM_PLAN_MAX_GROUPS && n < (1ll << 31);
+    const bool side_plan = side && use_plan && fmt.use32;
     size_t tmp_bytes = 0, scan_bytes = 0;
-    PSFM_HIP(rocprim::exclusive_scan(nullptr, scan_bytes, (int64_t*)nullptr, (int64_t*)nullptr, (int64_t)0,
-                                     (size_t)(n + 1), rocprim::plus<int64_t>(), s));
+    if (!use_plan)
+        PSFM_HIP(rocprim::exclusive_scan(nullptr, scan_bytes, (int64_t*)nullptr, (int64_t*)nullptr, (int64_t)0,
+                                         (size_t)(n + 1), rocprim::plus<int64_t>(), s));
+    if ((st = c->res_birth.ensure(sizeof(int) * n)) != PSFM_OK) return st;
+    if ((st = c->res_len.ensure(sizeof(int) * n)) != PSFM_OK) return st;
+    if ((st = c->res_off.ensure(sizeof(int64_t) * (n + 1))) != PSFM_OK) return st;
+    PsfmPlan pl;
+    pl.gstart = nullptr; pl.goff = nullptr; pl.keys = (const void*)c->sort_keys.p; pl.use32 = fmt.use32; pl.shift_b = d.shift_b; pl.shift_d = d.shift_d;
+    pl.birth_w = c->res_birth.as<int>(); pl.len_w = c->res_len.as<int>(); pl.off_w = c->res_off.as<int64_t>();
+    if (side_plan) {
+        if ((st = c->scan_tmp.ensure((sizeof(int64_t) + sizeof(int)) * (size_t)ng)) != PSFM_OK) return st;
+        if ((st = c->fin_counts.ensure(sizeof(int) * (size_t)ng * PSFM_COUNT_BLOCKS)) != PSFM_OK) return st;
+        int64_t* goff = c->scan_tmp.as<int64_t>();
+        int* gstart = (int*)(goff + ng);
+        constexpr int NW = PSFM_COUNT_BLOCK / PSFM_WAVE;
+        int rows = (side->nblk + 1 + NW - 1) / NW;
+        rows = rows < PSFM_COUNT_BLOCKS ? rows : PSFM_COUNT_BLOCKS;
+        hipLaunchKernelGGL(psfm_group_count_kernel, dim3((unsigned)rows), dim3(PSFM_COUNT_BLOCK), sizeof(int) * (size_t)ng, c->fin_stream,
+                           (const unsigned long long*)c->fin_keys.as<unsigned long long>(), (const int2*)c->seg_info.as<int2>(), side->nblk,
+                           side->seg_cap, side->spilled, d.shift_b, d.shift_d, (int)ng, c->fin_counts.as<int>());
+        hipLaunchKernelGGL(psfm_group_plan_counts_kernel, dim3(1), dim3(PSFM_PLAN_BLOCK), 0, c->fin_stream, (const int*)c->fin_counts.as<int>(),
+                           rows, gstart, goff, (int)ng, c->res_off.as<int64_t>() + n);
+        PSFM_HIP(hipGetLastError());
+        pl.gstart = gstart; pl.goff = goff;
+    }
+    if (side) PSFM_HIP(hipEventRecord(c->fin_ev_side, c->fin_stream));
     if (psfm_own_sort(fmt, n)) {
         if ((st = c->sort_tmp.ensure(scan_bytes)) != PSFM_OK) return st;
-        if ((st = psfm_sort_pairs32(c, c->sort_keys.as<unsigned>(), l_out, c->sort_keys.as<unsigned>() + n, l_in, n, end_bit, s)) != PSFM_OK) return st;
+        if ((st = psfm_sort_pairs32(c, c->sort_keys.as<unsigned>(), l_out, (unsigned*)k_half1, l_in, n, end_bit, s)) != PSFM_OK) return st;
     } else if (fmt.use32) {
-        unsigned* k_in = c->sort_keys.as<unsigned>() + n;
+        unsigned* k_in = (unsigned*)k_half1;
         unsigned* k_out = c->sort_keys.as<unsigned>();
         PSFM_HIP(rocprim::radix_sort_pairs(nullptr, tmp_bytes, k_in, k_out, l_in, l_out, (size_t)n, 0u, end_bit, s));
         if ((st = c->sort_tmp.ensure(tmp_bytes > scan_bytes ? tmp_bytes : scan_bytes)) != PSFM_OK) return st;
         PSFM_HIP(rocprim::radix_sort_pairs(c->sort_tmp.p, tmp_bytes, k_in, k_out, l_in, l_out, (size_t)n, 0u, end_bit, s));
     } else {
-        unsigned long long* k_in = c->sort_keys.as<unsigned long long>() + n;
+        unsigned long long* k_in = (unsigned long long*)k_half1;
         unsigned long long* k_out = c->sort_keys.as<unsigned long long>();
         PSFM_HIP(rocprim::radix_sort_pairs(nullptr, tmp_bytes, k_in, k_out, l_in, l_out, (size_t)n, 0u, end_bit, s));
         if ((st = c->sort_tmp.ensure(tmp_bytes > scan_bytes ? tmp_bytes : scan_bytes)) != PSFM_OK) return st;
         PSFM_HIP(rocprim::radix_sort_pairs(c->sort_tmp.p, tmp_bytes, k_in, k_out, l_in, l_out, (size_t)n, 0u, end_bit, s));
     }
-    if ((st = c->res_birth.ensure(sizeof(int) * n)) != PSFM_OK) return st;
-    if ((st = c->res_len.ensure(sizeof(int) * n)) != PSFM_OK) return st;
-    if ((st = c->res_off.ensure(sizeof(int64_t) * (n + 1))) != PSFM_OK) return st;
-    static const int plan_on = getenv("PSFM_FIN_PLAN") ? atoi(getenv("PSFM_FIN_PLAN")) : 1;
-    const long long lmax = (long long)d.n_flows + 1;
-    const long long ng = lmax * (lmax + 1) / 2 + lmax + 1;
-    PsfmPlan pl;
-    pl.gstart = nullptr; pl.goff = nullptr; pl.keys = (const void*)c->sort_keys.p; pl.use32 = fmt.use32; pl.shift_b = d.shift_b; pl.shift_d = d.shift_d;
-    pl.birth_w = c->res_birth.as<int>(); pl.len_w = c->res_len.as<int>(); pl.off_w = c->res_off.as<int64_t>();
-    if (plan_on && ng <= PSFM_PLAN_MAX_GROUPS && n < (1ll << 31)) {
+    if (side_plan) {
+    } else if (use_plan) {
         if ((st = c->scan_tmp.ensure((sizeof(int64_t) + sizeof(int)) * (size_t)ng)) != PSFM_OK) return st;
         int64_t* goff = c->scan_tmp.as<int64_t>();
         int* gstart = (int*)(goff + ng);
@@ -515,6 +630,7 @@
     }
     c->res_n_points = npts;
     if ((st = c->res_xy.ensure(sizeof(double2) * (size_t)(npts > 0 ? npts : 1))) != PSFM_OK) return st;
+    if (side) PSFM_HIP(hipStreamWaitEvent(s, c->fin_ev_side, 0));
     if (delta_log)
         hipLaunchKernelGGL(psfm_gather_delta_kernel, dim3((unsigned)((n + TILE_J - 1) / TILE_J)), dim3(PSFM_BLOCK), 0, s,
                            c->log.as<float2>(), d.cap, c->sort_lanes.as<int>(), c->res_birth.as<int>(),
@@ -572,25 +688,65 @@
                        c->fin_keys.as<unsigned long long>(), c->fin_lanes.as<int>(), d.shard_cap, so,
                        kdst, c->sort_lanes.as<int>() + half, fmt);
     PSFM_HIP(hipGetLastError());
-    return psfm_finalize_sorted(c, d, n, npts, false, s);
-}
+    void* k1 = fmt.use32 ? (void*)(c->sort_keys.as<unsigned>() + n) : (void*)(c->sort_keys.as<unsigned long long>() + n);
+    return psfm_finalize_sorted(c, d, n, npts, false, k1, c->sort_lanes.as<int>() + n, nullptr, s);
+}
+
+struct PsfmFinTotals {
+    long long n, n_points;
+    int overflow, n_lanes, spill_cnt, pad0, pad1;
+    unsigned epoch;
+};
 
 __global__ __launch_bounds__(PSFM_BLOCK) void psfm_compact_segments_kernel(
     const unsigned long long* __restrict__ fin_keys, const int* __restrict__ fin_lanes, const int2* __restrict__ seg_info, int nblk,
     int seg_cap, const PsfmCounters* __restrict__ ctr, int spill_cap, unsigned long long* __restrict__ keys, int* __restrict__ lanes,
-    PsfmKeyFmt fmt)
+    PsfmKeyFmt fmt, PsfmFinTotals* pub_host, PsfmFinTotals* __restrict__ pub_dev, unsigned epoch)
 {
     __shared__ long long s_part[PSFM_BLOCK / PSFM_WAVE];
+    __shared__ long long s_pts[PSFM_BLOCK / PSFM_WAVE];
     const int b = blockIdx.x, tid = threadIdx.x;
+    if (b == 0 && pub_dev) {
+        long long cn = 0, cp = 0;
+        for (int k = tid; k < nblk; k += PSFM_BLOCK) {
+            const int2 v = seg_info[k];
+            cn += min(max(v.x, 0), seg_cap);
+            cp += v.y;
+        }
+#pragma unroll
+        for (int o = 32; o > 0; o >>= 1) { cn += __shfl_down(cn, o); cp += __shfl_down(cp, o); }
+        if ((tid & (PSFM_WAVE - 1)) == 0) { s_part[tid / PSFM_WAVE] = cn; s_pts[tid / PSFM_WAVE] = cp; }
+        __syncthreads();
+        if (tid == 0) {
+            long long n = 0, pts = 0;
+            for (int w = 0; w < PSFM_BLOCK / PSFM_WAVE; ++w) { n += s_part[w]; pts += s_pts[w]; }
+            const int sc = ctr->spill_cnt;
+            n += min(max(sc, 0), spill_cap);
+            const int overflow = ctr->overflow, n_lanes = ctr->n_lanes, p0 = ctr->pad[0], p1 = ctr->pad[1];
+            pub_dev->n = n; pub_dev->n_points = pts; pub_dev->overflow = overflow; pub_dev->n_lanes = n_lanes;
+            pub_dev->spill_cnt = sc; pub_dev->pad0 = p0; pub_dev->pad1 = p1; pub_dev->epoch = epoch;
+            if (pub_host) {
+                __hip_atomic_store(&pub_host->n, n, __ATOMIC_RELAXED, __HIP_MEMORY_SCOPE_SYSTEM);
+                __hip_atomic_store(&pub_host->n_points, pts, __ATOMIC_RELAXED, __HIP_MEMORY_SCOPE_SYSTEM);
+                __hip_atomic_store(&pub_host->overflow, overflow, __ATOMIC_RELAXED, __HIP_MEMORY_SCOPE_SYSTEM);
+                __hip_atomic_store(&pub_host->n_lanes, n_lanes, __ATOMIC_RELAXED, __HIP_MEMORY_SCOPE_SYSTEM);
+                __hip_atomic_store(&pub_host->spill_cnt, sc, __ATOMIC_RELAXED, __HIP_MEMORY_SCOPE_SYSTEM);
+                __hip_atomic_store(&pub_host->pad0, p0, __ATOMIC_RELAXED, __HIP_MEMORY_SCOPE_SYSTEM);
+                __hip_atomic_store(&pub_host->pad1, p1, __ATOMIC_RELAXED, __HIP_MEMORY_SCOPE_SYSTEM);
+                __hip_atomic_store(&pub_host->epoch, epoch, __ATOMIC_RELEASE, __HIP_MEMORY_SCOPE_SYSTEM);
+            }
+        }
+        __syncthreads();
+    }
     long long mine = 0;
-    for (int k = tid; k < b; k += PSFM_BLOCK) mine += seg_info[k].x;
+    for (int k = tid; k < b && k < nblk; k += PSFM_BLOCK) mine += min(max(seg_info[k].x, 0), seg_cap);
 #pragma unroll
     for (int o = 32; o > 0; o >>= 1) mine += __shfl_down(mine, o);
     if ((tid & (PSFM_WAVE - 1)) == 0) s_part[tid / PSFM_WAVE] = mine;
     __syncthreads();
     long long dst = 0;
     for (int w = 0; w < PSFM_BLOCK / PSFM_WAVE; ++w) dst += s_part[w];
-    const int count = b < nblk ? seg_info[b].x : min(ctr->spill_cnt, spill_cap);
+    const int count = b < nblk ? min(max(seg_info[b].x, 0), seg_cap) : min(max(ctr->spill_cnt, 0), spill_cap);
     const long long src = (long long)b * seg_cap;
     for (int i0 = 0; i0 < count; i0 += 4 * PSFM_BLOCK) {
         unsigned long long k[4];
@@ -612,10 +768,137 @@
     }
 }
 
+static bool psfm_fin_handoff_on(void)
+{
+    static const int on = getenv("PSFM_FIN_HANDOFF") ? atoi(getenv("PSFM_FIN_HANDOFF")) : 1;
+    return on != 0;
+}
+
+static int64_t psfm_persist_cap_n(const PsfmTrackDims& d) { return (int64_t)d.nblk * d.seg_cap + d.spill_cap; }
+
+psfm_status psfm_finalize_persist_prepare(psfm_ctx* c, const PsfmTrackDims& d)
+{
+    psfm_status st;
+    unsigned end_bit = 0;
+    const PsfmKeyFmt fmt = psfm_key_fmt(d, &end_bit);
+    const int64_t cap_n = psfm_persist_cap_n(d);
+    if ((st = c->sort_keys.ensure((fmt.use32 ? sizeof(unsigned) : sizeof(unsigned long long)) * (size_t)cap_n * 2)) != PSFM_OK) return st;
+    if ((st = c->sort_lanes.ensure(sizeof(int) * (size_t)cap_n * 2)) != PSFM_OK) return st;
+    if (!psfm_fin_handoff_on()) return PSFM_OK;
+    if ((st = c->fin_totals.ensure(sizeof(PsfmFinTotals))) != PSFM_OK) return st;
+    if (!c->host_fin) {
+        PSFM_HIP(hipHostMalloc(&c->host_fin, 64, hipHostMallocCoherent));
+        memset(c->host_fin, 0, 64);
+    }
+    if (!c->fin_stream) PSFM_HIP(hipStreamCreateWithFlags(&c->fin_stream, hipStreamNonBlocking));
+    if (!c->fin_ev_compact) PSFM_HIP(hipEventCreateWithFlags(&c->fin_ev_compact, hipEventDisableTiming));
+    if (!c->fin_ev_side) PSFM_HIP(hipEventCreateWithFlags(&c->fin_ev_side, hipEventDisableTiming));
+    const long long lmax = (long long)d.n_flows + 1;
+    const long long ng = lmax * (lmax + 1) / 2 + lmax + 1;
+    if (fmt.use32 && ng <= PSFM_PLAN_MAX_GROUPS) {
+        if ((st = c->scan_tmp.ensure((sizeof(int64_t) + sizeof(int)) * (size_t)ng)) != PSFM_OK) return st;
+        if ((st = c->fin_counts.ensure(sizeof(int) * (size_t)ng * PSFM_COUNT_BLOCKS)) != PSFM_OK) return st;
+    }
+    return PSFM_OK;
+}
+
+static bool psfm_poll_epoch(const unsigned* word, unsigned epoch, hipStream_t s, hipError_t* err)
+{
+    using clk = std::chrono::steady_clock;
+    *err = hipSuccess;
+    const auto t0 = clk::now();
+    auto tq = t0;
+    for (;;) {
+        for (int k = 0; k < 64; ++k) {
+            if (__atomic_load_n(word, __ATOMIC_ACQUIRE) == epoch) return true;
+#if defined(__x86_64__) || defined(__i386__)
+            __builtin_ia32_pause();
+#endif
+        }
+        const auto now = clk::now();
+        if (now - tq >= std::chrono::microseconds(100)) {
+            tq = now;
+            const hipError_t e = hipStreamQuery(s);
+            if (e == hipSuccess) return __atomic_load_n(word, __ATOMIC_ACQUIRE) == epoch;
+            if (e != hipErrorNotReady) { *err = e; return false; }
+            if (now - t0 >= std::chrono::seconds(4)) return false;
+        }
+    }
+}
+
 psfm_status psfm_finalize_persist(psfm_ctx* c, const PsfmTrackDims& d, bool* fallback, hipStream_t s)
 {
     *fallback = false;
     const int nseg = d.nblk + 1;
+    psfm_status st;
+    unsigned end_bit_unused = 0;
+    const PsfmKeyFmt fmt = psfm_key_fmt(d, &end_bit_unused);
+    const int64_t cap_n = psfm_persist_cap_n(d);
+    const bool first = psfm_records_in_first_half(d, cap_n);
+    void* k_half1 = fmt.use32 ? (void*)(c->sort_keys.as<unsigned>() + cap_n) : (void*)(c->sort_keys.as<unsigned long long>() + cap_n);
+    int* l_half1 = c->sort_lanes.as<int>() + cap_n;
+    unsigned long long* kdst = first ? c->sort_keys.as<unsigned long long>() : (unsigned long long*)k_half1;
+    int* ldst = first ? c->sort_lanes.as<int>() : l_half1;
+    PsfmCounters* hc = (PsfmCounters*)c->host_pinned;
+    int64_t n = 0, npts = 0;
+    const bool handoff = psfm_fin_handoff_on();
+    if (handoff) {
+        PsfmFinTotals* hf = (PsfmFinTotals*)c->host_fin;
+        void* hf_dev = nullptr;
+        PSFM_HIP(hipHostGetDevicePointer(&hf_dev, c->host_fin, 0));
+        unsigned epoch = ++c->fin_epoch;
+        if (epoch == 0) epoch = ++c->fin_epoch;
+        hipLaunchKernelGGL(psfm_compact_segments_kernel, dim3((unsigned)nseg), dim3(PSFM_BLOCK), 0, s,
+                           c->fin_keys.as<unsigned long long>(), c->fin_lanes.as<int>(), (const int2*)c->seg_info.as<int2>(), d.nblk, d.seg_cap,
+                           (const PsfmCounters*)c->counters.as<PsfmCounters>(), d.spill_cap, kdst, ldst, fmt, (PsfmFinTotals*)hf_dev,
+                           c->fin_totals.as<PsfmFinTotals>(), epoch);
+        PSFM_HIP(hipGetLastError());
+        PSFM_HIP(hipEventRecord(c->fin_ev_compact, s));
+        PSFM_HIP(hipStreamWaitEvent(c->fin_stream, c->fin_ev_compact, 0));
+        if ((st = psfm_launch_persist_reset(c, d, c->fin_stream)) != PSFM_OK) return st;
+        auto leave = [&](psfm_status r) { (void)hipStreamSynchronize(c->fin_stream); return r; };
+        hipError_t perr = hipSuccess;
+        PsfmFinTotals t;
+        if (psfm_poll_epoch(&hf->epoch, epoch, s, &perr)) {
+            t = *hf;
+        } else {
+            if (perr != hipSuccess) {
+                psfm_set_error("persistent loop / compaction failed: %s", hipGetErrorString(perr));
+                return leave(PSFM_ERR_HIP);
+            }
+            if (hipMemcpyAsync(&t, c->fin_totals.p, sizeof(t), hipMemcpyDeviceToHost, s) != hipSuccess || hipStreamSynchronize(s) != hipSuccess ||
+                t.epoch != epoch) {
+                psfm_set_error("persistent finalize: the totals of the compaction did not arrive (%s)", hipGetErrorString(hipGetLastError()));
+                return leave(PSFM_ERR_HIP);
+            }
+        }
+        hc->overflow = t.overflow; hc->n_lanes = t.n_lanes; hc->spill_cnt = t.spill_cnt; hc->pad[0] = t.pad0; hc->pad[1] = t.pad1;
+        n = t.n; npts = t.n_points;
+        if (hc->pad[0]) fprintf(stderr, "psfm persist check: site %d index %d\n", hc->pad[0], hc->pad[1]);
+        if (hc->overflow & (4 | 8)) {
+            *fallback = true;
+            return leave(PSFM_OK);
+        }
+        if (hc->overflow != 0) {
+            psfm_set_error("capacity exceeded (persistent loop): overflow bits %d, trajectory records %lld (%d spilled of %d); "
+                           "raise psfm_ctx_set_capacity", hc->overflow, (long long)n, hc->spill_cnt, d.spill_cap);
+            return leave(PSFM_ERR_CAPACITY);
+        }
+        c->res_n_traj = n;
+        c->res_n_points = 0;
+        if (n == 0) {
+            st = leave(PSFM_OK);
+            psfm_persist_mark_clean(c, d);
+            return st;
+        }
+        PsfmSideWork side;
+        side.nblk = d.nblk; side.seg_cap = d.seg_cap;
+        side.spilled = hc->spill_cnt < 0 ? 0 : (hc->spill_cnt < d.spill_cap ? hc->spill_cnt : d.spill_cap);
+        st = psfm_finalize_sorted(c, d, n, npts, true, k_half1, l_half1, &side, s);
+        if (st != PSFM_OK) return leave(st);
+        psfm_persist_mark_clean(c, d);
+        return PSFM_OK;
+    }
     const size_t need = sizeof(int2) * (size_t)d.nblk;
     if (c->host_seg_bytes < need) {
         if (c->host_seg) (void)hipHostFree(c->host_seg);
@@ -624,7 +907,6 @@
         c->host_seg_bytes = need;
     }
     int2* hinfo = (int2*)c->host_seg;
-    PsfmCounters* hc = (PsfmCounters*)c->host_pinned;
     PSFM_HIP(hipMemcpyAsync(hc, c->counters.p, sizeof(PsfmCounters), hipMemcpyDeviceToHost, s));
     PSFM_HIP(hipMemcpyAsync(hinfo, c->seg_info.p, sizeof(int2) * (size_t)d.nblk, hipMemcpyDeviceToHost, s));
     PSFM_HIP(hipStreamSynchronize(s));
@@ -633,7 +915,6 @@
         *fallback = true;
         return PSFM_OK;
     }
-    int64_t n = 0, npts = 0;
     for (int b = 0; b < d.nblk; ++b) {
         n += hinfo[b].x;
         npts += hinfo[b].y;
@@ -648,18 +929,12 @@
     c->res_n_traj = n;
     c->res_n_points = 0;
     if (n == 0) return PSFM_OK;
-    psfm_status st;
-    if ((st = c->sort_keys.ensure(sizeof(unsigned long long) * n * 2)) != PSFM_OK) return st;
-    if ((st = c->sort_lanes.ensure(sizeof(int) * n * 2)) != PSFM_OK) return st;
-    unsigned end_bit_unused = 0;
-    const PsfmKeyFmt fmt = psfm_key_fmt(d, &end_bit_unused);
-    const int64_t half = psfm_records_in_first_half(d, n) ? 0 : n;
-    unsigned long long* kdst = fmt.use32 ? (unsigned long long*)(c->sort_keys.as<unsigned>() + half) : c->sort_keys.as<unsigned long long>() + half;
     hipLaunchKernelGGL(psfm_compact_segments_kernel, dim3((unsigned)nseg), dim3(PSFM_BLOCK), 0, s,
                        c->fin_keys.as<unsigned long long>(), c->fin_lanes.as<int>(), (const int2*)c->seg_info.as<int2>(), d.nblk, d.seg_cap,
-                       (const PsfmCounters*)c->counters.as<PsfmCounters>(), d.spill_cap, kdst, c->sort_lanes.as<int>() + half, fmt);
+                       (const PsfmCounters*)c->counters.as<PsfmCounters>(), d.spill_cap, kdst, ldst, fmt, (PsfmFinTotals*)nullptr,
+                       (PsfmFinTotals*)nullptr, 0u);
     PSFM_HIP(hipGetLastError());
-    return psfm_finalize_sorted(c, d, n, npts, true, s);
+    return psfm_finalize_sorted(c, d, n, npts, true, k_half1, l_half1, nullptr, s);
 }
 
 struct PsfmFinSeq {
diff --git a/particle-sfm_amd/csrc/psfm_internal.h b/particle-sfm_amd/csrc/psfm_internal.h
--- a/particle-sfm_amd/csrc/psfm_internal.h
+++ b/particle-sfm_amd/csrc/psfm_internal.h
@@ -130,6 +130,19 @@
     PsfmBuf sort_keys, sort_lanes, sort_tmp, scan_tmp;
     PsfmBuf fin_marks;
     bool fin_marks_clean = false;
+    void* host_fin = nullptr;
+    PsfmBuf fin_totals;
+    unsigned fin_epoch = 0;
+    hipStream_t fin_stream = nullptr;
+    hipEvent_t fin_ev_compact = nullptr, fin_ev_side = nullptr;
+    PsfmBuf fin_counts;
+    struct PersistClean {
+        bool ok = false;
+        const void* counters = nullptr; const void* shards = nullptr; const void* maps = nullptr; const void* bar = nullptr;
+        const void* handoff = nullptr;
+        int64_t G = 0;
+        int nblk = 0;
+    } persist_clean;
     PsfmBuf res_birth, res_len, res_off, res_xy;
     int64_t res_n_traj = 0, res_n_points = 0;
     int res_n_flows = 0;
@@ -246,11 +259,15 @@
 int psfm_persist_max_blocks(psfm_ctx* c);
 int psfm_persist_guests(void);
 psfm_status psfm_launch_chain_persist(psfm_ctx* c, const PsfmTrackDims& d, const float* flows, const uint8_t* occ,
-                                      int64_t occ_pitch, const float* flows_b, float thres, hipStream_t s);
+                                      int64_t occ_pitch, const float* flows_b, float thres, bool state_clean, hipStream_t s);
+psfm_status psfm_launch_persist_reset(psfm_ctx* c, const PsfmTrackDims& d, hipStream_t s);
+bool psfm_persist_state_clean(const psfm_ctx* c, const psfm_ctx::PersistClean& was, const PsfmTrackDims& d);
+void psfm_persist_mark_clean(psfm_ctx* c, const PsfmTrackDims& d);
 
 psfm_status psfm_finalize(psfm_ctx* c, const PsfmTrackDims& d, hipStream_t s);
 int psfm_sort_pairs32_passes(unsigned end_bit);
 psfm_status psfm_sort_pairs32(psfm_ctx* c, unsigned* k_half0, int* v_half0, unsigned* k_half1, int* v_half1, int64_t n, unsigned end_bit, hipStream_t s);
+psfm_status psfm_finalize_persist_prepare(psfm_ctx* c, const PsfmTrackDims& d);
 psfm_status psfm_finalize_persist(psfm_ctx* c, const PsfmTrackDims& d, bool* fallback, hipStream_t s);
 
 psfm_status psfm_solve_frame_enqueue(psfm_ctx* c, const PsfmTrackDims& d, const float* flow01, const float* flow12,
diff --git a/particle-sfm_amd/csrc/psfm_persist.hip b/particle-sfm_amd/csrc/psfm_persist.hip
--- a/particle-sfm_amd/csrc/psfm_persist.hip
+++ b/particle-sfm_amd/csrc/psfm_persist.hip
@@ -745,15 +745,37 @@
     return c->persist_max_blocks;
 }
 
+psfm_status psfm_launch_persist_reset(psfm_ctx* c, const PsfmTrackDims& d, hipStream_t s)
+{
+    const size_t bar_bytes = (size_t)(4 * PSFM_NSHARD + 1) * 128;
+    const size_t n_maps64 = ((size_t)d.G * 3 + 7) / 8, n_bar64 = bar_bytes / 8, n_handoff = (size_t)d.nblk * PP_BLOCK * 3;
+    hipLaunchKernelGGL(psfm_persist_init_kernel, dim3(1024), dim3(256), 0, s, c->counters.as<PsfmCounters>(),
+                       c->shards.as<PsfmShard>(), (int)d.G, c->occupied.as<unsigned long long>(), n_maps64,
+                       c->persist_bar.as<unsigned long long>(), n_bar64, c->handoff.as<unsigned long long>(), n_handoff);
+    PSFM_HIP(hipGetLastError());
+    return PSFM_OK;
+}
+
+bool psfm_persist_state_clean(const psfm_ctx* c, const psfm_ctx::PersistClean& was, const PsfmTrackDims& d)
+{
+    return was.ok && was.counters == c->counters.p && was.shards == c->shards.p && was.maps == c->occupied.p &&
+           was.bar == c->persist_bar.p && was.handoff == c->handoff.p && was.G == d.G && was.nblk == d.nblk;
+}
+
+void psfm_persist_mark_clean(psfm_ctx* c, const PsfmTrackDims& d)
+{
+    psfm_ctx::PersistClean& m = c->persist_clean;
+    m.ok = true;
+    m.counters = c->counters.p; m.shards = c->shards.p; m.maps = c->occupied.p; m.bar = c->persist_bar.p; m.handoff = c->handoff.p;
+    m.G = d.G; m.nblk = d.nblk;
+}
+
 psfm_status psfm_launch_chain_persist(psfm_ctx* c, const PsfmTrackDims& d, const float* flows, const uint8_t* occ,
-                                      int64_t occ_pitch, const float* flows_b, float thres, hipStream_t s)
-{
-    const size_t bar_bytes = (size_t)(4 * PSFM_NSHARD + 1) * 128;
-    {
-        const size_t n_maps64 = ((size_t)d.G * 3 + 7) / 8, n_bar64 = bar_bytes / 8, n_handoff = (size_t)d.nblk * PP_BLOCK * 3;
-        hipLaunchKernelGGL(psfm_persist_init_kernel, dim3(1024), dim3(256), 0, s, c->counters.as<PsfmCounters>(),
-                           c->shards.as<PsfmShard>(), (int)d.G, c->occupied.as<unsigned long long>(), n_maps64,
-                           c->persist_bar.as<unsigned long long>(), n_bar64, c->handoff.as<unsigned long long>(), n_handoff);
+                                      int64_t occ_pitch, const float* flows_b, float thres, bool state_clean, hipStream_t s)
+{
+    if (!state_clean) {
+        psfm_status st = psfm_launch_persist_reset(c, d, s);
+        if (st != PSFM_OK) return st;
     }
     PsfmPersistKernarg ka;
     PsfmPersistArgs& a = ka.hot;
```

Result: no change. 21.50 billion trajectory-points/s (-0.7%).
